# QingYunA/General-Medical-Image-Segmentation-CNN-Framework

Hardware: AMD Instinct MI355X
Metric: train voxels/sec (128^3 patches) 3D U-Net (higher is better)
Workload: dtype f32 (f16x3 split MFMA: every fp32 conv operand = two fp16 parts under a per-tensor power-of-two scale, three fp16 products per fp32 product, fp32 accumulate; graded against fp64 by the same tests as bf16x6 and the exact-fp32 MFMA path); 1 GPU; unet3d_f32_2x128: UNet3D(1,2,32) fwd+BCE+bwd+Adam+Dice, x=[2,1,128,128,128] fp32 per GPU, random-init (kaiming) weights, data-parallel replicas with RCCL gradient all-reduce, conv math f16x3; global_batch=2, parallelism=dp1, conv_math=f16x3, optimizer=torch.optim.Adam(fused=True)

## Files before the change

### general-medical-image-segmentation-cnn-framework_amd/csrc/bn_head.hip

```cpp
#include "common.h"
#include "internal.h"

namespace seg {

namespace {

constexpr int kBhMaxBlocks = 1024;

struct BhArgs {
    const float* y; int ldy;
    const float* mean; const float* rstd; const float* gamma; const float* beta;
    const float* wh; const float* bh;
    const float* dl; int lddl;
    float* out; int ldo;
    const float* s1; const float* s2;
    float* part;
    unsigned* amax;
    long long rows; int C; int act; float slope;
};

template <int K, int ACT>
__device__ __forceinline__ void bn_head_fwd_body(const BhArgs& a) {
    const int LPV = a.C / 4, VPB = 256 / LPV;
    const int c4 = threadIdx.x % LPV, vl = threadIdx.x / LPV;
    f32x4_t wr[K], al, be;
#pragma unroll
    for (int k = 0; k < K; ++k) wr[k] = ld4(a.wh + (long long)k * a.C + c4 * 4);
#pragma unroll
    for (int j = 0; j < 4; ++j) {
        al[j] = a.rstd[c4 * 4 + j] * (a.gamma ? a.gamma[c4 * 4 + j] : 1.f);
        be[j] = (a.beta ? a.beta[c4 * 4 + j] : 0.f) - a.mean[c4 * 4 + j] * al[j];
    }
    float bias[K];
#pragma unroll
// ... 104 lines not shown
        float s = vals[i];
        for (int o = 32; o >= LPV; o >>= 1) s += __shfl_xor(s, o, 64);
        vals[i] = s;
    }
    const int nl = LPV < 64 ? LPV : 64;
    if (lane < nl) {
#pragma unroll
        for (int i = 0; i < NS + K; ++i) sred[(wave * 64 + lane) * (NS + K) + i] = vals[i];
    }
    __syncthreads();
    const int ncol = (2 + K) * a.C + K;
    float* dst = a.part + (long long)blockIdx.x * ncol;
    for (int i = threadIdx.x; i < ncol; i += 256) {
        float s = 0.f;
        if (i < (2 + K) * a.C) {
            const int which = i / a.C, c = i % a.C;
            const int slot = which < 2 ? which * 4 + c % 4 : 8 + 4 * (which - 2) + c % 4;
            for (int w = 0; w < 4; ++w) s += sred[(w * 64 + (c / 4) % 64) * (NS + K) + slot];
        } else {
            const int k = i - (2 + K) * a.C;
            for (int w = 0; w < 4; ++w) s += sred[(w * 64 + 0) * (NS + K) + NS + k];
        }
        dst[i] = s;
    }
}
template <int K>
__global__ __launch_bounds__(256) void bn_head_bwd_sums_kernel(BhArgs a) {
    if (a.act == MI355SEG_ACT_RELU) bn_head_bwd_sums_body<K, MI355SEG_ACT_RELU>(a); else bn_head_bwd_sums_body<K, -1>(a);
}

__global__ __launch_bounds__(64) void bh_finalize_kernel(const float* __restrict__ part, int nblk, int ncol, float* __restrict__ o0, int n0,
                                                        float* __restrict__ o1, int n1, float* __restrict__ o2, int n2, float* __restrict__ o3,
                                                        float* __restrict__ alias0, float* __restrict__ alias1) {
    const int j = blockIdx.x;
    double s = 0.0;
    for (int b = threadIdx.x; b < nblk; b += 64) s += (double)part[(long long)b * ncol + j];
    s = wave_sum(s);
    if (threadIdx.x != 0) return;
    const float v = (float)s;
    if (j < n0) { o0[j] = v; if (alias0) alias0[j] = v; }
    else if (j < n0 + n1) { o1[j - n0] = v; if (alias1) alias1[j - n0] = v; }
    else if (j < n0 + n1 + n2) { if (o2) o2[j - n0 - n1] = v; }
    else if (o3) o3[j - n0 - n1 - n2] = v;
}

template <int K, int ACT>
__device__ __forceinline__ void bn_head_bwd_apply_body(const BhArgs& a) {
    __shared__ float sred[4 * 64 * 4];
    const int LPV = a.C / 4, VPB = 256 / LPV;
    const int c4 = threadIdx.x % LPV, vl = threadIdx.x / LPV;
    BhBwd<K> q;
    q.init(a, c4);
    const float invM = 1.f / (float)a.rows;
    f32x4_t k1, k2, sc, col = {0.f, 0.f, 0.f, 0.f};
#pragma unroll
    for (int j = 0; j < 4; ++j) { k1[j] = a.s1[c4 * 4 + j] * invM; k2[j] = a.s2[c4 * 4 + j] * invM; sc[j] = q.ga[j] * q.rs[j]; }
    float amax = 0.f;
    const long long stride = (long long)gridDim.x * VPB;
    for (long long v = (long long)blockIdx.x * VPB + vl; v < a.rows; v += 2 * stride) {
        const bool two = v + stride < a.rows;
        const float4 x0 = ldf4(a.y + v * a.ldy + c4 * 4);
        const float4 x1 = two ? ldf4(a.y + (v + stride) * a.ldy + c4 * 4) : make_float4(0.f, 0.f, 0.f, 0.f);
        float d0[K], d1[K];
#pragma unroll
        for (int k = 0; k < K; ++k) { d0[k] = a.dl[v * a.lddl + k]; d1[k] = two ? a.dl[(v + stride) * a.lddl + k] : 0.f; }
#pragma unroll
        for (int u = 0; u < 2; ++u) {
            if (u == 1 && !two) break;
            f32x4_t dz, xh, av;
            q.template eval<false, ACT>(a, u ? x1 : x0, u ? d1 : d0, dz, xh, av);
            f32x4_t od;
#pragma unroll
            for (int j = 0; j < 4; ++j) {
                od[j] = sc[j] * (dz[j] - k1[j] - xh[j] * k2[j]);
                amax = fmaxf(amax, fabsf(od[j]));
            }
// ... 219 lines not shown
}

int mi355seg_bn_act_head_bwd_sums_f32(const float* dlogits, int lddl, const float* y, int ldy, const float* mean, const float* rstd,
                                      const float* gamma, const float* beta, int act, float slope, const float* wh,
                                      float* s1, float* s2, float* dgamma, float* dbeta, float* dwh, float* dbh,
                                      long long rows, int C, int K, void* ws, size_t ws_bytes, void* stream) {
    SEG_CHECK_ARG(dlogits && y && mean && rstd && wh && s1 && s2 && bh_ok(rows, C, K, ldy) && lddl >= K && act >= 0 && act <= 4, "bn_act_head_bwd_sums: bad arguments");
    SEG_CHECK_ARG(((uintptr_t)y % 16) == 0 && ((uintptr_t)wh % 16) == 0, "bn_act_head_bwd_sums: y and the head weights must be 16-byte aligned");
    hipStream_t st = (hipStream_t)stream;
    const int grid = bh_grid(rows, 256 / (C / 4));
    const int ncol = (2 + K) * C + K;
    SEG_CHECK_WS((size_t)grid * ncol * sizeof(float), ws_bytes);
    BhArgs a{y, ldy, mean, rstd, gamma, beta, wh, nullptr, dlogits, lddl, nullptr, 0, nullptr, nullptr, (float*)ws, nullptr, rows, C, act, slope};
    {
        ProfScope ps(PF_NORM, 2.0 * rows * C * K * 2, 4.0 * rows * (C + K), st);
        BH_DISPATCH(bn_head_bwd_sums_kernel, K, grid, st, a);
        SEG_CHECK_LAUNCH();
    }
    hipLaunchKernelGGL(bh_finalize_kernel, dim3(ncol), dim3(64), 0, st, (const float*)ws, grid, ncol, s1, C, s2, C, dwh, K * C, dbh, dbeta, dgamma);
    SEG_CHECK_LAUNCH();
    return MI355SEG_OK;
}

int mi355seg_bn_act_head_bwd_apply_f32(const float* dlogits, int lddl, const float* y, int ldy, const float* mean, const float* rstd,
                                       const float* gamma, const float* beta, int act, float slope, const float* wh,
                                       const float* s1, const float* s2, float* dy, int lddy, float* dy_colsum, float* dy_amax,
                                       long long rows, int C, int K, void* ws, size_t ws_bytes, void* stream) {
    SEG_CHECK_ARG(dlogits && y && mean && rstd && wh && s1 && s2 && dy && bh_ok(rows, C, K, ldy) && lddl >= K && (lddy % 4) == 0 && act >= 0 && act <= 4,
                  "bn_act_head_bwd_apply: bad arguments");
    SEG_CHECK_ARG(((uintptr_t)y % 16) == 0 && ((uintptr_t)wh % 16) == 0 && ((uintptr_t)dy % 16) == 0, "bn_act_head_bwd_apply: y, dy and the head weights must be 16-byte aligned");
    hipStream_t st = (hipStream_t)stream;
    const int grid = bh_grid(rows, 256 / (C / 4)) * 2;
    if (dy_colsum) SEG_CHECK_WS((size_t)grid * C * sizeof(float), ws_bytes);
    BhArgs a{y, ldy, mean, rstd, gamma, beta, wh, nullptr, dlogits, lddl, dy, lddy, s1, s2, dy_colsum ? (float*)ws : nullptr,
             (unsigned*)dy_amax, rows, C, act, slope};
    {
        ProfScope ps(PF_NORM, 2.0 * rows * C * K, 4.0 * rows * (2.0 * C + K), st);
        BH_DISPATCH(bn_head_bwd_apply_kernel, K, grid, st, a);
        SEG_CHECK_LAUNCH();
    }
    if (dy_colsum) {
        hipLaunchKernelGGL(bh_finalize_kernel, dim3(C), dim3(64), 0, st, (const float*)ws, grid, C, dy_colsum, C, (float*)nullptr, 0, (float*)nullptr, 0,
                           (float*)nullptr, (float*)nullptr, (float*)nullptr);
        SEG_CHECK_LAUNCH();
    }
    return MI355SEG_OK;
}

int mi355seg_bn_act_pool_supported_f32(int N, int D, int H, int W, int C, int ldy) { return bp_ok(N, D, H, W, C, ldy) ? 1 : 0; }

size_t mi355seg_bn_act_pool_ws_bytes(int C) { return align_up((size_t)2 * kBhMaxBlocks * 2 * C * sizeof(float), 256) + 1024; }

int mi355seg_bn_act_pool_fwd_f32(const float* y, int ldy, const float* mean, const float* rstd, const float* gamma, const float* beta,
                                 int act, float slope, float* a, int lda, float* pooled, unsigned char* idx, float* a_amax,
                                 int N, int D, int H, int W, int C, void* stream) {
    SEG_CHECK_ARG(y && mean && rstd && a && pooled && idx && bp_ok(N, D, H, W, C, ldy) && (lda % 4) == 0 && act >= 0 && act <= 4, "bn_act_pool_fwd: bad arguments");
    SEG_CHECK_ARG(((uintptr_t)y % 16) == 0 && ((uintptr_t)a % 16) == 0 && ((uintptr_t)pooled % 16) == 0 && ((uintptr_t)idx % 4) == 0, "bn_act_pool_fwd: tensors must be 16-byte aligned");
    hipStream_t st = (hipStream_t)stream;
    BpArgs b{};
    b.y = y; b.ldy = ldy; b.mean = mean; b.rstd = rstd; b.gamma = gamma; b.beta = beta; b.a = a; b.lda = lda; b.p = pooled; b.idx = idx;
    b.amax = (unsigned*)a_amax; b.N = N; b.D = D; b.H = H; b.W = W; b.C = C; b.act = act; b.slope = slope;
    const long long npool = (long long)N * (D / 2) * (H / 2) * (W / 2);
    const int vpb = 256 / (C / 4);
    long long nb = (npool + vpb - 1) / vpb;
    nb = (nb + 3) / 4;
    const int grid = (int)(nb < 1 ? 1 : (nb > 4096 ? 4096 : nb));
    ProfScope ps(PF_NORM, 0.0, 4.0 * npool * C * (16.0 + 1.25), st);
    hipLaunchKernelGGL(bn_pool_fwd_kernel, dim3(grid), dim3(256), 0, st, b);
    SEG_CHECK_LAUNCH();
    return MI355SEG_OK;
}

int mi355seg_bn_act_pool_bwd_f32(const float* dskip, int ldds, const float* dpooled, const unsigned char* idx, const float* y, int ldy,
                                 const float* mean, const float* rstd, const float* gamma, const float* beta, int act, float slope,
                                 float* s1, float* s2, float* dgamma, float* dbeta, float* dy, int lddy, float* dy_colsum, float* dy_amax,
                                 int N, int D, int H, int W, int C, void* ws, size_t ws_bytes, void* stream) {
    SEG_CHECK_ARG(dskip && dpooled && idx && y && mean && rstd && s1 && s2 && dy && bp_ok(N, D, H, W, C, ldy) && (ldds % 4) == 0 && (lddy % 4) == 0 && act >= 0 && act <= 4,
                  "bn_act_pool_bwd: bad arguments");
    SEG_CHECK_ARG(((uintptr_t)y % 16) == 0 && ((uintptr_t)dskip % 16) == 0 && ((uintptr_t)dpooled % 16) == 0 && ((uintptr_t)dy % 16) == 0 && ((uintptr_t)idx % 4) == 0,
                  "bn_act_pool_bwd: tensors must be 16-byte aligned");
    hipStream_t st = (hipStream_t)stream;
    BpArgs b{};
    b.y = y; b.ldy = ldy; b.mean = mean; b.rstd = rstd; b.gamma = gamma; b.beta = beta; b.ds = dskip; b.ldds = ldds; b.dp = dpooled; b.cidx = idx;
    b.dy = dy; b.lddy = lddy; b.N = N; b.D = D; b.H = H; b.W = W; b.C = C; b.act = act; b.slope = slope;
    const long long npool = (long long)N * (D / 2) * (H / 2) * (W / 2);
    const int vpb = 256 / (C / 4);
    long long nb = (npool + vpb - 1) / vpb;
    nb = (nb + 3) / 4;
    const int grid = (int)(nb < 1 ? 1 : (nb > 2 * kBhMaxBlocks ? 2 * kBhMaxBlocks : nb));
    SEG_CHECK_WS((size_t)grid * 2 * C * sizeof(float), ws_bytes);
    b.part = (float*)ws;
    {
        ProfScope ps(PF_NORM, 0.0, 4.0 * npool * C * (16.0 + 1.25), st);
        hipLaunchKernelGGL(bn_pool_bwd_kernel<false>, dim3(grid), dim3(256), 0, st, b);
        SEG_CHECK_LAUNCH();
    }
    hipLaunchKernelGGL(bh_finalize_kernel, dim3(2 * C), dim3(64), 0, st, (const float*)ws, grid, 2 * C, s1, C, s2, C, (float*)nullptr, 0, (float*)nullptr, dbeta, dgamma);
    SEG_CHECK_LAUNCH();
    b.s1 = s1; b.s2 = s2; b.amax = (unsigned*)dy_amax; b.part = dy_colsum ? (float*)ws : nullptr;
    {
        ProfScope ps(PF_NORM, 0.0, 4.0 * npool * C * (24.0 + 1.25), st);
        hipLaunchKernelGGL(bn_pool_bwd_kernel<true>, dim3(grid), dim3(256), 0, st, b);
        SEG_CHECK_LAUNCH();
    }
    if (dy_colsum) {
        hipLaunchKernelGGL(bh_finalize_kernel, dim3(C), dim3(64), 0, st, (const float*)ws, grid, C, dy_colsum, C, (float*)nullptr, 0, (float*)nullptr, 0,
                           (float*)nullptr, (float*)nullptr, (float*)nullptr);
        SEG_CHECK_LAUNCH();
    }
    return MI355SEG_OK;
}

}
```

### general-medical-image-segmentation-cnn-framework_amd/csrc/conv_generic.hip

```cpp
#include "common.h"
#include "internal.h"
#include <string.h>
#include <stdlib.h>

namespace seg {

__global__ void pack_w_fwd_kernel(const float* __restrict__ w, float* __restrict__ wp, int Cout, int Cin, int T) {
    long long total = (long long)Cout * Cin * T;
    for (long long i = (long long)blockIdx.x * blockDim.x + threadIdx.x; i < total; i += (long long)gridDim.x * blockDim.x) {
        int co = (int)(i % Cout);
        long long r = i / Cout;
        int ci = (int)(r % Cin);
        int t = (int)(r / Cin);
        wp[i] = w[((long long)co * Cin + ci) * T + t];
    }
}
__global__ void pack_w_dgrad_kernel(const float* __restrict__ w, float* __restrict__ wd, int Cout, int Cin, int T, int flip) {
    long long total = (long long)Cout * Cin * T;
    for (long long i = (long long)blockIdx.x * blockDim.x + threadIdx.x; i < total; i += (long long)gridDim.x * blockDim.x) {
        int ci = (int)(i % Cin);
        long long r = i / Cin;
        int co = (int)(r % Cout);
        int t = (int)(r / Cout);
        int ts = flip ? (T - 1 - t) : t;
        wd[i] = w[((long long)co * Cin + ci) * T + ts];
    }
}

void pack_w_fwd(const float* w, float* wp, int Cout, int Cin, int T, hipStream_t st) {
    long long total = (long long)Cout * Cin * T;
    int grid = (int)((total + 255) / 256 > 2048 ? 2048 : (total + 255) / 256);
    hipLaunchKernelGGL(pack_w_fwd_kernel, dim3(grid), dim3(256), 0, st, w, wp, Cout, Cin, T);
}
void pack_w_dgrad(const float* w, float* wd, int Cout, int Cin, int T, int flip, hipStream_t st) {
// ... 80 lines not shown
            }
        }
        dx[v * lddx + ci] = acc;
    }
}

__global__ __launch_bounds__(256) void conv_wgrad_generic_kernel(const float* __restrict__ dy, int lddy,
        const float* __restrict__ x, int ldx, float* __restrict__ part, ConvGeom g, long long vox_per_split) {
    const int pair = blockIdx.x * blockDim.x + threadIdx.x;
    const int npair = g.Cin * g.Cout;
    const int tap = blockIdx.y;
    const int split = blockIdx.z;
    const int kw = tap % g.k, kh = (tap / g.k) % g.k, kd = tap / (g.k * g.k);
    const long long nvox = (long long)g.N * g.Do * g.Ho * g.Wo;
    long long v0 = (long long)split * vox_per_split;
    long long v1 = v0 + vox_per_split; if (v1 > nvox) v1 = nvox;
    if (pair >= npair) return;
    const int co = pair % g.Cout, ci = pair / g.Cout;
    float acc = 0.f;
    for (long long v = v0; v < v1; ++v) {
        int ow = (int)(v % g.Wo); long long r = v / g.Wo;
        int oh = (int)(r % g.Ho); r /= g.Ho;
        int od = (int)(r % g.Do); int n = (int)(r / g.Do);
        int id = od * g.stride - g.pad + kd, ih = oh * g.stride - g.pad + kh, iw = ow * g.stride - g.pad + kw;
        if ((unsigned)id >= (unsigned)g.D || (unsigned)ih >= (unsigned)g.H || (unsigned)iw >= (unsigned)g.W) continue;
        acc = fmaf(dy[v * lddy + co], x[((((long long)n * g.D + id) * g.H + ih) * g.W + iw) * ldx + ci], acc);
    }
    part[(((long long)split * gridDim.y + tap) * g.Cin + ci) * g.Cout + co] = acc;
}

__global__ __launch_bounds__(256) void wgrad_reduce_kernel(const float* __restrict__ part, float* __restrict__ dw, int splits, int T, int Cin,
                                                           int Cout, int accumulate, int CIT, int TT) {
    extern __shared__ float tr[];
    const long long total = (long long)T * Cin * Cout;
    const int co0 = blockIdx.x * 32, ci0 = blockIdx.y * CIT, t0 = blockIdx.z * TT;
    const int tn = min(TT, T - t0);
    const int run = CIT * TT, pitch = run + 1;
    for (int e0 = threadIdx.x; e0 < 32 * run; e0 += 1024) {
        long long idx[4]; int dst[4]; bool ok[4];
        double s[4] = {0.0, 0.0, 0.0, 0.0};
#pragma unroll
        for (int u = 0; u < 4; ++u) {
            const int e = e0 + 256 * u;
            const int col = e & 31, r = e >> 5;
            const int cil = r % CIT, tl = r / CIT;
            const int co = co0 + col, ci = ci0 + cil;
            ok[u] = e < 32 * run && co < Cout && ci < Cin && tl < tn;
            idx[u] = ok[u] ? ((long long)(t0 + tl) * Cin + ci) * Cout + co : 0;
            dst[u] = e < 32 * run ? col * pitch + cil * TT + tl : -1;
        }
        for (int k = 0; k < splits; ++k) {
            float v[4];
#pragma unroll
            for (int u = 0; u < 4; ++u) v[u] = part[(long long)k * total + idx[u]];
#pragma unroll
            for (int u = 0; u < 4; ++u) if (ok[u]) s[u] += (double)v[u];
        }
#pragma unroll
        for (int u = 0; u < 4; ++u) if (dst[u] >= 0) tr[dst[u]] = (float)s[u];
    }
    __syncthreads();
    const int cin_here = min(CIT, Cin - ci0);
    for (int e = threadIdx.x; e < 32 * run; e += 256) {
        const int col = e / run, j = e - col * run;
        const int cil = j / TT, tl = j - cil * TT;
        const int co = co0 + col;
        if (co < Cout && cil < cin_here && tl < tn) {
            const long long o = ((long long)co * Cin + ci0 + cil) * T + t0 + tl;
            const float v = tr[col * pitch + j];
            dw[o] = accumulate ? dw[o] + v : v;
        }
    }
}

__global__ void wgrad_reduce_flat_kernel(const float* __restrict__ part, float* __restrict__ dw, int splits, int T, int Cin,
                                         int Cout, int accumulate) {
    long long total = (long long)T * Cin * Cout;
    for (long long i = (long long)blockIdx.x * blockDim.x + threadIdx.x; i < total; i += (long long)gridDim.x * blockDim.x) {
        int co = (int)(i % Cout);
        long long r = i / Cout;
        int ci = (int)(r % Cin);
        int t = (int)(r / Cin);
        double s = 0.0;
        int k = 0;
        for (; k + 8 <= splits; k += 8) {
            float v[8];
#pragma unroll
            for (int u = 0; u < 8; ++u) v[u] = part[(long long)(k + u) * total + i];
#pragma unroll
            for (int u = 0; u < 8; ++u) s += (double)v[u];
        }
        for (; k < splits; ++k) s += (double)part[(long long)k * total + i];
        long long o = ((long long)co * Cin + ci) * T + t;
        dw[o] = accumulate ? dw[o] + (float)s : (float)s;
    }
}

__global__ __launch_bounds__(256) void wgrad_reduce_cols_kernel(const float* __restrict__ part, float* __restrict__ dw, int splits, int T, int Cin,
                                                                int Cout, int accumulate) {
    __shared__ double sh[8][32];
    const long long total = (long long)T * Cin * Cout;
    const int c = threadIdx.x & 31, q = threadIdx.x >> 5;
    const long long col = (long long)blockIdx.x * 32 + c;
    double s0 = 0.0, s1 = 0.0;
    if (col < total) {
        const float* p = part + col;
        int k = q;
        for (; k + 8 < splits; k += 16) { s0 += (double)p[(long long)k * total]; s1 += (double)p[(long long)(k + 8) * total]; }
        if (k < splits) s0 += (double)p[(long long)k * total];
    }
    sh[q][c] = s0 + s1;
    __syncthreads();
    if (q == 0 && col < total) {
        double s = sh[0][c];
#pragma unroll
        for (int j = 1; j < 8; ++j) s += sh[j][c];
        const int co = (int)(col % Cout); const long long r = col / Cout;
        const int ci = (int)(r % Cin), t = (int)(r / Cin);
        const long long o = ((long long)co * Cin + ci) * T + t;
        dw[o] = accumulate ? dw[o] + (float)s : (float)s;
    }
}

__global__ __launch_bounds__(256) void wgrad_reduce_cols_swapped_kernel(const float* __restrict__ part, float* __restrict__ dw, int splits, int T, int Cin,
                                                                        int Cout, int accumulate) {
    __shared__ double sh[8][32];
    const long long total = (long long)T * Cin * Cout;
    const int c = threadIdx.x & 31, q = threadIdx.x >> 5;
    const long long col = (long long)blockIdx.x * 32 + c;
    double s0 = 0.0, s1 = 0.0;
    if (col < total) {
        const float* p = part + col;
        int k = q;
        for (; k + 8 < splits; k += 16) { s0 += (double)p[(long long)k * total]; s1 += (double)p[(long long)(k + 8) * total]; }
        if (k < splits) s0 += (double)p[(long long)k * total];
    }
    sh[q][c] = s0 + s1;
    __syncthreads();
    if (q == 0 && col < total) {
        double s = sh[0][c];
#pragma unroll
        for (int j = 1; j < 8; ++j) s += sh[j][c];
        const int ci = (int)(col % Cin); const long long r = col / Cin;
        const int co = (int)(r % Cout), tp = (int)(r / Cout);
        const long long o = ((long long)co * Cin + ci) * T + (T - 1 - tp);
        dw[o] = accumulate ? dw[o] + (float)s : (float)s;
    }
}
void wgrad_reduce_swapped(const float* part, float* dw, int splits, int T, int Cin, int Cout, int accumulate, hipStream_t st) {
    const long long total = (long long)T * Cin * Cout;
    hipLaunchKernelGGL(wgrad_reduce_cols_swapped_kernel, dim3((unsigned)((total + 31) / 32)), dim3(256), 0, st, part, dw, splits, T, Cin, Cout, accumulate);
}

void wgrad_reduce(const float* part, float* dw, int splits, int T, int Cin, int Cout, int accumulate, hipStream_t st) {
    const int TT = T > 256 ? 256 : T;
    int CIT = 256 / TT;
    CIT = CIT < 1 ? 1 : (CIT > 32 ? 32 : CIT);
    if (CIT > Cin) CIT = Cin;
    auto blocks = [&](int cit) { return (long long)((Cout + 31) / 32) * ((Cin + cit - 1) / cit) * ((T + TT - 1) / TT); };
    if (splits >= 8) {
        const long long total = (long long)T * Cin * Cout;
        hipLaunchKernelGGL(wgrad_reduce_cols_kernel, dim3((unsigned)((total + 31) / 32)), dim3(256), 0, st, part, dw, splits, T, Cin, Cout, accumulate);
        return;
    }
    while (CIT > 1 && blocks(CIT) < 1024) CIT = (CIT + 1) / 2;
    if (blocks(CIT) < 256) {
        long long total = (long long)T * Cin * Cout;
        int grid = (int)((total + 255) / 256 > 4096 ? 4096 : (total + 255) / 256);
        hipLaunchKernelGGL(wgrad_reduce_flat_kernel, dim3(grid), dim3(256), 0, st, part, dw, splits, T, Cin, Cout, accumulate);
        return;
    }
    const size_t lds = (size_t)32 * (CIT * TT + 1) * sizeof(float);
    hipLaunchKernelGGL(wgrad_reduce_kernel, dim3((Cout + 31) / 32, (Cin + CIT - 1) / CIT, (T + TT - 1) / TT), dim3(256), lds, st, part, dw,
                       splits, T, Cin, Cout, accumulate, CIT, TT);
}

static int generic_splits(const ConvGeom& g) {
    const int T = g.k * g.k * g.k;
    const long long nvox = (long long)g.N * g.Do * g.Ho * g.Wo;
    int pairblocks = cdiv((long long)g.Cin * g.Cout, 256);
    long long want = 4096 / ((long long)pairblocks * T) + 1;
    long long maxs = nvox / 64 + 1;
    if (want > maxs) want = maxs;
    if (want > 128) want = 128;
    if (want < 1) want = 1;
    return (int)want;
}

size_t conv_generic_ws_bytes(int N, int D, int H, int W, int Cin, int Cout, int k, int stride, int pad) {
    ConvGeom g{N, D, H, W, Cin, Cout, k, stride, pad, (D + 2 * pad - k) / stride + 1, (H + 2 * pad - k) / stride + 1,
               (W + 2 * pad - k) / stride + 1};
    const size_t T = (size_t)k * k * k;
    size_t wbytes = align_up(T * Cin * Cout * sizeof(float), 256);
    size_t part = align_up((size_t)generic_splits(g) * T * Cin * Cout * sizeof(float), 256);
    size_t red = colsum_ws_bytes(Cout);
    return wbytes + (part > red ? part : red) + 1024;
}

static int ew_blocks(long long total) {
    long long b = (total + 255) / 256;
    return (int)(b < 1 ? 1 : (b > 16384 ? 16384 : b));
}

int conv_fwd_generic(const float* x, int ldx, const float* w, const float* bias, float* y, int ldy, const ConvGeom& g,
// ... 9 lines not shown
    {
        ProfScope ps(PF_GENERIC, 2.0 * total * T * g.Cin, 0.0, st);
        hipLaunchKernelGGL(conv_fwd_generic_kernel, dim3(ew_blocks(total)), dim3(256), 0, st, x, ldx, wp, bias, y, ldy, g);
    }
    SEG_CHECK_LAUNCH();
    if (ssum || ssq)
        return channel_sums(y, ldy, (long long)g.N * g.Do * g.Ho * g.Wo, g.Cout, ssum, ssq, nullptr, 0, (char*)ws + off,
                            ws_bytes - off, st);
    return MI355SEG_OK;
}

int conv_dgrad_generic(const float* dy, int lddy, const float* w, float* dx, int lddx, const ConvGeom& g, void* ws,
                       size_t ws_bytes, hipStream_t st) {
    const int T = g.k * g.k * g.k;
    Carver cv(ws);
    float* wd = cv.take<float>((size_t)T * g.Cin * g.Cout);
    SEG_CHECK_WS(cv.used(), ws_bytes);
    pack_w_dgrad(w, wd, g.Cout, g.Cin, T, 0, st);
    SEG_CHECK_LAUNCH();
    long long total = (long long)g.N * g.D * g.H * g.W * g.Cin;
    {
        ProfScope ps(PF_GENERIC, 2.0 * total * T * g.Cout, 0.0, st);
        hipLaunchKernelGGL(conv_dgrad_generic_kernel, dim3(ew_blocks(total)), dim3(256), 0, st, dy, lddy, wd, dx, lddx, g);
    }
    SEG_CHECK_LAUNCH();
    return MI355SEG_OK;
}

int conv_wgrad_generic(const float* dy, int lddy, const float* x, int ldx, float* dw, const ConvGeom& g, int accumulate,
                       void* ws, size_t ws_bytes, hipStream_t st) {
    const int T = g.k * g.k * g.k;
    const int splits = generic_splits(g);
    Carver cv(ws);
    float* part = cv.take<float>((size_t)splits * T * g.Cin * g.Cout);
    SEG_CHECK_WS(cv.used(), ws_bytes);
    const long long nvox = (long long)g.N * g.Do * g.Ho * g.Wo;
    long long vps = (nvox + splits - 1) / splits;
    dim3 grid(cdiv((long long)g.Cin * g.Cout, 256), T, splits);
    {
        ProfScope ps(PF_GENERIC, 2.0 * nvox * T * g.Cin * g.Cout, 0.0, st);
        hipLaunchKernelGGL(conv_wgrad_generic_kernel, grid, dim3(256), 0, st, dy, lddy, x, ldx, part, g, vps);
    }
    SEG_CHECK_LAUNCH();
    wgrad_reduce(part, dw, splits, T, g.Cin, g.Cout, accumulate, st);
    SEG_CHECK_LAUNCH();
    return MI355SEG_OK;
}

int conv_call(ConvCall* c, const char* who, const void* x, int ldx, const void* w, const void* y, int ldy, int N, int D, int H, int W,
              int Cin, int Cout, int k, int stride, int pad, void* ws, size_t ws_bytes, void* stream) {
    SEG_CHECK_ARG(N > 0 && D > 0 && H > 0 && W > 0 && Cin > 0 && Cout > 0, "%s: non-positive extent", who);
    SEG_CHECK_ARG(k >= 1 && k <= 16 && stride >= 1 && pad >= 0, "%s: bad k/stride/pad %d/%d/%d", who, k, stride, pad);
    SEG_CHECK_ARG(D + 2 * pad >= k && H + 2 * pad >= k && W + 2 * pad >= k, "%s: kernel larger than padded input", who);
    SEG_CHECK_ARG(x && w && y && ldx >= Cin && ldy >= Cout, "%s: null pointer or pitch < channels", who);
    *c = ConvCall{{N, D, H, W, Cin, Cout, k, stride, pad, (D + 2 * pad - k) / stride + 1, (H + 2 * pad - k) / stride + 1, (W + 2 * pad - k) / stride + 1},
                  ldx, ldy, x, y, w, ws, ws_bytes, (hipStream_t)stream};
    return MI355SEG_OK;
}

size_t ladder_ws_bytes(const Rung* r, const ConvGeom& g) {
    const ConvKey d = dense_key(g);
    size_t most = 0;
    for (;; ++r) {
        if (r->ws && (r->reach ? r->reach(g) : !r->fits || (r->fits(d) && (!r->aligned || r->aligned(d))))) {
            const size_t need = r->ws(g);
            if (need > most) most = need;
        }
// ... 458 lines not shown
```

### general-medical-image-segmentation-cnn-framework_amd/csrc/conv_gwgrad.hip

```cpp
#include "common.h"
#include "internal.h"

namespace seg {

using f32x16 = __attribute__((ext_vector_type(16))) float;
using f32x4 = __attribute__((ext_vector_type(4))) float;

struct GwArgs {
    const void* x; const void* dy; float* part;
    int ldx, lddy, N, D, H, W, Do, Ho, Wo, Cin, Cout, k, stride, pad, T;
    int ntiles, nstrips, npairs, ncob, ngroups;
};

constexpr int GW_V = 64, GW_TG = 8;
constexpr int GW_XIT = GW_TG * GW_V * 8 / 256, GW_DIT = GW_V * 8 / 256;
constexpr int GW_LDS = (GW_V * 32 + GW_TG * GW_V * 32) * 4;

template <typename IN_T>
__global__ __launch_bounds__(256, 2) void conv_gwgrad_kernel(GwArgs a) {
    const IN_T* __restrict__ xin = reinterpret_cast<const IN_T*>(a.x);
    const IN_T* __restrict__ dyin = reinterpret_cast<const IN_T*>(a.dy);
    extern __shared__ __attribute__((aligned(16))) float lds[];
    float* ds = lds;
    float* xs = lds + GW_V * 32;
    const int tid = threadIdx.x, lane = tid & 63;
    const int wave = __builtin_amdgcn_readfirstlane(tid >> 6);
    const int h = lane >> 5, i = lane & 31;

    const int nwg = gridDim.x, bid = blockIdx.x;
    const int q8 = nwg >> 3, r8 = nwg & 7, xcd = bid & 7;
    int t = (xcd < r8 ? xcd * (q8 + 1) : r8 * (q8 + 1) + (xcd - r8) * q8) + (bid >> 3);
    const int tg = t % a.ngroups; t /= a.ngroups;
    const int pair = t % a.npairs, strip = t / a.npairs;
    const int ci0 = (pair / a.ncob) * 32, co0 = (pair % a.ncob) * 32;
// ... 85 lines not shown
    p->ngroups = (p->T + GW_TG - 1) / GW_TG;
    long long units = (long long)p->npairs * p->ngroups;
    long long want = (768 + units - 1) / units;
    long long cap = (long long)(96u << 20) / ((long long)p->T * Cin * Cout * 4);
    if (cap < 1) cap = 1;
    if (want > cap) want = cap;
    if (want > p->ntiles) want = p->ntiles;
    if (want < 1) want = 1;
    p->nstrips = (int)want;
    return units * want < (1ll << 30);
}

size_t gwgrad_ws_bytes(int N, int D, int H, int W, int Cin, int Cout, int k, int stride, int pad) {
    GwPlan p;
    const int Do = (D + 2 * pad - k) / stride + 1, Ho = (H + 2 * pad - k) / stride + 1, Wo = (W + 2 * pad - k) / stride + 1;
    if (!gw_plan(N, Do, Ho, Wo, Cin, Cout, k, &p)) return 0;
    return align_up((size_t)p.nstrips * p.T * Cin * Cout * sizeof(float), 256) + 1024;
}

bool gwgrad_supported(int N, int D, int H, int W, int Cin, int Cout, int k, int stride, int pad, int ldx, int lddy) {
    GwPlan p;
    const int Do = (D + 2 * pad - k) / stride + 1, Ho = (H + 2 * pad - k) / stride + 1, Wo = (W + 2 * pad - k) / stride + 1;
    return (ldx % 4) == 0 && (lddy % 4) == 0 && k <= 7 && gw_plan(N, Do, Ho, Wo, Cin, Cout, k, &p);
}

template <typename IN_T>
int conv_gwgrad(const IN_T* dy, int lddy, const IN_T* x, int ldx, float* dw, int N, int D, int H, int W, int Cin, int Cout,
                int k, int stride, int pad, int accumulate, void* ws, size_t ws_bytes, hipStream_t st) {
    GwPlan p;
    const int Do = (D + 2 * pad - k) / stride + 1, Ho = (H + 2 * pad - k) / stride + 1, Wo = (W + 2 * pad - k) / stride + 1;
    SEG_CHECK_ARG(gw_plan(N, Do, Ho, Wo, Cin, Cout, k, &p), "conv_gwgrad: unsupported shape");
    SEG_CHECK_ARG(((uintptr_t)x % (4 * sizeof(IN_T))) == 0 && ((uintptr_t)dy % (4 * sizeof(IN_T))) == 0, "conv_gwgrad: pointers must be aligned to four elements");
    Carver cv(ws);
    float* part = cv.take<float>((size_t)p.nstrips * p.T * Cin * Cout);
    SEG_CHECK_WS(cv.used(), ws_bytes);
    GwArgs a{x, dy, part, ldx, lddy, N, D, H, W, Do, Ho, Wo, Cin, Cout, k, stride, pad, p.T,
             p.ntiles, p.nstrips, p.npairs, (Cout + 31) / 32, p.ngroups};
    const int nwg = p.nstrips * p.npairs * p.ngroups;
    const double vox = (double)N * Do * Ho * Wo;
    {
        ProfScope ps(PF_WGRAD, 2.0 * vox * p.T * Cin * Cout, (double)sizeof(IN_T) * vox * ((double)p.T * Cin + Cout) + 4.0 * p.T * Cin * Cout, st);
        SEG_SET_LDS((conv_gwgrad_kernel<IN_T>), GW_LDS);
        hipLaunchKernelGGL(conv_gwgrad_kernel<IN_T>, dim3(nwg), dim3(256), GW_LDS, st, a);
        SEG_CHECK_LAUNCH();
    }
    wgrad_reduce(part, dw, p.nstrips, p.T, Cin, Cout, accumulate, st);
    SEG_CHECK_LAUNCH();
    return MI355SEG_OK;
}

template int conv_gwgrad<float>(const float*, int, const float*, int, float*, int, int, int, int, int, int, int, int, int, int, void*, size_t, hipStream_t);
template int conv_gwgrad<bf16>(const bf16*, int, const bf16*, int, float*, int, int, int, int, int, int, int, int, int, int, void*, size_t, hipStream_t);

}
```

### general-medical-image-segmentation-cnn-framework_amd/csrc/conv_small.hip

```cpp
#include "common.h"
#include "internal.h"

namespace seg {

using f32x4 = __attribute__((ext_vector_type(4))) float;

struct SmallGeom { int N, D, H, W, Cin, Cout, ldx, ldy; };

template <typename T, int CIN>
__global__ __launch_bounds__(256) void stem_fwd_kernel(const T* __restrict__ x, const float* __restrict__ w,
        const float* __restrict__ bias, T* __restrict__ y, float* __restrict__ spart, SmallGeom g) {
    extern __shared__ __attribute__((aligned(16))) float sw[];
    const int Cout = g.Cout, LPV = Cout / 4;
    for (int i = threadIdx.x; i < 27 * CIN * Cout; i += 256) {
        int co = i % Cout, r = i / Cout, ci = r % CIN, tap = r / CIN;
        sw[i] = w[((long long)co * CIN + ci) * 27 + tap];
    }
    __syncthreads();
    const int cq = threadIdx.x % LPV, vl = threadIdx.x / LPV, VPB = 256 / LPV;
    const long long nvox = (long long)g.N * g.D * g.H * g.W;
    f32x4 bv = {0.f, 0.f, 0.f, 0.f};
    if (bias) bv = ld4(bias + cq * 4);
    f32x4 s1 = {0.f, 0.f, 0.f, 0.f}, s2 = s1;
    for (long long v = (long long)blockIdx.x * VPB + vl; v < nvox; v += (long long)gridDim.x * VPB) {
        int xw = (int)(v % g.W); long long r = v / g.W;
        int yh = (int)(r % g.H); r /= g.H;
        int zd = (int)(r % g.D); int n = (int)(r / g.D);
        f32x4 acc = bv;
#pragma unroll
        for (int tap = 0; tap < 27; ++tap) {
            const int dz = tap / 9 - 1, dy = (tap / 3) % 3 - 1, dx = tap % 3 - 1;
            const int iz = zd + dz, iy = yh + dy, ix = xw + dx;
            if ((unsigned)iz < (unsigned)g.D && (unsigned)iy < (unsigned)g.H && (unsigned)ix < (unsigned)g.W) {
                const T* xp = x + ((((long long)n * g.D + iz) * g.H + iy) * g.W + ix) * g.ldx;
// ... 362 lines not shown
            float s = acc[t][j];
            for (int o = 32; o >= LPV; o >>= 1) s += __shfl_xor(s, o, 64);
            acc[t][j] = s;
        }
    }
#pragma unroll
    for (int j = 0; j < 4; ++j) {
        float s = col[j];
        for (int o = 32; o >= LPV; o >>= 1) s += __shfl_xor(s, o, 64);
        col[j] = s;
    }
    __syncthreads();
    if (lane < LPV) {
#pragma unroll
        for (int t = 0; t < 27; ++t) st4(sm + ((wave * 28 + t) * LPV + lane) * 4, acc[t]);
        st4(sm + ((wave * 28 + 27) * LPV + lane) * 4, col);
    }
    __syncthreads();
    for (int i = threadIdx.x; i < 28 * Cout; i += 256) {
        const int t = i / Cout, co = i % Cout;
        float s = 0.f;
        for (int w = 0; w < 4; ++w) s += sm[((w * 28 + t) * LPV + co / 4) * 4 + co % 4];
        if (t < 27) part[((long long)blockIdx.x * 27 + t) * Cout + co] = s;
        else cpart[(long long)blockIdx.x * Cout + co] = s;
    }
}
__global__ __launch_bounds__(256, 2) void stem1_wgrad_bn_kernel(const float* __restrict__ x, StemBn b, float* __restrict__ part, float* __restrict__ cpart,
                                                               SmallGeom g, int ntiles) {
    if (b.act == MI355SEG_ACT_RELU) stem1_wgrad_bn_body<MI355SEG_ACT_RELU>(x, b, part, cpart, g, ntiles);
    else stem1_wgrad_bn_body<-1>(x, b, part, cpart, g, ntiles);
}

__global__ __launch_bounds__(64) void colpart_finalize_kernel(const float* __restrict__ cpart, int nblk, int C, float* __restrict__ out) {
    const int c = blockIdx.x;
    double s = 0.0;
    for (int k = threadIdx.x; k < nblk; k += 64) s += (double)cpart[(long long)k * C + c];
    s = wave_sum(s);
    if (threadIdx.x == 0) out[c] = (float)s;
}

template <typename T>
__global__ __launch_bounds__(256) void stem1k5_wgrad_kernel(const T* __restrict__ x, const T* __restrict__ dy,
        float* __restrict__ part, SmallGeom g, int lddy, int ntiles) {
    extern __shared__ __attribute__((aligned(16))) float sm[];
    const int Cout = g.Cout, LPV = Cout / 4, TX = 256 / LPV, HX = TX + 4, HY = S1_TY + 4;
    const int cq = threadIdx.x % LPV, xs = threadIdx.x / LPV;
    const int dzp = blockIdx.y;
    f32x4 acc[25];
#pragma unroll
    for (int t = 0; t < 25; ++t) acc[t] = f32x4{0.f, 0.f, 0.f, 0.f};
    const int ntx = g.W / TX, nty = g.H / S1_TY, ntz = g.D / S1_TZ;
    for (int tile = blockIdx.x; tile < ntiles; tile += gridDim.x) {
        int mt = tile;
        const int txi = mt % ntx; mt /= ntx;
        const int tyi = mt % nty; mt /= nty;
        const int tzi = mt % ntz; const int n = mt / ntz;
        const int x0 = txi * TX, y0 = tyi * S1_TY, z0 = tzi * S1_TZ;
        f32x4 dreg[S1_TZ * S1_TY];
#pragma unroll
        for (int line = 0; line < S1_TZ * S1_TY; ++line) {
            const int lz = line / S1_TY, ly = line % S1_TY;
            const long long v = (((long long)n * g.D + z0 + lz) * g.H + y0 + ly) * g.W + x0 + xs;
            dreg[line] = ld4(dy + v * lddy + cq * 4);
        }
        __syncthreads();
        for (int p = threadIdx.x; p < HX * HY * S1_TZ; p += 256) {
            const int hx = p % HX, r = p / HX, hy = r % HY, hz = r / HY;
            const int gz = z0 + hz + dzp - 2, gy = y0 - 2 + hy, gx = x0 - 2 + hx;
            float v = 0.f;
            if ((unsigned)gz < (unsigned)g.D && (unsigned)gy < (unsigned)g.H && (unsigned)gx < (unsigned)g.W)
                v = ld1(x + ((((long long)n * g.D + gz) * g.H + gy) * g.W + gx) * g.ldx);
// ... 80 lines not shown
    __syncthreads();
    if (threadIdx.x < g.Cin * g.Cout) {
        const int ci = threadIdx.x / g.Cout, co = threadIdx.x % g.Cout;
        part[((long long)blockIdx.x * g.Cin + ci) * g.Cout + co] = sh[0][ci * 4 + co] + sh[1][ci * 4 + co] + sh[2][ci * 4 + co] + sh[3][ci * 4 + co];
    }
}

static bool stem1_tiled_ok(const SmallGeom& g) {
    if (g.Cin != 1) return false;
    const int TX = 256 / (g.Cout / 4);
    return g.W % TX == 0 && g.H % S1_TY == 0 && g.D % S1_TZ == 0;
}
static size_t stem1_lds(int Cout) {
    const int TX = 256 / (Cout / 4);
    size_t a = (size_t)(TX + 2) * (S1_TY + 2) * (S1_TZ + 2) * 4, b = 256 * 9 * 4, c = (size_t)4 * 27 * Cout * 4;
    size_t m = a > b ? a : b;
    return m > c ? m : c;
}

bool stem_wgrad_bn_supported(int N, int D, int H, int W, int Cin, int Cout, int k, int stride, int pad) {
    if (!(k == 3 && stride == 1 && pad == 1 && Cin == 1 && Cout % 4 == 0 && Cout >= 4 && Cout <= 64 && ((Cout / 4) & (Cout / 4 - 1)) == 0)) return false;
    SmallGeom g{N, D, H, W, Cin, Cout, 1, Cout};
    return stem1_tiled_ok(g) && ((size_t)stem_bn_scratch_floats(Cout) + 6 * Cout) * 4 + (size_t)S1_TZ * S1_TY * 256 * 16 <= 80 * 1024;
}

int stem_wgrad_bn(const float* da, int ldda, const float* y, int ldy, const float* mean, const float* rstd, const float* gamma, const float* beta,
                  int act, float slope, const float* s1, const float* s2, const float* x, int ldx, float* dw, float* db,
                  int N, int D, int H, int W, int Cout, void* ws, size_t ws_bytes, hipStream_t st) {
    SmallGeom g{N, D, H, W, 1, Cout, ldx, 0};
    const long long nvox = (long long)N * D * H * W;
    const int ntiles = (int)(nvox / ((long long)S1_TZ * S1_TY * (256 / (Cout / 4))));
    const int nb = ntiles < 512 ? ntiles : 512;
    Carver cv(ws);
    float* part = cv.take<float>((size_t)nb * 27 * Cout);
    float* cpart = cv.take<float>((size_t)nb * Cout);
    SEG_CHECK_WS(cv.used(), ws_bytes);
    StemBn b{da, ldda, y, ldy, mean, rstd, gamma, beta, s1, s2, act, slope, 1.f / (float)nvox};
    const size_t lds = ((size_t)stem_bn_scratch_floats(Cout) + 6 * Cout) * 4 + (size_t)S1_TZ * S1_TY * 256 * 16;
    {
        ProfScope ps(PF_DIRECT, 2.0 * nvox * 27.0 * Cout, 4.0 * nvox * (1 + 2.0 * Cout), st);
        hipLaunchKernelGGL(stem1_wgrad_bn_kernel, dim3(nb), dim3(256), lds, st, x, b, part, cpart, g, ntiles);
        SEG_CHECK_LAUNCH();
    }
    wgrad_reduce(part, dw, nb, 27, 1, Cout, 0, st);
    SEG_CHECK_LAUNCH();
    if (db) {
        hipLaunchKernelGGL(colpart_finalize_kernel, dim3(Cout), dim3(64), 0, st, cpart, nb, Cout, db);
        SEG_CHECK_LAUNCH();
    }
    return MI355SEG_OK;
}

template <typename T, int COUT>
__global__ __launch_bounds__(256) void head_fwd_kernel(const T* __restrict__ x, const float* __restrict__ w,
        const float* __restrict__ bias, T* __restrict__ y, SmallGeom g) {
    const int LPV = g.Cin / 4, VPB = 256 / LPV;
    const int c4 = threadIdx.x % LPV, vl = threadIdx.x / LPV;
    const long long nvox = (long long)g.N * g.D * g.H * g.W;
    f32x4 wr[COUT];
#pragma unroll
    for (int co = 0; co < COUT; ++co) wr[co] = ld4(w + (long long)co * g.Cin + c4 * 4);
    for (long long v = (long long)blockIdx.x * VPB + vl; v < nvox; v += (long long)gridDim.x * VPB) {
        const f32x4 xv = ld4(x + v * g.ldx + c4 * 4);
        float o[COUT];
#pragma unroll
        for (int co = 0; co < COUT; ++co) {
            float s = xv[0] * wr[co][0] + xv[1] * wr[co][1] + xv[2] * wr[co][2] + xv[3] * wr[co][3];
            for (int off = LPV >> 1; off > 0; off >>= 1) s += __shfl_xor(s, off, 64);
            o[co] = s + (bias ? bias[co] : 0.f);
        }
        if (c4 == 0) {
#pragma unroll
            for (int co = 0; co < COUT; ++co) y[v * g.ldy + co] = o[co];
        }
    }
}

template <typename T, int COUT>
__global__ __launch_bounds__(256) void head_dgrad_kernel(const T* __restrict__ dy, int lddy, const float* __restrict__ w,
// ... 193 lines not shown
template <typename T>
int smallcin_wgrad(const T* dy, int lddy, const T* x, int ldx, float* dw, int N, int D, int H, int W, int Cin, int Cout,
                   int k, int stride, int pad, int accumulate, void* ws, size_t ws_bytes, hipStream_t st) {
    SmallConv g{N, D, H, W, (D + 2 * pad - k) / stride + 1, (H + 2 * pad - k) / stride + 1, (W + 2 * pad - k) / stride + 1,
                Cin, Cout, k, stride, pad, k * k * k, ldx, lddy};
    const long long nvox = (long long)N * g.Do * g.Ho * g.Wo;
    if (Cin == 1 && k == 5 && stride == 1 && pad == 2 && Cout % 4 == 0 && Cout <= 64 && (256 % (Cout / 4)) == 0 && lddy % 4 == 0 &&
        ((uintptr_t)dy % (4 * sizeof(T))) == 0) {
        SmallGeom sg{N, D, H, W, 1, Cout, ldx, 0};
        const int TX = 256 / (Cout / 4);
        if (W % TX == 0 && H % S1_TY == 0 && D % S1_TZ == 0) {
            if constexpr (sizeof(T) == 4) note_conv_path(MI355SEG_PATH_WGRAD_SMALLCIN_K5_TILED);
            const int ntiles = (int)(nvox / ((long long)S1_TZ * S1_TY * TX));
            int nb = ntiles < 128 ? ntiles : 128;
            SEG_CHECK_WS((size_t)nb * 125 * Cout * sizeof(float), ws_bytes);
            float* part5 = (float*)ws;
            size_t lds5 = (size_t)(TX + 4) * (S1_TY + 4) * S1_TZ * 4, red5 = (size_t)4 * 25 * Cout * 4;
            if (red5 > lds5) lds5 = red5;
            {
                ProfScope ps(PF_DIRECT, 2.0 * nvox * 125.0 * Cout, (double)sizeof(T) * nvox * (1 + Cout), st);
                hipLaunchKernelGGL((stem1k5_wgrad_kernel<T>), dim3(nb, 5), dim3(256), lds5, st, x, dy, part5, sg, lddy, ntiles);
                SEG_CHECK_LAUNCH();
            }
            wgrad_reduce(part5, dw, nb, 125, 1, Cout, accumulate, st);
            SEG_CHECK_LAUNCH();
            return MI355SEG_OK;
        }
    }
    if constexpr (sizeof(T) == 4) note_conv_path(MI355SEG_PATH_WGRAD_SMALLCIN);
    const int vw = (Cout % 4 == 0) ? 4 : 1, lpv = Cout / vw;
    int nblk = small_grid(nvox, 256 / lpv);
    if (nblk > 512) nblk = 512;
    SEG_CHECK_WS((size_t)nblk * g.T * Cin * Cout * sizeof(float), ws_bytes);
    float* part = (float*)ws;
    const int TPG = 25;
    dim3 grid(nblk, Cin, (g.T + TPG - 1) / TPG);
    size_t lds = (size_t)4 * TPG * Cout * 4;
    {
        ProfScope ps(PF_DIRECT, 2.0 * nvox * g.T * Cin * Cout, (double)sizeof(T) * nvox * (Cin + Cout), st);
        if (vw == 4) hipLaunchKernelGGL((smallcin_wgrad_kernel<T, 25, 4>), grid, dim3(256), lds, st, x, dy, part, g);
        else hipLaunchKernelGGL((smallcin_wgrad_kernel<T, 25, 1>), grid, dim3(256), lds, st, x, dy, part, g);
        SEG_CHECK_LAUNCH();
    }
    wgrad_reduce(part, dw, nblk, g.T, Cin, Cout, accumulate, st);
    SEG_CHECK_LAUNCH();
    return MI355SEG_OK;
}

template <typename T>
int smallcout_wgrad(const T* dy, int lddy, const T* x, int ldx, float* dw, int N, int D, int H, int W, int Cin, int Cout,
                    int k, int stride, int pad, int accumulate, void* ws, size_t ws_bytes, hipStream_t st) {
    SmallConv g{N, D, H, W, (D + 2 * pad - k) / stride + 1, (H + 2 * pad - k) / stride + 1, (W + 2 * pad - k) / stride + 1,
                Cin, Cout, k, stride, pad, k * k * k, ldx, lddy};
    const long long nvox = (long long)N * g.Do * g.Ho * g.Wo;
    int nblk = small_grid(nvox, 256 / (Cin / 4));
    if (nblk > 512) nblk = 512;
    SEG_CHECK_WS((size_t)nblk * g.T * Cin * Cout * sizeof(float), ws_bytes);
    float* part = (float*)ws;
    {
        ProfScope ps(PF_DIRECT, 2.0 * nvox * g.T * Cin * Cout, (double)sizeof(T) * nvox * (Cin + Cout), st);
        if (Cout == 2) {
            constexpr int TPG = 25;
            dim3 grid(nblk, (g.T + TPG - 1) / TPG);
            hipLaunchKernelGGL((smallcout_wgrad_kernel<T, 2, TPG>), grid, dim3(256), (size_t)4 * TPG * 2 * (Cin / 4) * 16, st, x, dy, part, g);
        } else {
            constexpr int TPG = 13;
            dim3 grid(nblk, (g.T + TPG - 1) / TPG);
            hipLaunchKernelGGL((smallcout_wgrad_kernel<T, 4, TPG>), grid, dim3(256), (size_t)4 * TPG * 4 * (Cin / 4) * 16, st, x, dy, part, g);
        }
        SEG_CHECK_LAUNCH();
    }
    wgrad_reduce(part, dw, nblk, g.T, Cin, Cout, accumulate, st);
    SEG_CHECK_LAUNCH();
    return MI355SEG_OK;
}

bool stem_supported(int Cin, int Cout, int k, int stride, int pad, int ldy) {
    const int lpv = Cout / 4;
    return k == 3 && stride == 1 && pad == 1 && (Cin == 1 || Cin == 2 || Cin == 4) && Cout % 4 == 0 && Cout >= 4 && Cout <= 64 &&
           (lpv & (lpv - 1)) == 0 && ldy % 4 == 0;
}
bool head_supported(int Cin, int Cout, int k, int stride, int pad, int ldx) {
    const int lpv = Cin / 4;
    return k == 1 && stride == 1 && pad == 0 && (Cout == 2 || Cout == 4) && Cin % 4 == 0 && Cin >= 4 && Cin <= 256 &&
           (lpv & (lpv - 1)) == 0 && ldx % 4 == 0;
}

size_t small_ws_bytes(int Cin, int Cout, int k) {
    size_t T = (size_t)k * k * k;
    return align_up((size_t)1024 * T * Cin * Cout * sizeof(float), 256) + colsum_ws_bytes(Cout) + 1024;
}
// ... 23 lines not shown
            }
            else hipLaunchKernelGGL((stem1_fwd_kernel<T, false>), dim3(nb), dim3(256), stem1_lds(Cout), st, x, w, bias, y, spart, g, ntiles, (unsigned*)nullptr);
            SEG_CHECK_LAUNCH();
        }
        if (in_kernel) {
            if (!tile_stats_finalize2(spart, nb, Cout, ssum, ssq, reinterpret_cast<double*>((char*)ws + sp_bytes), st)) { set_error("stem_fwd: statistics finalise refused"); return MI355SEG_EINVAL; }
            SEG_CHECK_LAUNCH();
            return MI355SEG_OK;
        }
        if (ssum) return channel_sums(y, ldy, nvox, Cout, ssum, ssq, nullptr, 0, ws, ws_bytes, st);
        return MI355SEG_OK;
    }
    {
        ProfScope ps(PF_DIRECT, 2.0 * nvox * 27.0 * Cin * Cout, (double)sizeof(T) * nvox * (Cin + Cout), st);
        if constexpr (sizeof(T) == 4) note_conv_path(Cin == 1 ? MI355SEG_PATH_FWD_STEM_C1 : (Cin == 2 ? MI355SEG_PATH_FWD_STEM_C2 : MI355SEG_PATH_FWD_STEM_C4));
        if (Cin == 1) hipLaunchKernelGGL((stem_fwd_kernel<T, 1>), dim3(nblk), dim3(256), lds, st, x, w, bias, y, spart, g);
        else if (Cin == 2) hipLaunchKernelGGL((stem_fwd_kernel<T, 2>), dim3(nblk), dim3(256), lds, st, x, w, bias, y, spart, g);
        else hipLaunchKernelGGL((stem_fwd_kernel<T, 4>), dim3(nblk), dim3(256), lds, st, x, w, bias, y, spart, g);
        SEG_CHECK_LAUNCH();
    }
    if (ssum) return channel_sums(y, ldy, nvox, Cout, ssum, ssq, nullptr, 0, ws, ws_bytes, st);
    return MI355SEG_OK;
}

template <typename T>
int stem_wgrad(const T* dy, int lddy, const T* x, int ldx, float* dw, int N, int D, int H, int W, int Cin, int Cout,
               int accumulate, void* ws, size_t ws_bytes, hipStream_t st) {
    SmallGeom g{N, D, H, W, Cin, Cout, ldx, 0};
    const long long nvox = (long long)N * D * H * W;
    const int vpb = 256 / (Cout / 4);
    int nblk = small_grid(nvox, vpb);
    if (nblk > 512) nblk = 512;
    SEG_CHECK_WS((size_t)nblk * 27 * Cin * Cout * sizeof(float), ws_bytes);
    float* part = (float*)ws;
    size_t lds = (size_t)4 * 27 * Cout * 4;
    if (stem1_tiled_ok(g)) {
        const int ntiles = (int)(nvox / ((long long)S1_TZ * S1_TY * (256 / (Cout / 4))));
        int nb = ntiles < 512 ? ntiles : 512;
        if constexpr (sizeof(T) == 4) note_conv_path(MI355SEG_PATH_WGRAD_STEM_TILED);
        {
            ProfScope ps(PF_DIRECT, 2.0 * nvox * 27.0 * Cin * Cout, (double)sizeof(T) * nvox * (Cin + Cout), st);
            hipLaunchKernelGGL(stem1_wgrad_kernel<T>, dim3(nb), dim3(256), stem1_lds(Cout), st, x, dy, part, g, lddy, ntiles);
            SEG_CHECK_LAUNCH();
        }
        wgrad_reduce(part, dw, nb, 27, Cin, Cout, accumulate, st);
        SEG_CHECK_LAUNCH();
        return MI355SEG_OK;
    }
    if (Cin == 4 && ldx % 4 == 0 && ((uintptr_t)x % (4 * sizeof(T))) == 0 && (size_t)4 * 9 * 4 * Cout * 4 <= 64 * 1024) {
        if constexpr (sizeof(T) == 4) note_conv_path(MI355SEG_PATH_WGRAD_STEM_C4);
        ProfScope ps(PF_DIRECT, 2.0 * nvox * 27.0 * Cin * Cout, (double)sizeof(T) * nvox * (Cin + Cout), st);
        hipLaunchKernelGGL((stem4_wgrad_kernel<T>), dim3(nblk, 3), dim3(256), (size_t)4 * 9 * 4 * Cout * 4, st, x, dy, part, g, lddy);
        SEG_CHECK_LAUNCH();
    } else {
        if constexpr (sizeof(T) == 4) note_conv_path(MI355SEG_PATH_WGRAD_STEM);
        ProfScope ps(PF_DIRECT, 2.0 * nvox * 27.0 * Cin * Cout, (double)sizeof(T) * nvox * (Cin + Cout), st);
        hipLaunchKernelGGL((stem_wgrad_kernel<T, 0>), dim3(nblk, Cin), dim3(256), lds, st, x, dy, part, g, lddy);
        SEG_CHECK_LAUNCH();
    }
    wgrad_reduce(part, dw, nblk, 27, Cin, Cout, accumulate, st);
    SEG_CHECK_LAUNCH();
    return MI355SEG_OK;
}

template <typename T>
int head_fwd(const T* x, int ldx, const float* w, const float* bias, T* y, int ldy, int N, int D, int H, int W, int Cin,
             int Cout, hipStream_t st) {
    SmallGeom g{N, D, H, W, Cin, Cout, ldx, ldy};
    const long long nvox = (long long)N * D * H * W;
    const int nblk = small_grid(nvox, 256 / (Cin / 4)) * 2;
    ProfScope ps(PF_DIRECT, 2.0 * nvox * Cin * Cout, (double)sizeof(T) * nvox * (Cin + Cout), st);
    if (Cout == 2) hipLaunchKernelGGL((head_fwd_kernel<T, 2>), dim3(nblk), dim3(256), 0, st, x, w, bias, y, g);
    else hipLaunchKernelGGL((head_fwd_kernel<T, 4>), dim3(nblk), dim3(256), 0, st, x, w, bias, y, g);
    SEG_CHECK_LAUNCH();
    return MI355SEG_OK;
}

template <typename T>
int head_dgrad(const T* dy, int lddy, const float* w, T* dx, int lddx, int N, int D, int H, int W, int Cin, int Cout,
               hipStream_t st) {
    SmallGeom g{N, D, H, W, Cin, Cout, lddx, 0};
    const long long nvox = (long long)N * D * H * W;
    const int nblk = small_grid(nvox, 256 / (Cin / 4)) * 2;
    ProfScope ps(PF_DIRECT, 2.0 * nvox * Cin * Cout, (double)sizeof(T) * nvox * (Cin + Cout), st);
    if (Cout == 2) hipLaunchKernelGGL((head_dgrad_kernel<T, 2>), dim3(nblk), dim3(256), 0, st, dy, lddy, w, dx, g);
    else hipLaunchKernelGGL((head_dgrad_kernel<T, 4>), dim3(nblk), dim3(256), 0, st, dy, lddy, w, dx, g);
    SEG_CHECK_LAUNCH();
    return MI355SEG_OK;
}

template <typename T>
int head_wgrad(const T* dy, int lddy, const T* x, int ldx, float* dw, int N, int D, int H, int W, int Cin, int Cout,
               int accumulate, void* ws, size_t ws_bytes, hipStream_t st) {
    SmallGeom g{N, D, H, W, Cin, Cout, ldx, 0};
    const long long nvox = (long long)N * D * H * W;
    int nblk = small_grid(nvox, 256 / (Cin / 4));
    if (nblk > 512) nblk = 512;
    SEG_CHECK_WS((size_t)nblk * Cin * Cout * sizeof(float), ws_bytes);
    float* part = (float*)ws;
    {
        ProfScope ps(PF_DIRECT, 2.0 * nvox * Cin * Cout, (double)sizeof(T) * nvox * (Cin + Cout), st);
        if (Cout == 2) hipLaunchKernelGGL((head_wgrad_kernel<T, 2>), dim3(nblk), dim3(256), 0, st, x, dy, lddy, part, g);
        else hipLaunchKernelGGL((head_wgrad_kernel<T, 4>), dim3(nblk), dim3(256), 0, st, x, dy, lddy, part, g);
        SEG_CHECK_LAUNCH();
    }
    wgrad_reduce(part, dw, nblk, 1, Cin, Cout, accumulate, st);
    SEG_CHECK_LAUNCH();
    return MI355SEG_OK;
}

bool tinypw_supported(int Cin, int Cout, int k, int stride, int pad) { return k == 1 && stride == 1 && pad == 0 && Cin <= 4 && Cout <= 4; }
template <typename T>
int tinypw_fwd(const T* x, int ldx, const float* w, const float* bias, T* y, int ldy, long long nvox, int Cin, int Cout, hipStream_t st) {
    TinyPw g{Cin, Cout, ldx, ldy, nvox};
    ProfScope ps(PF_DIRECT, 2.0 * nvox * Cin * Cout, (double)sizeof(T) * nvox * (Cin + Cout), st);
    hipLaunchKernelGGL((tinypw_fwd_kernel<T>), dim3(small_grid(nvox, 256) * 4), dim3(256), 0, st, x, w, bias, y, g);
    SEG_CHECK_LAUNCH();
    return MI355SEG_OK;
}
template <typename T>
int tinypw_dgrad(const T* dy, int lddy, const float* w, T* dx, int lddx, long long nvox, int Cin, int Cout, hipStream_t st) {
    TinyPw g{Cin, Cout, lddx, lddy, nvox};
    ProfScope ps(PF_DIRECT, 2.0 * nvox * Cin * Cout, (double)sizeof(T) * nvox * (Cin + Cout), st);
    hipLaunchKernelGGL((tinypw_dgrad_kernel<T>), dim3(small_grid(nvox, 256) * 4), dim3(256), 0, st, dy, w, dx, g);
    SEG_CHECK_LAUNCH();
    return MI355SEG_OK;
}
template <typename T>
int tinypw_wgrad(const T* dy, int lddy, const T* x, int ldx, float* dw, long long nvox, int Cin, int Cout, int accumulate, void* ws, size_t ws_bytes,
                 hipStream_t st) {
    TinyPw g{Cin, Cout, ldx, lddy, nvox};
    int nblk = small_grid(nvox, 256);
    if (nblk > 512) nblk = 512;
    SEG_CHECK_WS((size_t)nblk * Cin * Cout * sizeof(float), ws_bytes);
    float* part = (float*)ws;
    {
        ProfScope ps(PF_DIRECT, 2.0 * nvox * Cin * Cout, (double)sizeof(T) * nvox * (Cin + Cout), st);
        hipLaunchKernelGGL((tinypw_wgrad_kernel<T>), dim3(nblk), dim3(256), 0, st, x, dy, part, g);
        SEG_CHECK_LAUNCH();
    }
    wgrad_reduce(part, dw, nblk, 1, Cin, Cout, accumulate, st);
    SEG_CHECK_LAUNCH();
    return MI355SEG_OK;
}

#define SEG_INST(T) \
    template int smallcin_wgrad<T>(const T*, int, const T*, int, float*, int, int, int, int, int, int, int, int, int, int, void*, size_t, hipStream_t); \
    template int smallcout_wgrad<T>(const T*, int, const T*, int, float*, int, int, int, int, int, int, int, int, int, int, void*, size_t, hipStream_t); \
    template int stem_fwd<T>(const T*, int, const float*, const float*, T*, int, int, int, int, int, int, int, double*, double*, void*, size_t, hipStream_t, float*, bool*); \
    template int stem_wgrad<T>(const T*, int, const T*, int, float*, int, int, int, int, int, int, int, void*, size_t, hipStream_t); \
    template int head_fwd<T>(const T*, int, const float*, const float*, T*, int, int, int, int, int, int, int, hipStream_t); \
    template int head_dgrad<T>(const T*, int, const float*, T*, int, int, int, int, int, int, int, hipStream_t); \
    template int head_wgrad<T>(const T*, int, const T*, int, float*, int, int, int, int, int, int, int, void*, size_t, hipStream_t); \
    template int tinypw_fwd<T>(const T*, int, const float*, const float*, T*, int, long long, int, int, hipStream_t); \
    template int tinypw_dgrad<T>(const T*, int, const float*, T*, int, long long, int, int, hipStream_t); \
    template int tinypw_wgrad<T>(const T*, int, const T*, int, float*, long long, int, int, int, void*, size_t, hipStream_t);
SEG_INST(float)
SEG_INST(bf16)
#undef SEG_INST

}
```

### general-medical-image-segmentation-cnn-framework_amd/csrc/conv_wgrad_lowp.hip

```cpp
#include "common.h"
#include "internal.h"
#include <initializer_list>
#include <type_traits>
#include <stdlib.h>

namespace seg {

using f32x16 = __attribute__((ext_vector_type(16))) float;
using f32x4 = __attribute__((ext_vector_type(4))) float;
typedef short s16x4 __attribute__((ext_vector_type(4)));
typedef short s16x8 __attribute__((ext_vector_type(8)));
typedef __attribute__((address_space(3))) s16x4 lds_s16x4;

constexpr int LW_WAVES = 8;
constexpr int LW_THREADS = LW_WAVES * 64;
constexpr int LW_TPW = 4;

template <int BX, int KS, int NP, int S = 1>
struct LTile {
    static constexpr int HALO = KS / 2;
    static constexpr int NTAPS = KS == 3 ? 27 : KS * KS;
    static constexpr int PLANES = KS == 3 ? 1 : KS;
    static constexpr int VOX = (NP >= 2 || S == 2) ? 128 : 256;
    static constexpr int TY = BX == 8 ? 8 : 4;
    static constexpr int LINES = VOX / BX;
    static constexpr int TZ = LINES / TY;
    static constexpr int HX = (BX - 1) * S + KS, HY = (TY - 1) * S + KS, HZ = KS == 3 ? (TZ - 1) * S + 3 : TZ;
    static_assert(S == 1 || KS == 3, "strided tiles are built for k3");
    static constexpr int NVOX = HX * HY * HZ;
    static constexpr int ROW = 64 * NP + (S == 1 ? 32 : 0);
    static constexpr int KSTEPS = VOX / 32;
    static constexpr int X_BYTES = NVOX * ROW, D_BYTES = VOX * ROW;
    static constexpr int LDS_BYTES = X_BYTES + D_BYTES;
    static_assert(TZ >= 1 && LINES % TY == 0, "tile lines must fill whole y-rows");
// ... 711 lines not shown
    SEG_SET_LDS((conv_wgrad_wide_kernel<BX, KS, IN_T>), F::LDS_BYTES);
    hipLaunchKernelGGL((conv_wgrad_wide_kernel<BX, KS, IN_T>), dim3(nwg), dim3(FW_THREADS), F::LDS_BYTES, st, a);
}

template <int KS>
static void dispatch_lwgrad(int math, const LWgradPlan& p, const LWgradArgs& a, int nwg, hipStream_t st) {
    if (math == MATH_X3 && a.amax_x) {
        if (p.BX == 16) launch_lwgrad<16, KS, 2, float>(a, nwg, st);
        else launch_lwgrad<8, KS, 2, float>(a, nwg, st);
    } else if (math == MATH_X3) {
        if (p.BX == 16) launch_lwgrad<16, KS, 3, float>(a, nwg, st);
        else launch_lwgrad<8, KS, 3, float>(a, nwg, st);
    } else {
        if (p.BX == 32) launch_lwgrad<32, KS, 1, bf16>(a, nwg, st);
        else if (p.BX == 16) launch_lwgrad<16, KS, 1, bf16>(a, nwg, st);
        else launch_lwgrad<8, KS, 1, bf16>(a, nwg, st);
    }
}

int conv_wgrad_lowp(int math, const void* dy, int lddy, const void* x, int ldx, float* dw, int N, int D, int H, int W, int Cin,
                    int Cout, int k, int stride, int accumulate, void* ws, size_t ws_bytes, hipStream_t st, const float* x_amax, const float* dy_amax,
                    const ConvPro* pro) {
    LWgradPlan p;
    const int pad = k / 2, Do = lw_out(D, k, stride, pad), Ho = lw_out(H, k, stride, pad), Wo = lw_out(W, k, stride, pad);
    const bool wide = g_wgrad_wide != 0 && (math == MATH_B16 || (math == MATH_X3 && x3_f16())) && lwgrad_plan(math, k, stride, N, Do, Ho, Wo, Cin, Cout, &p, true);
    LWgradPlan psw;
    const bool swap = !wide && !pro && g_wgrad_wide != 0 && math == MATH_X3 && x3_f16() && k == 3 && stride == 1 && Cin % 64 == 0 && Cout % 64 != 0 &&
                      lwgrad_plan(math, k, stride, N, Do, Ho, Wo, Cout, Cin, &psw, true) && psw.nstrips >= 8 && lw_offsets_fit(math, Ho, Wo, lddy, H, W, ldx);
    if (math == MATH_X3) note_conv_path(wide ? MI355SEG_PATH_WGRAD_LOWP_WIDE : (swap ? MI355SEG_PATH_WGRAD_LOWP_SWAPPED : MI355SEG_PATH_WGRAD_LOWP_NARROW));
    else if (math == MATH_B16) note_conv_path(wide ? MI355SEG_PATH_B16_WGRAD_LOWP_WIDE : (swap ? MI355SEG_PATH_B16_WGRAD_LOWP_SWAPPED : MI355SEG_PATH_B16_WGRAD_LOWP_NARROW));
    if (swap) {
        SEG_CHECK_ARG(((uintptr_t)x % 16) == 0 && ((uintptr_t)dy % 16) == 0, "conv_wgrad_lowp: pointers must be 16-byte aligned");
        Carver cv(ws);
        float* part = cv.take<float>((size_t)psw.nstrips * psw.taps * Cin * Cout);
        float* amax = cv.take<float>(2);
        SEG_CHECK_WS(cv.used(), ws_bytes);
        LWgradArgs a{dy, x, part, lddy, ldx, N, D, H, W, Cout, Cin, Do, Ho, Wo, psw.ntx, psw.nty, psw.ntz, psw.ntiles, psw.nstrips, psw.npairs, Cin / psw.cob, psw.taps,
                     nullptr, nullptr, nullptr, nullptr, 0, 0.f, 0};
        if (!x_amax || !dy_amax) {
            if (hipMemsetAsync(amax, 0, 2 * sizeof(float), st) != hipSuccess) { set_error("conv_wgrad_lowp: hipMemsetAsync failed"); return MI355SEG_EHIP; }
            if (!x_amax) { tensor_amax((const float*)x, ldx, (long long)N * D * H * W, Cin, nullptr, amax, st); x_amax = amax; }
            if (!dy_amax) { tensor_amax((const float*)dy, lddy, (long long)N * Do * Ho * Wo, Cout, nullptr, amax + 1, st); dy_amax = amax + 1; }
            SEG_CHECK_LAUNCH();
        }
        a.amax_x = dy_amax; a.amax_dy = x_amax;
#ifdef MI355SEG_TUNE
        { static const char* e = getenv("MI355SEG_DBG"); a.dbg = e ? atoi(e) : 0; }
#endif
        const int nwg = psw.nstrips * psw.npairs * psw.planes;
        const double vox = (double)N * Do * Ho * Wo;
        {
            ProfScope ps(PF_WGRAD, 2.0 * vox * psw.taps * Cin * Cout, 4.0 * vox * (Cin + Cout) + 4.0 * psw.taps * Cin * Cout, st);
            if (psw.BX == 16) launch_wide<16, 3, float>(a, nwg, st); else launch_wide<8, 3, float>(a, nwg, st);
            SEG_CHECK_LAUNCH();
        }
        wgrad_reduce_swapped(part, dw, psw.nstrips, psw.taps, Cin, Cout, accumulate, st);
        SEG_CHECK_LAUNCH();
        return MI355SEG_OK;
    }
    SEG_CHECK_ARG(wide || lwgrad_plan(math, k, stride, N, Do, Ho, Wo, Cin, Cout, &p), "conv_wgrad_lowp: unsupported shape");
    SEG_CHECK_ARG(((uintptr_t)x % 16) == 0 && ((uintptr_t)dy % 16) == 0, "conv_wgrad_lowp: pointers must be 16-byte aligned");
    SEG_CHECK_ARG(lw_offsets_fit(math, H, W, ldx, Ho, Wo, lddy), "conv_wgrad_lowp: a tile's halo spans more than 2 GB (wgrad_lowp_supported says so)");
    Carver cv(ws);
    float* part = cv.take<float>((size_t)p.nstrips * p.taps * Cin * Cout);
    const bool f16 = math == MATH_X3 && x3_f16();
    float* amax = f16 ? cv.take<float>(2) : nullptr;
    SEG_CHECK_WS(cv.used(), ws_bytes);
    LWgradArgs a{x, dy, part, ldx, lddy, N, D, H, W, Cin, Cout, Do, Ho, Wo, p.ntx, p.nty, p.ntz, p.ntiles, p.nstrips, p.npairs, Cout / p.cob, p.taps, nullptr, nullptr, nullptr, nullptr, 0, 0.f, 0};
    if (f16) {
        if (!x_amax || !dy_amax) {
            if (hipMemsetAsync(amax, 0, 2 * sizeof(float), st) != hipSuccess) { set_error("conv_wgrad_lowp: hipMemsetAsync failed"); return MI355SEG_EHIP; }
            if (!x_amax) { tensor_amax((const float*)x, ldx, (long long)N * D * H * W, Cin, nullptr, amax, st); x_amax = amax; }
            if (!dy_amax) { tensor_amax((const float*)dy, lddy, (long long)N * Do * Ho * Wo, Cout, nullptr, amax + 1, st); dy_amax = amax + 1; }
            SEG_CHECK_LAUNCH();
        }
        a.amax_x = x_amax; a.amax_dy = dy_amax;
    }
    if (pro) {
        SEG_CHECK_ARG(f16 && stride == 1 && k == 3 && pro->al && pro->be && conv_pro_act_ok(pro->act) && x_amax, "conv_wgrad_lowp: the norm + activation prologue needs the f16x3 k3 kernels and the caller's bound on the prologue's output");
        a.pro_al = pro->al; a.pro_be = pro->be; a.pro_act = pro->act; a.pro_slope = pro->act == MI355SEG_ACT_RELU ? 0.f : pro->slope;
        SEG_CHECK_ARG(a.pro_slope >= 0.f && a.pro_slope < 1.f, "conv_wgrad_lowp: prologue slope must lie in [0, 1)");
    }
#ifdef MI355SEG_TUNE
    { static const char* e = getenv("MI355SEG_DBG"); a.dbg = e ? atoi(e) : 0; }
#endif
    const int nwg = p.nstrips * p.npairs * p.planes;
    const double vox = (double)N * Do * Ho * Wo;
    {
        ProfScope ps(PF_WGRAD, 2.0 * vox * p.taps * Cin * Cout, (math == MATH_B16 ? 2.0 : 4.0) * vox * (Cin + Cout) + 4.0 * p.taps * Cin * Cout, st);
        if (wide) {
            if (math == MATH_X3) { if (p.BX == 16) launch_wide<16, 3, float>(a, nwg, st); else launch_wide<8, 3, float>(a, nwg, st); }
            else if (k == 3) { if (p.BX == 32) launch_wide<32, 3, bf16>(a, nwg, st); else if (p.BX == 16) launch_wide<16, 3, bf16>(a, nwg, st); else launch_wide<8, 3, bf16>(a, nwg, st); }
            else { if (p.BX == 32) launch_wide<32, 5, bf16>(a, nwg, st); else if (p.BX == 16) launch_wide<16, 5, bf16>(a, nwg, st); else launch_wide<8, 5, bf16>(a, nwg, st); }
        }
        else if (k == 3 && stride == 2) {
            if (p.BX == 32) launch_lwgrad<32, 3, 1, bf16, 2>(a, nwg, st);
            else if (p.BX == 16) launch_lwgrad<16, 3, 1, bf16, 2>(a, nwg, st);
// ... 13 lines not shown
```

### general-medical-image-segmentation-cnn-framework_amd/csrc/conv_wgrad_mfma.hip

```cpp
#include "common.h"
#include "internal.h"
#include <initializer_list>

namespace seg {

using f32x16 = __attribute__((ext_vector_type(16))) float;
using f32x4 = __attribute__((ext_vector_type(4))) float;

constexpr int WG_WAVES = 8;
constexpr int WG_THREADS = WG_WAVES * 64;
constexpr int TPW = (27 + WG_WAVES - 1) / WG_WAVES;

template <int BX, int KS>
struct WTile {
    static constexpr int HALO = KS / 2;
    static constexpr int NTAPS = KS == 3 ? 27 : KS * KS;
    static constexpr int PLANES = KS == 3 ? 1 : KS;
    static constexpr int TY = BX == 8 ? 8 : 4;
    static constexpr int LINES = 256 / BX;
    static constexpr int TZ = LINES / TY;
    static constexpr int HX = BX + 2 * HALO, HY = TY + 2 * HALO, HZ = KS == 3 ? TZ + 2 : TZ;
    static_assert((NTAPS + WG_WAVES - 1) / WG_WAVES == TPW, "tap dealing assumes 4 tap-tiles per wave");
    static constexpr int NVOX = HX * HY * HZ;
    static constexpr int XPIECES = NVOX * 8;
    static constexpr int XITER = (XPIECES + WG_THREADS - 1) / WG_THREADS;
    static constexpr int DYITER = 256 * 8 / WG_THREADS;
    static constexpr int X_FLOATS = NVOX * 32;
    static constexpr int LDS_BYTES = (X_FLOATS + 256 * 32) * 4;
};

struct WgradArgs {
    const float* x; const float* dy; float* part;
    int ldx, lddy, N, D, H, W, Cin, Cout;
    int ntx, nty, ntz, ntiles, nstrips, npairs, ncob, ntaps_total;
// ... 148 lines not shown
    if (cap < 1) cap = 1;
    if (want > cap) want = (int)cap;
    if (want > p->ntiles) want = p->ntiles;
    if (want < 1) want = 1;
    p->nstrips = want;
    return true;
}

bool wgrad_mfma_supported(int N, int D, int H, int W, int Cin, int Cout, int k, int stride, int pad, int ldx, int lddy) {
    if (!((k == 3 && pad == 1) || (k == 5 && pad == 2)) || stride != 1 || (ldx % 4) || (lddy % 4)) return false;
    WgradPlan p;
    return wgrad_plan(k, N, D, H, W, Cin, Cout, &p);
}

size_t wgrad_mfma_ws_bytes(int N, int D, int H, int W, int Cin, int Cout, int k) {
    WgradPlan p;
    if (!wgrad_plan(k, N, D, H, W, Cin, Cout, &p)) return 0;
    return align_up((size_t)p.nstrips * p.taps * Cin * Cout * sizeof(float), 256) + 1024;
}

template <int BX, int KS>
static void launch_wgrad(const WgradArgs& a, int nwg, hipStream_t st) {
    using T = WTile<BX, KS>;
    SEG_SET_LDS((conv_wgrad_kernel<BX, KS>), T::LDS_BYTES);
    hipLaunchKernelGGL((conv_wgrad_kernel<BX, KS>), dim3(nwg), dim3(WG_THREADS), T::LDS_BYTES, st, a);
}

int conv_wgrad_mfma(const float* dy, int lddy, const float* x, int ldx, float* dw, int N, int D, int H, int W, int Cin,
                    int Cout, int k, int accumulate, void* ws, size_t ws_bytes, hipStream_t st) {
    WgradPlan p;
    SEG_CHECK_ARG(wgrad_plan(k, N, D, H, W, Cin, Cout, &p), "conv_wgrad_mfma: unsupported shape");
    SEG_CHECK_ARG(((uintptr_t)x % 16) == 0 && ((uintptr_t)dy % 16) == 0, "conv_wgrad_mfma: pointers must be 16-byte aligned");
    Carver cv(ws);
    float* part = cv.take<float>((size_t)p.nstrips * p.taps * Cin * Cout);
    SEG_CHECK_WS(cv.used(), ws_bytes);
    WgradArgs a{x, dy, part, ldx, lddy, N, D, H, W, Cin, Cout, p.ntx, p.nty, p.ntz, p.ntiles, p.nstrips, p.npairs, Cout / 32, p.taps};
    const int nwg = p.nstrips * p.npairs * p.planes;
    const double vox = (double)N * D * H * W;
    {
        ProfScope ps(PF_WGRAD, 2.0 * vox * p.taps * Cin * Cout, 4.0 * (vox * (Cin + Cout) + (double)p.taps * Cin * Cout), st);
        if (k == 3) {
            if (p.BX == 32) launch_wgrad<32, 3>(a, nwg, st);
            else if (p.BX == 16) launch_wgrad<16, 3>(a, nwg, st);
            else launch_wgrad<8, 3>(a, nwg, st);
        } else {
            if (p.BX == 32) launch_wgrad<32, 5>(a, nwg, st);
            else if (p.BX == 16) launch_wgrad<16, 5>(a, nwg, st);
            else launch_wgrad<8, 5>(a, nwg, st);
        }
        SEG_CHECK_LAUNCH();
    }
    wgrad_reduce(part, dw, p.nstrips, p.taps, Cin, Cout, accumulate, st);
    SEG_CHECK_LAUNCH();
    return MI355SEG_OK;
}

}
```

### general-medical-image-segmentation-cnn-framework_amd/csrc/convt.hip

```cpp
#include "common.h"
#include "internal.h"

namespace seg {

__global__ void convt_pack_kernel(const float* __restrict__ w, float* __restrict__ wp, float* __restrict__ wd, int Cin, int Cout) {
    long long total = (long long)Cin * Cout * 8;
    for (long long i = (long long)blockIdx.x * blockDim.x + threadIdx.x; i < total; i += (long long)gridDim.x * blockDim.x) {
        int t = (int)(i % 8); long long r = i / 8;
        int co = (int)(r % Cout); int ci = (int)(r / Cout);
        float v = w[i];
        if (wp) wp[((long long)t * Cin + ci) * Cout + co] = v;
        if (wd) wd[((long long)t * Cout + co) * Cin + ci] = v;
    }
}

template <typename T>
__global__ __launch_bounds__(256) void convt_fwd_kernel(const T* __restrict__ x, int ldx, const float* __restrict__ wp,
        const float* __restrict__ bias, T* __restrict__ y, int ldy, int N, int D, int H, int W, int Cin, int Cout) {
    const int D2 = 2 * D, H2 = 2 * H, W2 = 2 * W;
    const long long total = (long long)N * D2 * H2 * W2 * Cout;
    for (long long i = (long long)blockIdx.x * blockDim.x + threadIdx.x; i < total; i += (long long)gridDim.x * blockDim.x) {
        int co = (int)(i % Cout); long long v = i / Cout;
        int ow = (int)(v % W2); long long r = v / W2;
        int oh = (int)(r % H2); r /= H2;
        int od = (int)(r % D2); int n = (int)(r / D2);
        int t = ((od & 1) << 2) | ((oh & 1) << 1) | (ow & 1);
        const T* xp = x + ((((long long)n * D + (od >> 1)) * H + (oh >> 1)) * W + (ow >> 1)) * ldx;
        const float* wq = wp + (long long)t * Cin * Cout + co;
        float acc = bias ? bias[co] : 0.f;
        int ci = 0;
        for (; ci + 4 <= Cin; ci += 4) {
            acc = fmaf(xp[ci], wq[(long long)ci * Cout], acc);
            acc = fmaf(xp[ci + 1], wq[(long long)(ci + 1) * Cout], acc);
            acc = fmaf(xp[ci + 2], wq[(long long)(ci + 2) * Cout], acc);
// ... 18 lines not shown
#pragma unroll
        for (int t = 0; t < 8; ++t) {
            const T* dp = dy + ((((long long)n * D2 + 2 * id + (t >> 2)) * H2 + 2 * ih + ((t >> 1) & 1)) * W2 + 2 * iw + (t & 1)) * lddy;
            const float* wq = wd + (long long)t * Cout * Cin + ci;
            for (int co = 0; co < Cout; ++co) acc = fmaf(dp[co], wq[(long long)co * Cin], acc);
        }
        dx[v * lddx + ci] = acc;
    }
}

template <typename T>
__global__ __launch_bounds__(256) void convt_wgrad_kernel(const T* __restrict__ dy, int lddy, const T* __restrict__ x, int ldx,
        float* __restrict__ part, int N, int D, int H, int W, int Cin, int Cout, long long vps) {
    const int pair = blockIdx.x * blockDim.x + threadIdx.x;
    const int t = blockIdx.y, split = blockIdx.z;
    const long long nvox = (long long)N * D * H * W;
    long long v0 = (long long)split * vps, v1 = v0 + vps;
    if (v1 > nvox) v1 = nvox;
    if (pair >= Cin * Cout) return;
    const int co = pair % Cout, ci = pair / Cout;
    const int H2 = 2 * H, W2 = 2 * W, D2 = 2 * D;
    float acc = 0.f;
    for (long long v = v0; v < v1; ++v) {
        int iw = (int)(v % W); long long r = v / W;
        int ih = (int)(r % H); r /= H;
        int id = (int)(r % D); int n = (int)(r / D);
        long long ov = (((long long)n * D2 + 2 * id + (t >> 2)) * H2 + 2 * ih + ((t >> 1) & 1)) * W2 + 2 * iw + (t & 1);
        acc = fmaf(x[v * ldx + ci], dy[ov * lddy + co], acc);
    }
    part[(((long long)split * 8 + t) * Cin + ci) * Cout + co] = acc;
}

__global__ __launch_bounds__(256) void convt_wgrad_reduce_kernel(const float* __restrict__ part, float* __restrict__ dw, int splits, int Cin, int Cout) {
    __shared__ float sh[8][32];
    const long long pairs = (long long)Cin * Cout, total = 8 * pairs;
    const int c = threadIdx.x & 31, q = threadIdx.x >> 5;
    const long long col = (long long)blockIdx.x * 32 + c;
    float s0 = 0.f, s1 = 0.f;
    if (col < total) {
        const float* p = part + col;
        int k = q;
        for (; k + 8 < splits; k += 16) { s0 += p[(long long)k * total]; s1 += p[(long long)(k + 8) * total]; }
        if (k < splits) s0 += p[(long long)k * total];
    }
    sh[q][c] = s0 + s1;
    __syncthreads();
    if (q == 0 && col < total) {
        float s = sh[0][c];
#pragma unroll
        for (int j = 1; j < 8; ++j) s += sh[j][c];
        const long long t = col / pairs, pr = col - t * pairs;
        dw[pr * 8 + t] = s;
    }
}

void convt_wgrad_reduce(const float* part, float* dw, int splits, int Cin, int Cout, hipStream_t st) {
    const long long b = ((long long)8 * Cin * Cout + 31) / 32;
    hipLaunchKernelGGL(convt_wgrad_reduce_kernel, dim3((unsigned)b), dim3(256), 0, st, part, dw, splits, Cin, Cout);
}

static int convt_splits(long long nvox, int Cin, int Cout) {
    int pairblocks = cdiv((long long)Cin * Cout, 256);
    long long want = 4096 / ((long long)pairblocks * 8) + 1;
    long long maxs = nvox / 64 + 1;
    if (want > maxs) want = maxs;
    if (want > 128) want = 128;
    return (int)(want < 1 ? 1 : want);
}
static int tgrid(long long total) {
    long long b = (total + 255) / 256;
    return (int)(b < 1 ? 1 : (b > 16384 ? 16384 : b));
}
}

using namespace seg;

extern "C" {


size_t mi355seg_convt3d_k2s2_ws_bytes(int N, int D, int H, int W, int Cin, int Cout) {
    size_t wb = align_up((size_t)8 * Cin * Cout * sizeof(float), 256);
    if (convt_direct_ws_bytes(Cin, Cout) > wb) wb = convt_direct_ws_bytes(Cin, Cout);
    size_t part = align_up((size_t)convt_splits((long long)N * D * H * W, Cin, Cout) * 8 * Cin * Cout * sizeof(float), 256);
    size_t red = colsum_ws_bytes(Cout);
    size_t pw = pw_wgrad_ws_bytes((long long)N * D * H * W, Cin, Cout, 8);
    if (pw > part) part = pw;
    const size_t lw = convt_wgrad_lowp_ws_bytes((long long)N * D * H * W, Cin, Cout);
    if (lw > part) part = lw;
    const size_t slab = convt_direct_slab_bytes((long long)N * D * H * W, Cin, Cout);
// ... 22 lines not shown
```

### general-medical-image-segmentation-cnn-framework_amd/csrc/convt_api.inc

```
#define CONVT_B16 (MI355SEG_PATH_B16_CONVT_FWD_DIRECT - MI355SEG_PATH_CONVT_FWD_DIRECT)
#define CONVT_NOTE(code) note_conv_path(sizeof(TT) == 4 ? (code) : (code) + CONVT_B16)
int FN(convt3d_k2s2_fwd)(const TT* x, int ldx, const float* w, const float* bias,
                                  TT* y, int ldy, int N, int D, int H, int W, int Cin, int Cout,
                                  void* ws, size_t ws_bytes, void* stream) {
    return FN(convt3d_k2s2_fwd_ax)(x, ldx, w, bias, y, ldy, N, D, H, W, Cin, Cout, nullptr, ws, ws_bytes, stream);
}
int FN(convt3d_k2s2_fwd_ax)(const TT* x, int ldx, const float* w, const float* bias,
                                  TT* y, int ldy, int N, int D, int H, int W, int Cin, int Cout, float* y_amax,
                                  void* ws, size_t ws_bytes, void* stream) {
    SEG_CHECK_ARG(x && w && y && N > 0 && D > 0 && H > 0 && W > 0 && Cin > 0 && Cout > 0 && ldx >= Cin && ldy >= Cout,
                  "convt3d_k2s2_fwd: bad arguments");
    SEG_CHECK_ARG(!(y_amax && sizeof(TT) != 4), "convt3d_k2s2_fwd_ax: y_amax is for fp32 tensors");
    hipStream_t st = (hipStream_t)stream;
    if ((sizeof(TT) == 2 || f32_conv_policy() == MATH_X3) && convt_direct_supported((int)sizeof(TT), false, N, D, H, W, Cin, Cout, ldx, ldy) &&
        ((uintptr_t)x % 16) == 0 && ((uintptr_t)y % 16) == 0 && ((uintptr_t)bias % 16) == 0) {
        CONVT_NOTE(MI355SEG_PATH_CONVT_FWD_DIRECT);
        return convt_direct<TT>(false, x, ldx, w, bias, y, ldy, N, D, H, W, Cin, Cout, ws, ws_bytes, st, y_amax);
    }
    struct AmaxAfter {
        const TT* y; int ldy; long long rows; int C; float* slot; hipStream_t st;
        ~AmaxAfter() { if constexpr (sizeof(TT) == 4) { if (slot) tensor_amax((const float*)y, ldy, rows, C, nullptr, slot, st); } }
    } after{y, ldy, (long long)N * 8 * D * H * W, Cout, y_amax, st};
    if (convt_mfma_supported(TT_MATH, N, D, H, W, Cin, Cout, ldx, ldy) && ((uintptr_t)x % 16) == 0) {
        CONVT_NOTE(MI355SEG_PATH_CONVT_FWD_MFMA);
// ... 16 lines not shown
                                    void* ws, size_t ws_bytes, void* stream) {
    SEG_CHECK_ARG(dy && w && dx && N > 0 && D > 0 && H > 0 && W > 0 && Cin > 0 && Cout > 0 && lddy >= Cout && lddx >= Cin,
                  "convt3d_k2s2_dgrad: bad arguments");
    hipStream_t st = (hipStream_t)stream;
    if ((sizeof(TT) == 2 || f32_conv_policy() == MATH_X3) && convt_direct_supported((int)sizeof(TT), true, N, D, H, W, Cin, Cout, lddx, lddy) &&
        ((uintptr_t)dy % 16) == 0 && ((uintptr_t)dx % 16) == 0) {
        CONVT_NOTE(MI355SEG_PATH_CONVT_DGRAD_DIRECT);
        return convt_direct<TT>(true, dy, lddy, w, nullptr, dx, lddx, N, D, H, W, Cin, Cout, ws, ws_bytes, st);
    }
    if (convt_mfma_supported(TT_MATH, N, D, H, W, Cin, Cout, lddx, lddy) && ((uintptr_t)dy % 16) == 0) {
        CONVT_NOTE(MI355SEG_PATH_CONVT_DGRAD_MFMA);
        return convt_dgrad_mfma(TT_MATH, dy, lddy, w, dx, lddx, N, D, H, W, Cin, Cout, ws, ws_bytes, st);
    }
    CONVT_NOTE(MI355SEG_PATH_CONVT_DGRAD_PLAIN);
    Carver cv(ws);
    float* wd = cv.take<float>((size_t)8 * Cin * Cout);
    SEG_CHECK_WS(cv.used(), ws_bytes);
    hipLaunchKernelGGL(convt_pack_kernel, dim3(tgrid((long long)8 * Cin * Cout)), dim3(256), 0, st, w, (float*)nullptr, wd, Cin, Cout);
    SEG_CHECK_LAUNCH();
    long long total = (long long)N * D * H * W * Cin;
    hipLaunchKernelGGL(convt_dgrad_kernel<TT>, dim3(tgrid(total)), dim3(256), 0, st, dy, lddy, wd, dx, lddx, N, D, H, W, Cin, Cout);
    SEG_CHECK_LAUNCH();
    return MI355SEG_OK;
}

int FN(convt3d_k2s2_wgrad)(const TT* dy, int lddy, const TT* x, int ldx,
                                    float* dw, float* db, int N, int D, int H, int W, int Cin, int Cout,
                                    void* ws, size_t ws_bytes, void* stream) {
    SEG_CHECK_ARG(dy && x && dw && N > 0 && D > 0 && H > 0 && W > 0 && Cin > 0 && Cout > 0 && lddy >= Cout && ldx >= Cin,
                  "convt3d_k2s2_wgrad: bad arguments");
    hipStream_t st = (hipStream_t)stream;
    const long long nvox = (long long)N * D * H * W;
    if (db) {
        int rc = channel_sums(dy, lddy, nvox * 8, Cout, nullptr, nullptr, db, 0, ws, ws_bytes, st);
        if (rc) return rc;
    }
    if ((sizeof(TT) == 2 || f32_conv_policy() == MATH_X3) && convt_wgrad_lowp_supported(nvox, Cin, Cout, ldx, lddy, (int)sizeof(TT)) &&
        ((uintptr_t)x % 16) == 0 && ((uintptr_t)dy % 16) == 0) {
        float* part; int nstrips;
        CONVT_NOTE(MI355SEG_PATH_CONVT_WGRAD_LOWP);
        int rc = convt_wgrad_lowp(dy, lddy, x, ldx, N, D, H, W, Cin, Cout, &part, &nstrips, ws, ws_bytes, st);
        if (rc) return rc;
        convt_wgrad_reduce(part, dw, nstrips, Cin, Cout, st);
        SEG_CHECK_LAUNCH();
        return MI355SEG_OK;
    }
    if (pw_wgrad_supported(nvox, Cin, Cout, 8, ldx, lddy) && ((uintptr_t)x % (4 * sizeof(TT))) == 0 && ((uintptr_t)dy % (4 * sizeof(TT))) == 0) {
        float* part; int nstrips;
        CONVT_NOTE(MI355SEG_PATH_CONVT_WGRAD_MFMA);
        int rc = pw_wgrad_mfma(dy, lddy, x, ldx, N, D, H, W, Cin, Cout, 8, &part, &nstrips, ws, ws_bytes, st);
        if (rc) return rc;
        convt_wgrad_reduce(part, dw, nstrips, Cin, Cout, st);
        SEG_CHECK_LAUNCH();
        return MI355SEG_OK;
    }
    CONVT_NOTE(MI355SEG_PATH_CONVT_WGRAD_PLAIN);
    const int splits = convt_splits(nvox, Cin, Cout);
    Carver cv(ws);
    float* part = cv.take<float>((size_t)splits * 8 * Cin * Cout);
    SEG_CHECK_WS(cv.used(), ws_bytes);
    long long vps = (nvox + splits - 1) / splits;
    dim3 grid(cdiv((long long)Cin * Cout, 256), 8, splits);
    hipLaunchKernelGGL(convt_wgrad_kernel<TT>, grid, dim3(256), 0, st, dy, lddy, x, ldx, part, N, D, H, W, Cin, Cout, vps);
    SEG_CHECK_LAUNCH();
    convt_wgrad_reduce(part, dw, splits, Cin, Cout, st);
    SEG_CHECK_LAUNCH();
    return MI355SEG_OK;
}

#undef CONVT_NOTE
#undef CONVT_B16
```

### general-medical-image-segmentation-cnn-framework_amd/csrc/convt_wgrad_lowp.hip

```cpp
#include "common.h"
#include "internal.h"
#include <type_traits>

namespace seg {

using f32x16 = __attribute__((ext_vector_type(16))) float;
using f32x4 = __attribute__((ext_vector_type(4))) float;
typedef short s16x4 __attribute__((ext_vector_type(4)));
typedef short s16x8 __attribute__((ext_vector_type(8)));
typedef __attribute__((address_space(3))) s16x4 lds_s16x4;

template <int NP>
struct CwCfg {
    static constexpr int V = NP == 3 ? 32 : 64;
    static constexpr int ROW = 64 * NP;
    static constexpr int X_BYTES = 2 * V * ROW, D_BYTES = 8 * V * ROW;
    static constexpr int LDS_BYTES = X_BYTES + D_BYTES;
    static constexpr int KSTEPS = V / 16;
};

struct CwArgs {
    const void* x; const void* dy; float* part;
    int ldx, lddy, N, D, H, W, Cin, Cout;
    int ntiles, nstrips, npairs, ncob;
};

__device__ __forceinline__ bf16x8_t cw_frag(const unsigned char* p, int row_bytes) {
    const s16x4 a = __builtin_amdgcn_ds_read_tr16_b64_v4i16((lds_s16x4*)p);
    const s16x4 b = __builtin_amdgcn_ds_read_tr16_b64_v4i16((lds_s16x4*)(p + 4 * row_bytes));
    return __builtin_bit_cast(bf16x8_t, (s16x8)__builtin_shufflevector(a, b, 0, 1, 2, 3, 4, 5, 6, 7));
}

template <int NP, typename IN_T>
__global__ __launch_bounds__(256, 2) void convt_wgrad_lowp_kernel(CwArgs a) {
// ... 350 lines not shown
    if (want > cap) want = (int)cap;
    if (want > p->ntiles) want = p->ntiles;
    if (want < 1) want = 1;
    p->nstrips = want;
    return true;
}

size_t convt_wgrad_lowp_ws_bytes(long long nvox, int Cin, int Cout) {
    size_t best = 0;
    for (int np : {1, 3}) {
        CwPlan p;
        if (!cw_plan(np, nvox, Cin, Cout, &p)) continue;
        const size_t b = align_up((size_t)p.nstrips * 8 * Cin * Cout * sizeof(float), 256) + 1024;
        if (b > best) best = b;
    }
    return best;
}

bool convt_wgrad_lowp_supported(long long nvox, int Cin, int Cout, int ldx, int lddy, int elem_bytes) {
    CwPlan p;
    const int al = 16 / elem_bytes;
    return (ldx % al) == 0 && (lddy % al) == 0 && cw_plan(elem_bytes == 4 ? 3 : 1, nvox, Cin, Cout, &p);
}

template <typename IN_T>
int convt_wgrad_lowp(const IN_T* dy, int lddy, const IN_T* x, int ldx, int N, int D, int H, int W, int Cin, int Cout,
                     float** part_out, int* nstrips_out, void* ws, size_t ws_bytes, hipStream_t st) {
    constexpr int NP = std::is_same<IN_T, float>::value ? 3 : 1;
    CwPlan p;
    const long long nvox = (long long)N * D * H * W;
    SEG_CHECK_ARG(cw_plan(NP, nvox, Cin, Cout, &p), "convt_wgrad_lowp: unsupported shape");
    SEG_CHECK_ARG(((uintptr_t)x % 16) == 0 && ((uintptr_t)dy % 16) == 0, "convt_wgrad_lowp: pointers must be 16-byte aligned");
    Carver cv(ws);
    float* part = cv.take<float>((size_t)p.nstrips * 8 * Cin * Cout);
    SEG_CHECK_WS(cv.used(), ws_bytes);
    CwArgs a{x, dy, part, ldx, lddy, N, D, H, W, Cin, Cout, p.ntiles, p.nstrips, p.npairs, (Cout + 31) / 32};
    SEG_SET_LDS((convt_wgrad_lowp_kernel<NP, IN_T>), CwCfg<NP>::LDS_BYTES);
    ProfScope ps(PF_CONVT, 2.0 * nvox * 8 * Cin * Cout, (double)sizeof(IN_T) * nvox * (Cin + 8.0 * Cout) + 32.0 * Cin * Cout, st);
    hipLaunchKernelGGL((convt_wgrad_lowp_kernel<NP, IN_T>), dim3(p.nstrips * p.npairs), dim3(256), CwCfg<NP>::LDS_BYTES, st, a);
    SEG_CHECK_LAUNCH();
    *part_out = part; *nstrips_out = p.nstrips;
    return MI355SEG_OK;
}
template int convt_wgrad_lowp<float>(const float*, int, const float*, int, int, int, int, int, int, int, float**, int*, void*, size_t, hipStream_t);
template int convt_wgrad_lowp<bf16>(const bf16*, int, const bf16*, int, int, int, int, int, int, int, float**, int*, void*, size_t, hipStream_t);

}
```

### general-medical-image-segmentation-cnn-framework_amd/csrc/internal.h

```cpp
#pragma once
#include "common.h"

namespace seg {

size_t colsum_ws_bytes(int C);
int channel_sums(const float* x, int ldx, long long rows, int C, double* sum, double* sq, float* fsum, int accumulate,
                 void* ws, size_t ws_bytes, hipStream_t st);
int channel_sums(const bf16* x, int ldx, long long rows, int C, double* sum, double* sq, float* fsum, int accumulate,
                 void* ws, size_t ws_bytes, hipStream_t st);

int finalize_channel_partials(const float* part, int nblk, int C, double* sum, double* sq, hipStream_t st);

bool stem_supported(int Cin, int Cout, int k, int stride, int pad, int ldy);
bool stem4_lowp_supported(int Cin, int Cout, int k, int stride, int pad, int ldx, int ldy);
size_t stem4_lowp_ws_bytes(int Cout);
int stem4_fwd_lowp(const bf16* x, const float* w, const float* bias, bf16* y, int ldy, int N, int D, int H, int W, int Cout,
                   void* ws, size_t ws_bytes, hipStream_t st);
int stem4_wgrad_lowp(const bf16* dy, int lddy, const bf16* x, float* dw, int N, int D, int H, int W, int Cout, int accumulate,
                     void* ws, size_t ws_bytes, hipStream_t st);
bool head_supported(int Cin, int Cout, int k, int stride, int pad, int ldx);
size_t small_ws_bytes(int Cin, int Cout, int k);
template <typename T> int stem_fwd(const T* x, int ldx, const float* w, const float* bias, T* y, int ldy, int N, int D, int H, int W, int Cin,
             int Cout, double* ssum, double* ssq, void* ws, size_t ws_bytes, hipStream_t st, float* y_amax = nullptr, bool* amax_done = nullptr);
bool stem_wgrad_bn_supported(int N, int D, int H, int W, int Cin, int Cout, int k, int stride, int pad);
int stem_wgrad_bn(const float* da, int ldda, const float* y, int ldy, const float* mean, const float* rstd, const float* gamma, const float* beta,
                  int act, float slope, const float* s1, const float* s2, const float* x, int ldx, float* dw, float* db,
                  int N, int D, int H, int W, int Cout, void* ws, size_t ws_bytes, hipStream_t st);
template <typename T> int stem_wgrad(const T* dy, int lddy, const T* x, int ldx, float* dw, int N, int D, int H, int W, int Cin, int Cout,
               int accumulate, void* ws, size_t ws_bytes, hipStream_t st);
template <typename T> int head_fwd(const T* x, int ldx, const float* w, const float* bias, T* y, int ldy, int N, int D, int H, int W, int Cin,
             int Cout, hipStream_t st);
template <typename T> int head_dgrad(const T* dy, int lddy, const float* w, T* dx, int lddx, int N, int D, int H, int W, int Cin, int Cout,
               hipStream_t st);
bool tinypw_supported(int Cin, int Cout, int k, int stride, int pad);
template <typename T> int tinypw_fwd(const T* x, int ldx, const float* w, const float* bias, T* y, int ldy, long long nvox, int Cin, int Cout, hipStream_t st);
template <typename T> int tinypw_dgrad(const T* dy, int lddy, const float* w, T* dx, int lddx, long long nvox, int Cin, int Cout, hipStream_t st);
template <typename T> int tinypw_wgrad(const T* dy, int lddy, const T* x, int ldx, float* dw, long long nvox, int Cin, int Cout, int accumulate, void* ws,
                                       size_t ws_bytes, hipStream_t st);
bool smallcin_wgrad_supported(int Cin, int Cout, int k);
bool smallcout_wgrad_supported(int Cin, int Cout, int k, int ldx);
size_t small_wgrad_ws_bytes(int Cin, int Cout, int k);
template <typename T> int smallcin_wgrad(const T* dy, int lddy, const T* x, int ldx, float* dw, int N, int D, int H, int W, int Cin, int Cout,
// ... 150 lines not shown
```

### general-medical-image-segmentation-cnn-framework_amd/csrc/norm.hip

```cpp
#include "common.h"
#include "internal.h"
#include <initializer_list>
#include <type_traits>

namespace seg {

constexpr int kRedThreads = 256;
constexpr int kMaxRedBlocks = 1024;

struct RedPlan {
    bool vec;
    int lanes;
    int rpi;
    int nblk;
};

static bool is_pow2(int v) { return v > 0 && (v & (v - 1)) == 0; }

static bool red_plan(long long rows, int C, int ld, RedPlan* p) {
    if (is_pow2(C) && C >= 4 && C <= 1024 && (ld % 4) == 0) {
        p->vec = true;
        p->lanes = C / 4;
    } else if (C <= kRedThreads) {
        p->vec = false;
        p->lanes = C;
    } else {
        return false;
    }
    p->rpi = kRedThreads / p->lanes;
    long long iters = (rows + p->rpi - 1) / p->rpi;
    long long nb = (iters + 7) / 8;
    p->nblk = (int)(nb < 1 ? 1 : (nb > kMaxRedBlocks ? kMaxRedBlocks : nb));
    return true;
}
// ... 562 lines not shown
    else
        act_host_dispatch(act, [&](auto A_) { hipLaunchKernelGGL((act_kernel<T, false, true, decltype(A_)::value>), grid, dim3(256), 0, st, dy, lddy, x,
                           ldx, res, ldres, dx, lddx, rows, C, rm.lanes, rm.rpi, act, slope, (const float*)nullptr, addend, ldadd); });
    SEG_CHECK_LAUNCH();
    return MI355SEG_OK;
}

template <typename T>
struct SumF {
    const T* x; int ldx; long long rows; int use_pivot;
    struct State { float p[4]; };
    __device__ __forceinline__ State prepC(int g, int c, int nj, int C) const {
        State s;
        for (int j = 0; j < 4; ++j) s.p[j] = (use_pivot && j < nj) ? stats_pivot(x, ldx, 0, rows, c + j) : 0.f;
        return s;
    }
    __device__ __forceinline__ void eval(const State& st, long long r, int g, int c, int C, float& a, float& b) const {
        float v = ld1(x + r * ldx + c) - st.p[0]; a = v; b = v * v;
    }
    __device__ __forceinline__ void eval4(const State& st, long long r, int g, int c, int C, float4& a, float4& b) const {
        float4 v = ldf4(x + r * ldx + c);
        v.x -= st.p[0]; v.y -= st.p[1]; v.z -= st.p[2]; v.w -= st.p[3];
        a = v; b = make_float4(v.x * v.x, v.y * v.y, v.z * v.z, v.w * v.w);
    }
};

template <> struct Combine64<SumF<bf16>> { static constexpr bool value = true; };

template <typename T>
__global__ __launch_bounds__(64) void sums_finalize_kernel(const float* __restrict__ part, int nblk, int C, double* __restrict__ sum,
                                     double* __restrict__ sq, float* __restrict__ fsum, int accumulate,
                                     const T* __restrict__ x, int ldx, long long rows, int use_pivot) {
    const int c = blockIdx.x;
    double a = 0.0, b = 0.0;
    for (int k = threadIdx.x; k < nblk; k += 64) {
        a += (double)part[((long long)k * C + c) * 2];
        b += (double)part[((long long)k * C + c) * 2 + 1];
    }
    a = wave_sum(a); b = wave_sum(b);
    if (threadIdx.x != 0) return;
    if (use_pivot) {
        const double pv = (double)stats_pivot(x, ldx, 0, rows, c), n = (double)rows;
        b = b + 2.0 * pv * a + n * pv * pv;
        a = a + n * pv;
    }
    if (sum) sum[c] = a;
    if (sq) sq[c] = b;
    if (fsum) fsum[c] = accumulate ? fsum[c] + (float)a : (float)a;
}

size_t colsum_ws_bytes(int C) { return align_up((size_t)kMaxRedBlocks * C * 2 * sizeof(float), 256); }

int finalize_channel_partials(const float* part, int nblk, int C, double* sum, double* sq, hipStream_t st) {
    hipLaunchKernelGGL(sums_finalize_kernel<float>, dim3(C), dim3(64), 0, st, part, nblk, C, sum, sq, (float*)nullptr, 0,
                       (const float*)nullptr, 0, 0LL, 0);
    SEG_CHECK_LAUNCH();
    return MI355SEG_OK;
}

template <typename T>
static int channel_sums_chunk(const T* x, int ldx, long long rows, int C, double* sum, double* sq, float* fsum, int accumulate,
                              void* ws, size_t ws_bytes, hipStream_t st) {
    SEG_CHECK_WS(colsum_ws_bytes(C), ws_bytes);
    float* part = (float*)ws;
    RedPlan p;
    const int use_pivot = sq != nullptr;
    SumF<T> f{x, ldx, rows, use_pivot};
    int rc = launch_colreduce2(f, rows, 1, C, ldx, part, &p, st);
    if (rc) return rc;
    hipLaunchKernelGGL(sums_finalize_kernel<T>, dim3(C), dim3(64), 0, st, part, p.nblk, C, sum, sq, fsum, accumulate, x, ldx, rows, use_pivot);
    SEG_CHECK_LAUNCH();
    return MI355SEG_OK;
}

template <typename T>
static int channel_sums_t(const T* x, int ldx, long long rows, int C, double* sum, double* sq, float* fsum, int accumulate,
                          void* ws, size_t ws_bytes, hipStream_t st) {
    int c0 = 0;
    while (c0 < C) {
        int rem = C - c0, take;
        if (rem >= 4 && (ldx % 4) == 0 && (c0 % 4) == 0 && ((uintptr_t)x % (4 * sizeof(T))) == 0) {
            take = 4;
            while (take * 2 <= rem && take * 2 <= 1024) take *= 2;
        } else {
            take = rem < 256 ? rem : 256;
        }
        int rc = channel_sums_chunk(x + c0, ldx, rows, take, sum ? sum + c0 : nullptr, sq ? sq + c0 : nullptr, fsum ? fsum + c0 : nullptr,
                                    accumulate, ws, ws_bytes, st);
        if (rc) return rc;
        c0 += take;
    }
    return MI355SEG_OK;
}
int channel_sums(const float* x, int ldx, long long rows, int C, double* sum, double* sq, float* fsum, int accumulate,
                 void* ws, size_t ws_bytes, hipStream_t st) {
    return channel_sums_t(x, ldx, rows, C, sum, sq, fsum, accumulate, ws, ws_bytes, st);
}
int channel_sums(const bf16* x, int ldx, long long rows, int C, double* sum, double* sq, float* fsum, int accumulate,
                 void* ws, size_t ws_bytes, hipStream_t st) {
    return channel_sums_t(x, ldx, rows, C, sum, sq, fsum, accumulate, ws, ws_bytes, st);
}

template <int NV, int MODE>
__global__ __launch_bounds__(256) void part_reduce_kernel(const float* __restrict__ part, int nblk, int C, int R, double* __restrict__ tmp) {
    constexpr int NO = MODE == 1 ? 2 : NV;
    __shared__ double sh[8][32][NO];
    const int cl = threadIdx.x & 31, q = threadIdx.x >> 5, c = blockIdx.x * 32 + cl, rb = blockIdx.y;
    const int rpb = (nblk + R - 1) / R, k0 = rb * rpb, k1 = min(nblk, k0 + rpb);
    double a[NO];
#pragma unroll
    for (int v = 0; v < NO; ++v) a[v] = 0.0;
    if (c < C)
        for (int k = k0 + q; k < k1; k += 8) {
            const float* p = part + ((long long)k * C + c) * NV;
            if (MODE == 1) {
                const double s = (double)p[0], n = (double)p[2];
                a[0] += s; a[1] += (double)p[1] + (n > 0.0 ? s * s / n : 0.0);
            } else {
#pragma unroll
                for (int v = 0; v < NV; ++v) a[v] += (double)p[v];
            }
        }
#pragma unroll
    for (int v = 0; v < NO; ++v) sh[q][cl][v] = a[v];
    __syncthreads();
    if (q == 0 && c < C) {
#pragma unroll
        for (int v = 0; v < NO; ++v) {
            double t = sh[0][cl][v];
#pragma unroll
            for (int j = 1; j < 8; ++j) t += sh[j][cl][v];
            tmp[((long long)rb * C + c) * NO + v] = t;
        }
// ... 154 lines not shown
```

### general-medical-image-segmentation-cnn-framework_amd/csrc/norm_api.inc

```



int FN(norm_stats)(const TT* x, int ldx, long long rows, int groups, int C, float eps,
                            float* mean, float* rstd, float* running_mean, float* running_var,
                            float momentum, void* ws, size_t ws_bytes, void* stream) {
    SEG_CHECK_ARG(x && mean && rstd && rows > 0 && groups > 0 && C > 0 && ldx >= C, "norm_stats: bad arguments");
    SEG_CHECK_ARG(!(running_mean && groups != 1), "norm_stats: running stats need groups == 1");
    SEG_CHECK_ARG((running_mean == nullptr) == (running_var == nullptr), "norm_stats: running_mean/var must come together");
    RedPlan p;
    SEG_CHECK_ARG(red_plan(rows, C, ldx, &p), "norm_stats: unsupported channel count C=%d", C);
    size_t need = (size_t)groups * p.nblk * C * 2 * sizeof(float);
    SEG_CHECK_WS(need, ws_bytes);
    float* part = (float*)ws;
    hipStream_t st = (hipStream_t)stream;
    StatsF<TT> f{x, ldx, rows};
    ProfScope ps(PF_NORM, 0.0, (double)sizeof(TT) * rows * groups * C, st);
    int rc = launch_colreduce2(f, rows, groups, C, ldx, part, &p, st);
    if (rc) return rc;
    hipLaunchKernelGGL(stats_finalize_kernel<TT>, dim3(groups * C), dim3(64), 0, st, part, p.nblk, C,
                       groups, (double)rows, eps, mean, rstd, running_mean, running_var, momentum, x, ldx);
    SEG_CHECK_LAUNCH();
    return MI355SEG_OK;
}

// ... 42 lines not shown
    int ldmin = 4;
    if ((lddy % 4) || (ldx % 4) || (res && (ldres % 4))) ldmin = 1;
    SEG_CHECK_ARG(red_plan(rows, C, ldmin, &p), "norm_act_bwd_sums: unsupported channel count C=%d", C);
    Carver cv(ws);
    float* part = cv.take<float>((size_t)groups * p.nblk * C * 2);
    SEG_CHECK_WS(cv.used(), ws_bytes);
    hipStream_t st = (hipStream_t)stream;
    int rc = MI355SEG_OK;
    {
        ProfScope ps(PF_NORM, 0.0, (double)sizeof(TT) * rows * groups * C * (res ? 3.0 : 2.0), st);
        act_host_dispatch(act, [&](auto A_) {
            BwdF<TT, decltype(A_)::value> f{dy, lddy, x, ldx, mean, rstd, gamma, beta, res, ldres, act, slope};
            rc = launch_colreduce2(f, rows, groups, C, ldmin, part, &p, st);
        });
    }
    if (rc) return rc;
    hipLaunchKernelGGL(bwd_finalize_kernel, dim3(groups * C), dim3(64), 0, st, part, p.nblk, C, groups, s1, s2, dgamma, dbeta);
    SEG_CHECK_LAUNCH();
    return MI355SEG_OK;
}

int FN(norm_act_bwd_apply_ax)(const TT* dy, int lddy, const TT* x, int ldx,
                           const float* mean, const float* rstd, const float* gamma, const float* beta, const TT* res, int ldres,
                           const float* s1, const float* s2, TT* dx, int lddx, TT* dres, int lddres, float* dx_colsum, float* dx_amax,
                           long long rows, int groups, int C, int act, float slope, void* ws, size_t ws_bytes, void* stream) {
    SEG_CHECK_ARG(dy && x && mean && rstd && s1 && s2 && dx && rows > 0 && groups > 0 && C > 0, "norm_act_bwd_apply: bad arguments");
    SEG_CHECK_ARG(!(dx_colsum && groups != 1), "norm_act_bwd_apply: dx column sums need groups == 1");
    bool v = vec_ok(C, {lddy, ldx, lddx, res ? ldres : 4, dres ? lddres : 4});
    RowMap rm = ew_map(C, v);
    int nrb = row_grid(rows, rm.rpi);
    if (dx_colsum && nrb > 1024) nrb = 1024;
    const bool fused_sum = dx_colsum && rm.lanes == (v ? C / 4 : C) && (256 % rm.lanes) == 0;
    Carver cv(ws);
    float* dxpart = fused_sum ? cv.take<float>((size_t)nrb * C * 2) : nullptr;
    SEG_CHECK_WS(cv.used(), ws_bytes);
    hipStream_t st = (hipStream_t)stream;
    dim3 grid(nrb, groups);
    unsigned* ao = reinterpret_cast<unsigned*>(dx_amax);
    {
        ProfScope ps(PF_NORM, 0.0, (double)sizeof(TT) * rows * groups * C * 3.0, st);
        if (v)
            act_host_dispatch(act, [&](auto A_) { hipLaunchKernelGGL((norm_act_bwd_apply_kernel<TT, true, decltype(A_)::value>), grid, dim3(256), 0, st, dy, lddy, x, ldx, mean,
                               rstd, gamma, beta, res, ldres, s1, s2, dx, lddx, dres, lddres, rows, C, rm.lanes, rm.rpi, act, slope, dxpart, ao); });
        else
            act_host_dispatch(act, [&](auto A_) { hipLaunchKernelGGL((norm_act_bwd_apply_kernel<TT, false, decltype(A_)::value>), grid, dim3(256), 0, st, dy, lddy, x, ldx, mean,
                               rstd, gamma, beta, res, ldres, s1, s2, dx, lddx, dres, lddres, rows, C, rm.lanes, rm.rpi, act, slope, dxpart, ao); });
        SEG_CHECK_LAUNCH();
    }
    if (dx_colsum) {
        if (fused_sum) {
            hipLaunchKernelGGL(sums_finalize_kernel<float>, dim3(C), dim3(64), 0, st, dxpart, nrb, C, (double*)nullptr, (double*)nullptr, dx_colsum, 0,
                               (const float*)nullptr, 0, 0LL, 0);
            SEG_CHECK_LAUNCH();
        } else {
            return channel_sums(dx, lddx, rows, C, nullptr, nullptr, dx_colsum, 0, ws, ws_bytes, st);
        }
    }
    return MI355SEG_OK;
}

int FN(norm_act_bwd_apply)(const TT* dy, int lddy, const TT* x, int ldx,
                           const float* mean, const float* rstd, const float* gamma, const float* beta, const TT* res, int ldres,
                           const float* s1, const float* s2, TT* dx, int lddx, TT* dres, int lddres, float* dx_colsum,
                           long long rows, int groups, int C, int act, float slope, void* ws, size_t ws_bytes, void* stream) {
    return FN(norm_act_bwd_apply_ax)(dy, lddy, x, ldx, mean, rstd, gamma, beta, res, ldres, s1, s2, dx, lddx, dres, lddres, dx_colsum, nullptr,
                                     rows, groups, C, act, slope, ws, ws_bytes, stream);
}

static int NORM_IMPL(const TT* dy, int lddy, const TT* x, int ldx,
                             const float* mean, const float* rstd, const float* gamma, const float* beta,
                             const TT* res, int ldres,
                             TT* dx, int lddx, float* dgamma, float* dbeta, TT* dres, int lddres, float* dx_colsum,
                             long long rows, int groups, int C, int act, float slope,
                             void* ws, size_t ws_bytes, void* stream, float* dx_amax = nullptr) {
    SEG_CHECK_ARG(dy && x && mean && rstd && dx && rows > 0 && groups > 0 && C > 0, "norm_act_bwd: bad arguments");
    SEG_CHECK_ARG(!(dgamma && groups != 1), "norm_act_bwd: affine grads need groups == 1");
    SEG_CHECK_ARG(!(dx_colsum && groups != 1), "norm_act_bwd: dx column sums need groups == 1");
    SEG_CHECK_ARG((dgamma == nullptr) == (dbeta == nullptr), "norm_act_bwd: dgamma/dbeta must come together");
    const size_t sb = align_up((size_t)groups * C * sizeof(float), 256);
    SEG_CHECK_WS(2 * sb + 256, ws_bytes);
    char* tail = (char*)ws + ((ws_bytes - 2 * sb) & ~(size_t)255);
    float* s1 = (float*)tail;
    float* s2 = (float*)(tail + sb);
    const size_t front = (size_t)(tail - (char*)ws);
    int rc = FN(norm_act_bwd_sums)(dy, lddy, x, ldx, mean, rstd, gamma, beta, res, ldres, s1, s2, dgamma, dbeta, rows, groups, C, act, slope,
                                   ws, front, stream);
    if (rc) return rc;
    return FN(norm_act_bwd_apply_ax)(dy, lddy, x, ldx, mean, rstd, gamma, beta, res, ldres, s1, s2, dx, lddx, dres, lddres, dx_colsum, dx_amax,
// ... 152 lines not shown
```

### general-medical-image-segmentation-cnn-framework_amd/distributed.py

```python
import os

import torch
import torch.distributed as dist


def init_from_env(backend=None):
    world = int(os.environ.get("WORLD_SIZE", "1"))
    rank = int(os.environ.get("RANK", "0"))
    local = int(os.environ.get("LOCAL_RANK", "0"))
    if world > 1 and not dist.is_initialized():
        os.environ.setdefault("MASTER_ADDR", "127.0.0.1")
        os.environ.setdefault("MASTER_PORT", "29500")
        if backend is None:
            backend = "nccl" if torch.cuda.is_available() else "gloo"
        if backend == "nccl":
            torch.cuda.set_device(local % max(1, torch.cuda.device_count()))
        dist.init_process_group(backend=backend, rank=rank, world_size=world)
    return rank, world, local


def self_launch(nproc, argv, env=None):
    import socket
    import subprocess
    import sys
# ... 112 lines not shown
                 "and in broadcast_buffers" if dev == "cuda" else "host clock (CPU / gloo rehearsal)",
    }


class GradAllReducer:

    def __init__(self, model, bucket_mb=32.0, overlap=True, always=False):
        self.params = [p for p in model.parameters() if p.requires_grad]
        self.always = always
        self.bucket_mb = bucket_mb
        self.timer, self.pack_timer, self.unpack_timer = CommTimer(), CommTimer(), CommTimer()
        cap = int(bucket_mb * (1 << 20) / 4)
        self.buckets, cur, n = [], [], 0
        for p in reversed(self.params):
            if cur and n + p.numel() > cap:
                self.buckets.append(cur)
                cur, n = [], 0
            cur.append(p)
            n += p.numel()
        if cur:
            self.buckets.append(cur)
        self._flat = [None] * len(self.buckets)
        self._pending = [len(b) for b in self.buckets]
        self._works = [None] * len(self.buckets)
        self._handles = []
        if overlap:
            for bi, bucket in enumerate(self.buckets):
                for p in bucket:
                    self._handles.append(p.register_post_accumulate_grad_hook(self._make_hook(bi)))

    def _active(self):
        return self.always or world_size() > 1

    def suspend_hooks(self, on=True):
        self._suspended = bool(on)
        if on:
            self._pending = [len(b) for b in self.buckets]

    def _make_hook(self, bi):
        def hook(_param):
            if not self._active() or getattr(self, "_suspended", False):
                return
            self._pending[bi] -= 1
            if self._pending[bi] == 0:
                self._launch(bi)
        return hook

    def _launch(self, bi):
        bucket = self.buckets[bi]
        grads = [p.grad if p.grad is not None else torch.zeros_like(p) for p in bucket]
        total = sum(g.numel() for g in grads)
        flat = self._flat[bi]
        if flat is None or flat.numel() != total or flat.device != grads[0].device:
            flat = torch.empty(total, dtype=grads[0].dtype, device=grads[0].device)
            self._flat[bi] = flat
        token = self.pack_timer.start(flat.device)
        torch.cat([g.reshape(-1) for g in grads], out=flat)
        self.pack_timer.stop(token)
        self._avg_in_collective = dist.get_backend() == "nccl"
        op = dist.ReduceOp.AVG if self._avg_in_collective else dist.ReduceOp.SUM
        self._works[bi] = dist.all_reduce(flat, op=op, async_op=True)

    def detach(self):
        for h in self._handles:
            h.remove()
        self._handles = []
# ... 124 lines not shown
```

### general-medical-image-segmentation-cnn-framework_amd/engine.py

```python
import torch

from . import functional as F
from .utils.metric import class_metrics_from_counts, metric_from_counts


def two_channel_gt(gt):
    return F.two_channel_gt(gt)


def mixed_precision_dtype(config=None):
    import os
    mode = None
    if config is not None:
        mode = config.get("mixed_precision") if hasattr(config, "get") else getattr(config, "mixed_precision", None)
    mode = str(mode if mode is not None else os.environ.get("ACCELERATE_MIXED_PRECISION", "no")).lower()
    if mode in ("no", "none", "false", "fp32", "f32", ""):
        return torch.float32
    if mode in ("bf16", "bfloat16"):
        return torch.bfloat16
    raise ValueError(f"mixed_precision must be 'no' or 'bf16', got {mode!r}")


def make_adam(params, lr, **kw):
    params = list(params)
    if "fused" not in kw and "foreach" not in kw and params and all(p.is_cuda and p.is_floating_point() for p in params):
        try:
            return torch.optim.Adam(params, lr=lr, fused=True, **kw)
        except (RuntimeError, TypeError, ValueError):
            pass
    return torch.optim.Adam(params, lr=lr, **kw)


def _forward(model, leaves, *args):
    if leaves is None:
        return model(*args)
    return torch.func.functional_call(model, leaves, args)


def _sync_metrics(out, multiclass):
    if multiclass:
        m = class_metrics_from_counts(out["class_counts"])
        out["class_dice"] = m["dice"]
        out["dice"] = m["mean_dice"]
        out["jaccard"] = m["mean_jaccard"]
    else:
        out["jaccard"], out["dice"] = metric_from_counts(out["counts"].cpu().tolist())


def train_step(model, optimizer, x, gt, criterion=None, sync_metric=True, grad_hook=None, dtype=None, step_optimizer=True, _leaves=None,
               multiclass=None, label_bad=None):
    optimizer.zero_grad(set_to_none=True)
    loss_terms = class_counts = None
    if multiclass is None:
        gt2 = two_channel_gt(gt)
    else:
        if isinstance(multiclass, bool) or not isinstance(multiclass, int) or not 2 <= multiclass <= F.MAX_LOSS_CLASSES:
            raise ValueError(f"train_step: multiclass must be the number of classes, an integer in 2..{F.MAX_LOSS_CLASSES}, got {multiclass!r}")
        if not hasattr(criterion, "tail_labels"):
            raise ValueError("train_step: multiclass needs a criterion with a tail_labels method (utils.loss_function.CompoundLoss; config.loss)")
        labels, label_bad = F.labels_u8(gt, multiclass, label_bad)
    x = x.to(torch.float32)
    bns = [m for m in model.modules()
           if isinstance(m, torch.nn.modules.batchnorm._BatchNorm) and m.training and m.num_batches_tracked is not None]
    F.dropout_pool_begin_step()
    with F.prepacked_weights(model, (str(dtype or F.compute_dtype()), F.conv_math_signature(), tuple(x.shape))) as pp:
        if (dtype or F.compute_dtype()) == torch.float32 and not pp.replaying:
            F.prefetch_weight_amax(model)
        try:
            with F.autocast(dtype or F.compute_dtype()), F.counters_batched(bns):
                if getattr(model, "takes_frequency_bands", False):
                    from .models.three_d.IS import frequency_bands
                    low_x, high_x = frequency_bands(x, impl=getattr(model, "band_split", "fft"))
                    pred, _ = _forward(model, _leaves, x, low_x, high_x)
                else:
                    pred = _forward(model, _leaves, x)
        finally:
            F.clear_weight_amax()
        F.flush_deferred_waits()
        if bns:
            torch._foreach_add_([m.num_batches_tracked for m in bns], 1)
        if multiclass is not None:
            if pred.shape[1] != multiclass:
                raise ValueError(f"train_step: multiclass={multiclass} but the model has {pred.shape[1]} output channels")
            loss, mask, counts, loss_terms, class_counts = criterion.tail_labels(pred, labels)
        elif criterion is None:
            loss, mask, counts = F.bce_argmax_dice(pred, gt2)
        elif hasattr(criterion, "tail"):
            loss, mask, counts, loss_terms = criterion.tail(pred, gt2)
        else:
            loss = criterion(pred, gt2)
            with torch.no_grad():
                mask = F.argmax_channels(pred)
                gt_lab = F.argmax_channels(gt2)
                counts = F.dice_counts(gt_lab, mask)
        loss.backward()
    if _leaves is not None:
        for name, p in model.named_parameters():
            p.grad = _leaves[name].grad
    if grad_hook is not None:
        grad_hook(model)
    if step_optimizer:
        optimizer.step()
    out = {"pred": pred, "mask": mask, "loss": loss.detach(), "counts": counts}
    if loss_terms is not None:
        out["loss_terms"] = loss_terms
    if class_counts is not None:
        out["class_counts"], out["label_bad"] = class_counts, label_bad
    if sync_metric:
        _sync_metrics(out, multiclass)
    return out


class GraphedTrainStep:

    def __init__(self, model, optimizer, x, gt, criterion=None, warmup=3, dtype=None, grad_hook=None, multiclass=None):
        from ._lib import lib
        if not all(g.get("capturable", False) for g in optimizer.param_groups):
            raise ValueError("GraphedTrainStep: build the optimizer with capturable=True (e.g. torch.optim.Adam(..., capturable=True))")
        lib().call("mi355seg_prof_enable", 0)
        self.model, self.optimizer, self.criterion, self.grad_hook = model, optimizer, criterion, grad_hook
        self.x = x.detach().to(torch.float32).clone()
        self.gt = gt.detach().clone()
        self.multiclass = multiclass
        self.label_bad = torch.zeros(1, dtype=torch.int64, device=self.x.device) if multiclass is not None else None
        mc = {"multiclass": multiclass, "label_bad": self.label_bad} if multiclass is not None else {}
        if grad_hook is not None and hasattr(grad_hook, "suspend_hooks"):
            grad_hook.suspend_hooks(True)
        side = torch.cuda.Stream()
        side.wait_stream(torch.cuda.current_stream())
        with torch.cuda.stream(side):
            self.first = None
            for _ in range(warmup):
                o = train_step(model, optimizer, self.x, self.gt, criterion, sync_metric=False, dtype=dtype, grad_hook=grad_hook, **mc)
                self.first = {"loss": o["loss"].detach().clone(), "counts": o["counts"].clone()}
                if "loss_terms" in o:
                    self.first["loss_terms"] = o["loss_terms"].clone()
                if "class_counts" in o:
                    self.first["class_counts"] = o["class_counts"].clone()
                del o
        torch.cuda.current_stream().wait_stream(side)
        torch.cuda.synchronize()
        self.graph = torch.cuda.CUDAGraph()
        self.opt_graph = None
        F.amax_pool_reset()
        leaves = {name: p.detach().requires_grad_(p.requires_grad) for name, p in model.named_parameters()}
        if grad_hook is None:
            with torch.cuda.graph(self.graph):
                self.out = train_step(model, optimizer, self.x, self.gt, criterion, sync_metric=False, dtype=dtype, _leaves=leaves, **mc)
        else:
            with torch.cuda.graph(self.graph):
                self.out = train_step(model, optimizer, self.x, self.gt, criterion, sync_metric=False, dtype=dtype, step_optimizer=False, _leaves=leaves, **mc)
            for p in model.parameters():
                if p.requires_grad and p.grad is None:
                    p.grad = torch.zeros_like(p)
            self.opt_graph = torch.cuda.CUDAGraph()
            with torch.cuda.graph(self.opt_graph, pool=self.graph.pool()):
                optimizer.step()
        F.amax_pool_reset()
        self._prepack_arenas = [rec.get("arena") for rec in F.prepack_plans(model).values()]

    def __call__(self, x, gt, sync_metric=True):
        self.x.copy_(x, non_blocking=True)
        self.gt.copy_(gt, non_blocking=True)
        F.flush_deferred_waits()
        self.graph.replay()
        if self.opt_graph is not None:
            self.grad_hook(self.model)
            self.opt_graph.replay()
        out = dict(self.out)
        if sync_metric:
            _sync_metrics(out, self.multiclass)
        return out


def weights_init_normal(init_type):
    from torch.nn import init

    def init_func(m):
        name = type(m).__name__
        if "BatchNorm2d" in name:
            if getattr(m, "weight", None) is not None:
                init.normal_(m.weight.data, 1.0, 0.02)
            if getattr(m, "bias", None) is not None:
                init.constant_(m.bias.data, 0.0)
            return
        if not (hasattr(m, "weight") and ("Conv" in name or "Linear" in name)):
            return
        table = {
            "normal": lambda w: init.normal_(w, 0.0, 0.02),
            "xavier": lambda w: init.xavier_normal_(w, gain=0.02),
            "xavier_uniform": lambda w: init.xavier_uniform_(w, gain=1.0),
            "kaiming": lambda w: init.kaiming_normal_(w, a=0, mode="fan_in"),
# ... 13 lines not shown
```

### general-medical-image-segmentation-cnn-framework_amd/functional.py

```python
import collections
import ctypes
import os
import threading
import weakref

import numpy as np
import torch
from torch.autograd import Function

from ._lib import lib, Mi355SegError

ACT_NONE, ACT_RELU, ACT_ELU, ACT_LRELU, ACT_SIGMOID = 0, 1, 2, 3, 4

_WS = {}

class _AutocastState(threading.local):

    def __init__(self):
        self.stack = [torch.float32]


_AUTOCAST = _AutocastState()
_SFX = {torch.float32: "f32", torch.bfloat16: "bf16"}

# ... 133 lines not shown
        L = lib()
        if rec is None:
            if torch.cuda.is_current_stream_capturing():
                return self
            if len(plans) >= 4:
                old = next(iter(plans))
                L.call("mi355seg_prepack_free", plans.pop(old)["plan"])
            L.call("mi355seg_prepack_record_begin")
            self.mode, self.sig, self.plans = "record", sig, plans
        elif rec["plan"]:
            L.call("mi355seg_prepack_run", rec["plan"], _p(rec["arena"]), rec["arena"].numel(), _stream())
            self.mode = "run"
            prepacked_weights.active = L.query("mi355seg_prepack_active") != 0
        return self

    def __exit__(self, *exc):
        L = lib()
        mode, self.mode = self.mode, None
        if mode == "record":
            n = len(self.params)
            base = (ctypes.c_void_p * n)(*[p.data_ptr() for p in self.params])
            size = (ctypes.c_size_t * n)(*[p.numel() * p.element_size() for p in self.params])
            plan, nbytes = ctypes.c_int(0), ctypes.c_size_t(0)
            L.call("mi355seg_prepack_record_end", ctypes.byref(plan), ctypes.byref(nbytes), base, size, n)
            if exc[0] is not None:
                if plan.value:
                    L.call("mi355seg_prepack_free", plan.value)
            else:
                arena = torch.empty(max(int(nbytes.value), 256), dtype=torch.uint8, device=self.params[0].device) if plan.value else None
                self.plans[self.sig] = {"plan": plan.value, "arena": arena}
        elif mode == "run":
            prepacked_weights.active = False
            L.call("mi355seg_prepack_done", _stream())
        return False


def _require_cuda(t, what, allow_bf16=False):
    if not t.is_cuda:
        raise Mi355SegError(f"{what}: expected a tensor on an MI355X (cuda/HIP) device, got {t.device}; "
                            "there is no CPU fallback in this package")
    if t.dtype != torch.float32 and not (allow_bf16 and t.dtype == torch.bfloat16):
        raise Mi355SegError(f"{what}: expected float32{' or bfloat16' if allow_bf16 else ''}, got {t.dtype}")


def aligned_contiguous(t):
    t = t.contiguous()
    if t.data_ptr() % 16:
        t = t.clone(memory_format=torch.contiguous_format)
    return t


def cl_view(t, what="tensor", allow_bf16=True):
    _require_cuda(t, what, allow_bf16=allow_bf16)
    if t.dim() != 5:
        raise Mi355SegError(f"{what}: expected 5-D [N,D,H,W,C], got shape {tuple(t.shape)}")
    N, D, H, W, C = t.shape
    s = t.stride()
    ld = s[3]
    ok = (C == 1 or s[4] == 1) and ld >= C and W > 1
    ok = ok and (H == 1 or s[2] == W * ld) and (D == 1 or s[1] == H * W * ld) and (N == 1 or s[0] == D * H * W * ld)
    ok = ok and t.data_ptr() % 16 == 0
    if not ok:
        t = aligned_contiguous(t)
        ld = C
    return t, ld

# ... 3165 lines not shown
```

### include/mi355seg.h

```cpp
#ifndef MI355SEG_H
#define MI355SEG_H

#include <stddef.h>
#include <stdint.h>

#ifdef __cplusplus
extern "C" {
#endif

#if defined(__HIP__) || defined(__HIPCC__)
typedef __bf16 mi355seg_bf16;
#else
typedef uint16_t mi355seg_bf16;
#endif

#define MI355SEG_OK 0
#define MI355SEG_EINVAL (-1)
#define MI355SEG_EWORKSPACE (-2)
#define MI355SEG_EHIP (-3)

#define MI355SEG_ACT_NONE 0
#define MI355SEG_ACT_RELU 1
#define MI355SEG_ACT_ELU 2
#define MI355SEG_ACT_LRELU 3
// ... 590 lines not shown
int mi355seg_maxpool2_fwd_bf16(const mi355seg_bf16* x, int ldx, mi355seg_bf16* y, int ldy, uint8_t* idx, int N, int D, int H, int W, int C, void* stream);
int mi355seg_maxpool2_bwd_bf16(const mi355seg_bf16* dy, int lddy, const uint8_t* idx, mi355seg_bf16* dx, int lddx, int N, int D, int H, int W, int C, void* stream);
int mi355seg_maxpool2_bwd_add_bf16(const mi355seg_bf16* dy, int lddy, const uint8_t* idx, const mi355seg_bf16* add, int ldadd, mi355seg_bf16* dx, int lddx, int N, int D, int H, int W, int C, void* stream);
int mi355seg_upsample2_fwd_bf16(const mi355seg_bf16* x, int ldx, mi355seg_bf16* y, int ldy, int N, int D, int H, int W, int C, void* stream);
int mi355seg_upsample2_bwd_bf16(const mi355seg_bf16* dy, int lddy, mi355seg_bf16* dx, int lddx, int N, int D, int H, int W, int C, void* stream);
int mi355seg_convt3d_k2s2_fwd_ax_bf16(const mi355seg_bf16* x, int ldx, const float* w, const float* bias, mi355seg_bf16* y, int ldy, int N, int D, int H, int W, int Cin, int Cout, float* y_amax, void* ws, size_t ws_bytes, void* stream);
int mi355seg_convt3d_k2s2_fwd_bf16(const mi355seg_bf16* x, int ldx, const float* w, const float* bias, mi355seg_bf16* y, int ldy, int N, int D, int H, int W, int Cin, int Cout, void* ws, size_t ws_bytes, void* stream);
int mi355seg_convt3d_k2s2_dgrad_bf16(const mi355seg_bf16* dy, int lddy, const float* w, mi355seg_bf16* dx, int lddx, int N, int D, int H, int W, int Cin, int Cout, void* ws, size_t ws_bytes, void* stream);
int mi355seg_convt3d_k2s2_wgrad_bf16(const mi355seg_bf16* dy, int lddy, const mi355seg_bf16* x, int ldx, float* dw, float* db, int N, int D, int H, int W, int Cin, int Cout, void* ws, size_t ws_bytes, void* stream);
int mi355seg_ncdhw_f32_to_ndhwc_bf16(const float* src, mi355seg_bf16* dst, int lddst, long long N, int C, long long S, void* stream);
int mi355seg_ndhwc_bf16_to_ncdhw_f32(const mi355seg_bf16* src, int ldsrc, float* dst, long long N, int C, long long S, void* stream);
int mi355seg_copy_rows_bf16(const mi355seg_bf16* src, int ldsrc, mi355seg_bf16* dst, int lddst, long long rows, int C, void* stream);
int mi355seg_add_rows_bf16(const mi355seg_bf16* src, int ldsrc, mi355seg_bf16* dst, int lddst, long long rows, int C, void* stream);
int mi355seg_repeat_channels_bf16(const mi355seg_bf16* x, int ldx, mi355seg_bf16* y, int ldy, long long rows, int C, int rep, void* stream);
int mi355seg_repeat_channels_bwd_bf16(const mi355seg_bf16* dy, int lddy, mi355seg_bf16* dx, int lddx, long long rows, int C, int rep, void* stream);
int mi355seg_add_bias_bf16(mi355seg_bf16* y, int ldy, const float* bias, long long rows, int C, void* stream);
size_t mi355seg_conv3d_ws_bytes_bf16(int N, int D, int H, int W, int Cin, int Cout, int k, int stride, int pad);
int mi355seg_conv3d_fwd_bf16(const mi355seg_bf16* x, int ldx, const float* w, const float* bias, mi355seg_bf16* y, int ldy, int N, int D, int H, int W, int Cin, int Cout, int k, int stride, int pad, double* stats_sum, double* stats_sq, void* ws, size_t ws_bytes, void* stream);
int mi355seg_conv3d_fwd_res_bf16(const mi355seg_bf16* x, int ldx, const float* w, const float* bias, const mi355seg_bf16* res, int ldres, mi355seg_bf16* y, int ldy, int N, int D, int H, int W, int Cin, int Cout, int k, int stride, int pad, void* ws, size_t ws_bytes, void* stream);
int mi355seg_conv3d_dgrad_bf16(const mi355seg_bf16* dy, int lddy, const float* w, mi355seg_bf16* dx, int lddx, int N, int D, int H, int W, int Cin, int Cout, int k, int stride, int pad, void* ws, size_t ws_bytes, void* stream);
int mi355seg_conv3d_dgrad_res_bf16(const mi355seg_bf16* dy, int lddy, const float* w, const mi355seg_bf16* res, int ldres, mi355seg_bf16* dx, int lddx, int N, int D, int H, int W, int Cin, int Cout, int k, int stride, int pad, void* ws, size_t ws_bytes, void* stream);
int mi355seg_conv3d_wgrad_bf16(const mi355seg_bf16* dy, int lddy, const mi355seg_bf16* x, int ldx, float* dw, float* db, int N, int D, int H, int W, int Cin, int Cout, int k, int stride, int pad, int accumulate, void* ws, size_t ws_bytes, void* stream);
int mi355seg_cast_f32_to_bf16(const float* src, int ldsrc, mi355seg_bf16* dst, int lddst, long long rows, int C, void* stream);
int mi355seg_cast_bf16_to_f32(const mi355seg_bf16* src, int ldsrc, float* dst, int lddst, long long rows, int C, void* stream);

int mi355seg_prepack_record_begin(void);
int mi355seg_prepack_record_end(int* plan, size_t* arena_bytes, const void* const* param_base_host, const size_t* param_bytes_host, int nparams);
int mi355seg_prepack_jobs(int plan);
int mi355seg_prepack_run(int plan, void* arena, size_t arena_bytes, void* stream);
int mi355seg_prepack_done(void* stream);
int mi355seg_prepack_active(void);
int mi355seg_prepack_free(int plan);

#ifdef __cplusplus
}
#endif
#endif
```

Measured before the change: 221.0 million voxels/s.

## Defer parameter-gradient reduction kernels into one batched flush after backward

Adds a deferral mechanism. Per-layer partial-sum slabs for weight, bias and BN parameter gradients are redirected into a persistent arena, and the many small finalize/reduce launches are recorded as jobs instead of run inline. A single flush after loss.backward runs them together. The goal is to remove many tiny kernel launches and their serialization during backward. In exchange it adds arena memory, a measure pass on the first step, and falls back when gradients are read inside backward (e.g. DDP hooks) or when the arena exceeds its size cap.

```diff
diff --git a/general-medical-image-segmentation-cnn-framework_amd/csrc/bn_head.hip b/general-medical-image-segmentation-cnn-framework_amd/csrc/bn_head.hip
--- a/general-medical-image-segmentation-cnn-framework_amd/csrc/bn_head.hip
+++ b/general-medical-image-segmentation-cnn-framework_amd/csrc/bn_head.hip
@@ -1,5 +1,6 @@
 #include "common.h"
 #include "internal.h"
+#include "grad_flush.h"
 
 namespace seg {
 
@@ -170,16 +171,7 @@
 __global__ __launch_bounds__(64) void bh_finalize_kernel(const float* __restrict__ part, int nblk, int ncol, float* __restrict__ o0, int n0,
                                                         float* __restrict__ o1, int n1, float* __restrict__ o2, int n2, float* __restrict__ o3,
                                                         float* __restrict__ alias0, float* __restrict__ alias1) {
-    const int j = blockIdx.x;
-    double s = 0.0;
-    for (int b = threadIdx.x; b < nblk; b += 64) s += (double)part[(long long)b * ncol + j];
-    s = wave_sum(s);
-    if (threadIdx.x != 0) return;
-    const float v = (float)s;
-    if (j < n0) { o0[j] = v; if (alias0) alias0[j] = v; }
-    else if (j < n0 + n1) { o1[j - n0] = v; if (alias1) alias1[j - n0] = v; }
-    else if (j < n0 + n1 + n2) { if (o2) o2[j - n0 - n1] = v; }
-    else if (o3) o3[j - n0 - n1 - n2] = v;
+    bh_finalize_body((int)blockIdx.x, part, nblk, ncol, o0, n0, o1, n1, o2, n2, o3, alias0, alias1);
 }
 
 template <int K, int ACT>
@@ -465,15 +457,16 @@
     hipStream_t st = (hipStream_t)stream;
     const int grid = bh_grid(rows, 256 / (C / 4)) * 2;
     if (dy_colsum) SEG_CHECK_WS((size_t)grid * C * sizeof(float), ws_bytes);
-    BhArgs a{y, ldy, mean, rstd, gamma, beta, wh, nullptr, dlogits, lddl, dy, lddy, s1, s2, dy_colsum ? (float*)ws : nullptr,
+    float* cpart = dy_colsum ? grad_slab((float*)ws, (size_t)grid * C, st) : nullptr;
+    BhArgs a{y, ldy, mean, rstd, gamma, beta, wh, nullptr, dlogits, lddl, dy, lddy, s1, s2, cpart,
              (unsigned*)dy_amax, rows, C, act, slope};
     {
         ProfScope ps(PF_NORM, 2.0 * rows * C * K, 4.0 * rows * (2.0 * C + K), st);
         BH_DISPATCH(bn_head_bwd_apply_kernel, K, grid, st, a);
         SEG_CHECK_LAUNCH();
     }
-    if (dy_colsum) {
-        hipLaunchKernelGGL(bh_finalize_kernel, dim3(C), dim3(64), 0, st, (const float*)ws, grid, C, dy_colsum, C, (float*)nullptr, 0, (float*)nullptr, 0,
+    if (dy_colsum && !grad_defer(GradJob{cpart, dy_colsum, GJ_BH, 0, 0, 0, {grid, C, 0, 0, 0, 0}}, st)) {
+        hipLaunchKernelGGL(bh_finalize_kernel, dim3(C), dim3(64), 0, st, (const float*)cpart, grid, C, dy_colsum, C, (float*)nullptr, 0, (float*)nullptr, 0,
                            (float*)nullptr, (float*)nullptr, (float*)nullptr);
         SEG_CHECK_LAUNCH();
     }
@@ -530,14 +523,15 @@
     }
     hipLaunchKernelGGL(bh_finalize_kernel, dim3(2 * C), dim3(64), 0, st, (const float*)ws, grid, 2 * C, s1, C, s2, C, (float*)nullptr, 0, (float*)nullptr, dbeta, dgamma);
     SEG_CHECK_LAUNCH();
-    b.s1 = s1; b.s2 = s2; b.amax = (unsigned*)dy_amax; b.part = dy_colsum ? (float*)ws : nullptr;
+    float* cpart = dy_colsum ? grad_slab((float*)ws, (size_t)grid * C, st) : nullptr;
+    b.s1 = s1; b.s2 = s2; b.amax = (unsigned*)dy_amax; b.part = cpart;
     {
         ProfScope ps(PF_NORM, 0.0, 4.0 * npool * C * (24.0 + 1.25), st);
         hipLaunchKernelGGL(bn_pool_bwd_kernel<true>, dim3(grid), dim3(256), 0, st, b);
         SEG_CHECK_LAUNCH();
     }
-    if (dy_colsum) {
-        hipLaunchKernelGGL(bh_finalize_kernel, dim3(C), dim3(64), 0, st, (const float*)ws, grid, C, dy_colsum, C, (float*)nullptr, 0, (float*)nullptr, 0,
+    if (dy_colsum && !grad_defer(GradJob{cpart, dy_colsum, GJ_BH, 0, 0, 0, {grid, C, 0, 0, 0, 0}}, st)) {
+        hipLaunchKernelGGL(bh_finalize_kernel, dim3(C), dim3(64), 0, st, (const float*)cpart, grid, C, dy_colsum, C, (float*)nullptr, 0, (float*)nullptr, 0,
                            (float*)nullptr, (float*)nullptr, (float*)nullptr);
         SEG_CHECK_LAUNCH();
     }
diff --git a/general-medical-image-segmentation-cnn-framework_amd/csrc/conv_generic.hip b/general-medical-image-segmentation-cnn-framework_amd/csrc/conv_generic.hip
--- a/general-medical-image-segmentation-cnn-framework_amd/csrc/conv_generic.hip
+++ b/general-medical-image-segmentation-cnn-framework_amd/csrc/conv_generic.hip
@@ -1,5 +1,6 @@
 #include "common.h"
 #include "internal.h"
+#include "grad_flush.h"
 #include <string.h>
 #include <stdlib.h>
 
@@ -146,45 +147,7 @@
 __global__ __launch_bounds__(256) void wgrad_reduce_kernel(const float* __restrict__ part, float* __restrict__ dw, int splits, int T, int Cin,
                                                            int Cout, int accumulate, int CIT, int TT) {
     extern __shared__ float tr[];
-    const long long total = (long long)T * Cin * Cout;
-    const int co0 = blockIdx.x * 32, ci0 = blockIdx.y * CIT, t0 = blockIdx.z * TT;
-    const int tn = min(TT, T - t0);
-    const int run = CIT * TT, pitch = run + 1;
-    for (int e0 = threadIdx.x; e0 < 32 * run; e0 += 1024) {
-        long long idx[4]; int dst[4]; bool ok[4];
-        double s[4] = {0.0, 0.0, 0.0, 0.0};
-#pragma unroll
-        for (int u = 0; u < 4; ++u) {
-            const int e = e0 + 256 * u;
-            const int col = e & 31, r = e >> 5;
-            const int cil = r % CIT, tl = r / CIT;
-            const int co = co0 + col, ci = ci0 + cil;
-            ok[u] = e < 32 * run && co < Cout && ci < Cin && tl < tn;
-            idx[u] = ok[u] ? ((long long)(t0 + tl) * Cin + ci) * Cout + co : 0;
-            dst[u] = e < 32 * run ? col * pitch + cil * TT + tl : -1;
-        }
-        for (int k = 0; k < splits; ++k) {
-            float v[4];
-#pragma unroll
-            for (int u = 0; u < 4; ++u) v[u] = part[(long long)k * total + idx[u]];
-#pragma unroll
-            for (int u = 0; u < 4; ++u) if (ok[u]) s[u] += (double)v[u];
-        }
-#pragma unroll
-        for (int u = 0; u < 4; ++u) if (dst[u] >= 0) tr[dst[u]] = (float)s[u];
-    }
-    __syncthreads();
-    const int cin_here = min(CIT, Cin - ci0);
-    for (int e = threadIdx.x; e < 32 * run; e += 256) {
-        const int col = e / run, j = e - col * run;
-        const int cil = j / TT, tl = j - cil * TT;
-        const int co = co0 + col;
-        if (co < Cout && cil < cin_here && tl < tn) {
-            const long long o = ((long long)co * Cin + ci0 + cil) * T + t0 + tl;
-            const float v = tr[col * pitch + j];
-            dw[o] = accumulate ? dw[o] + v : v;
-        }
-    }
+    wgrad_reduce_body(tr, (int)blockIdx.x, (int)blockIdx.y, (int)blockIdx.z, part, dw, splits, T, Cin, Cout, accumulate, CIT, TT);
 }
 
 __global__ void wgrad_reduce_flat_kernel(const float* __restrict__ part, float* __restrict__ dw, int splits, int T, int Cin,
@@ -212,57 +175,15 @@
 
 __global__ __launch_bounds__(256) void wgrad_reduce_cols_kernel(const float* __restrict__ part, float* __restrict__ dw, int splits, int T, int Cin,
                                                                 int Cout, int accumulate) {
-    __shared__ double sh[8][32];
-    const long long total = (long long)T * Cin * Cout;
-    const int c = threadIdx.x & 31, q = threadIdx.x >> 5;
-    const long long col = (long long)blockIdx.x * 32 + c;
-    double s0 = 0.0, s1 = 0.0;
-    if (col < total) {
-        const float* p = part + col;
-        int k = q;
-        for (; k + 8 < splits; k += 16) { s0 += (double)p[(long long)k * total]; s1 += (double)p[(long long)(k + 8) * total]; }
-        if (k < splits) s0 += (double)p[(long long)k * total];
-    }
-    sh[q][c] = s0 + s1;
-    __syncthreads();
-    if (q == 0 && col < total) {
-        double s = sh[0][c];
-#pragma unroll
-        for (int j = 1; j < 8; ++j) s += sh[j][c];
-        const int co = (int)(col % Cout); const long long r = col / Cout;
-        const int ci = (int)(r % Cin), t = (int)(r / Cin);
-        const long long o = ((long long)co * Cin + ci) * T + t;
-        dw[o] = accumulate ? dw[o] + (float)s : (float)s;
-    }
-}
-
+    wgrad_reduce_cols_body<false>((int)blockIdx.x, part, dw, splits, T, Cin, Cout, accumulate);
+}
 __global__ __launch_bounds__(256) void wgrad_reduce_cols_swapped_kernel(const float* __restrict__ part, float* __restrict__ dw, int splits, int T, int Cin,
                                                                         int Cout, int accumulate) {
-    __shared__ double sh[8][32];
-    const long long total = (long long)T * Cin * Cout;
-    const int c = threadIdx.x & 31, q = threadIdx.x >> 5;
-    const long long col = (long long)blockIdx.x * 32 + c;
-    double s0 = 0.0, s1 = 0.0;
-    if (col < total) {
-        const float* p = part + col;
-        int k = q;
-        for (; k + 8 < splits; k += 16) { s0 += (double)p[(long long)k * total]; s1 += (double)p[(long long)(k + 8) * total]; }
-        if (k < splits) s0 += (double)p[(long long)k * total];
-    }
-    sh[q][c] = s0 + s1;
-    __syncthreads();
-    if (q == 0 && col < total) {
-        double s = sh[0][c];
-#pragma unroll
-        for (int j = 1; j < 8; ++j) s += sh[j][c];
-        const int ci = (int)(col % Cin); const long long r = col / Cin;
-        const int co = (int)(r % Cout), tp = (int)(r / Cout);
-        const long long o = ((long long)co * Cin + ci) * T + (T - 1 - tp);
-        dw[o] = accumulate ? dw[o] + (float)s : (float)s;
-    }
+    wgrad_reduce_cols_body<true>((int)blockIdx.x, part, dw, splits, T, Cin, Cout, accumulate);
 }
 void wgrad_reduce_swapped(const float* part, float* dw, int splits, int T, int Cin, int Cout, int accumulate, hipStream_t st) {
     const long long total = (long long)T * Cin * Cout;
+    if (grad_defer(GradJob{part, dw, GJ_COLS_SWAPPED, accumulate, 0, 0, {splits, T, Cin, Cout, 0, 0}}, st)) return;
     hipLaunchKernelGGL(wgrad_reduce_cols_swapped_kernel, dim3((unsigned)((total + 31) / 32)), dim3(256), 0, st, part, dw, splits, T, Cin, Cout, accumulate);
 }
 
@@ -274,6 +195,7 @@
     auto blocks = [&](int cit) { return (long long)((Cout + 31) / 32) * ((Cin + cit - 1) / cit) * ((T + TT - 1) / TT); };
     if (splits >= 8) {
         const long long total = (long long)T * Cin * Cout;
+        if (grad_defer(GradJob{part, dw, GJ_COLS, accumulate, 0, 0, {splits, T, Cin, Cout, 0, 0}}, st)) return;
         hipLaunchKernelGGL(wgrad_reduce_cols_kernel, dim3((unsigned)((total + 31) / 32)), dim3(256), 0, st, part, dw, splits, T, Cin, Cout, accumulate);
         return;
     }
@@ -281,9 +203,11 @@
     if (blocks(CIT) < 256) {
         long long total = (long long)T * Cin * Cout;
         int grid = (int)((total + 255) / 256 > 4096 ? 4096 : (total + 255) / 256);
+        grad_defer(GradJob{part, dw, GJ_NONE, accumulate, 0, 0, {}}, st);
         hipLaunchKernelGGL(wgrad_reduce_flat_kernel, dim3(grid), dim3(256), 0, st, part, dw, splits, T, Cin, Cout, accumulate);
         return;
     }
+    if (grad_defer(GradJob{part, dw, GJ_WGRAD, accumulate, 0, 0, {splits, T, Cin, Cout, CIT, TT}}, st)) return;
     const size_t lds = (size_t)32 * (CIT * TT + 1) * sizeof(float);
     hipLaunchKernelGGL(wgrad_reduce_kernel, dim3((Cout + 31) / 32, (Cin + CIT - 1) / CIT, (T + TT - 1) / TT), dim3(256), lds, st, part, dw,
                        splits, T, Cin, Cout, accumulate, CIT, TT);
@@ -359,7 +283,7 @@
     const int T = g.k * g.k * g.k;
     const int splits = generic_splits(g);
     Carver cv(ws);
-    float* part = cv.take<float>((size_t)splits * T * g.Cin * g.Cout);
+    float* part = grad_slab(cv.take<float>((size_t)splits * T * g.Cin * g.Cout), (size_t)splits * T * g.Cin * g.Cout, st);
     SEG_CHECK_WS(cv.used(), ws_bytes);
     const long long nvox = (long long)g.N * g.Do * g.Ho * g.Wo;
     long long vps = (nvox + splits - 1) / splits;
diff --git a/general-medical-image-segmentation-cnn-framework_amd/csrc/conv_gwgrad.hip b/general-medical-image-segmentation-cnn-framework_amd/csrc/conv_gwgrad.hip
--- a/general-medical-image-segmentation-cnn-framework_amd/csrc/conv_gwgrad.hip
+++ b/general-medical-image-segmentation-cnn-framework_amd/csrc/conv_gwgrad.hip
@@ -1,5 +1,6 @@
 #include "common.h"
 #include "internal.h"
+#include "grad_flush.h"
 
 namespace seg {
 
@@ -151,7 +152,7 @@
     SEG_CHECK_ARG(gw_plan(N, Do, Ho, Wo, Cin, Cout, k, &p), "conv_gwgrad: unsupported shape");
     SEG_CHECK_ARG(((uintptr_t)x % (4 * sizeof(IN_T))) == 0 && ((uintptr_t)dy % (4 * sizeof(IN_T))) == 0, "conv_gwgrad: pointers must be aligned to four elements");
     Carver cv(ws);
-    float* part = cv.take<float>((size_t)p.nstrips * p.T * Cin * Cout);
+    float* part = grad_slab(cv.take<float>((size_t)p.nstrips * p.T * Cin * Cout), (size_t)p.nstrips * p.T * Cin * Cout, st);
     SEG_CHECK_WS(cv.used(), ws_bytes);
     GwArgs a{x, dy, part, ldx, lddy, N, D, H, W, Do, Ho, Wo, Cin, Cout, k, stride, pad, p.T,
              p.ntiles, p.nstrips, p.npairs, (Cout + 31) / 32, p.ngroups};
diff --git a/general-medical-image-segmentation-cnn-framework_amd/csrc/conv_small.hip b/general-medical-image-segmentation-cnn-framework_amd/csrc/conv_small.hip
--- a/general-medical-image-segmentation-cnn-framework_amd/csrc/conv_small.hip
+++ b/general-medical-image-segmentation-cnn-framework_amd/csrc/conv_small.hip
@@ -1,5 +1,6 @@
 #include "common.h"
 #include "internal.h"
+#include "grad_flush.h"
 
 namespace seg {
 
@@ -428,11 +429,7 @@
 }
 
 __global__ __launch_bounds__(64) void colpart_finalize_kernel(const float* __restrict__ cpart, int nblk, int C, float* __restrict__ out) {
-    const int c = blockIdx.x;
-    double s = 0.0;
-    for (int k = threadIdx.x; k < nblk; k += 64) s += (double)cpart[(long long)k * C + c];
-    s = wave_sum(s);
-    if (threadIdx.x == 0) out[c] = (float)s;
+    colpart_finalize_body((int)blockIdx.x, cpart, nblk, C, out);
 }
 
 template <typename T>
@@ -579,8 +576,9 @@
     const int ntiles = (int)(nvox / ((long long)S1_TZ * S1_TY * (256 / (Cout / 4))));
     const int nb = ntiles < 512 ? ntiles : 512;
     Carver cv(ws);
-    float* part = cv.take<float>((size_t)nb * 27 * Cout);
+    float* part = grad_slab(cv.take<float>((size_t)nb * 27 * Cout), (size_t)nb * 27 * Cout, st);
     float* cpart = cv.take<float>((size_t)nb * Cout);
+    if (db) cpart = grad_slab(cpart, (size_t)nb * Cout, st);
     SEG_CHECK_WS(cv.used(), ws_bytes);
     StemBn b{da, ldda, y, ldy, mean, rstd, gamma, beta, s1, s2, act, slope, 1.f / (float)nvox};
     const size_t lds = ((size_t)stem_bn_scratch_floats(Cout) + 6 * Cout) * 4 + (size_t)S1_TZ * S1_TY * 256 * 16;
@@ -591,7 +589,7 @@
     }
     wgrad_reduce(part, dw, nb, 27, 1, Cout, 0, st);
     SEG_CHECK_LAUNCH();
-    if (db) {
+    if (db && !grad_defer(GradJob{cpart, db, GJ_COLPART, 0, 0, 0, {nb, Cout, 0, 0, 0, 0}}, st)) {
         hipLaunchKernelGGL(colpart_finalize_kernel, dim3(Cout), dim3(64), 0, st, cpart, nb, Cout, db);
         SEG_CHECK_LAUNCH();
     }
@@ -851,7 +849,7 @@
     int nblk = small_grid(nvox, 256 / lpv);
     if (nblk > 512) nblk = 512;
     SEG_CHECK_WS((size_t)nblk * g.T * Cin * Cout * sizeof(float), ws_bytes);
-    float* part = (float*)ws;
+    float* part = grad_slab((float*)ws, (size_t)nblk * g.T * Cin * Cout, st);
     const int TPG = 25;
     dim3 grid(nblk, Cin, (g.T + TPG - 1) / TPG);
     size_t lds = (size_t)4 * TPG * Cout * 4;
@@ -875,7 +873,7 @@
     int nblk = small_grid(nvox, 256 / (Cin / 4));
     if (nblk > 512) nblk = 512;
     SEG_CHECK_WS((size_t)nblk * g.T * Cin * Cout * sizeof(float), ws_bytes);
-    float* part = (float*)ws;
+    float* part = grad_slab((float*)ws, (size_t)nblk * g.T * Cin * Cout, st);
     {
         ProfScope ps(PF_DIRECT, 2.0 * nvox * g.T * Cin * Cout, (double)sizeof(T) * nvox * (Cin + Cout), st);
         if (Cout == 2) {
@@ -965,7 +963,7 @@
     int nblk = small_grid(nvox, vpb);
     if (nblk > 512) nblk = 512;
     SEG_CHECK_WS((size_t)nblk * 27 * Cin * Cout * sizeof(float), ws_bytes);
-    float* part = (float*)ws;
+    float* part = grad_slab((float*)ws, (size_t)nblk * 27 * Cin * Cout, st);
     size_t lds = (size_t)4 * 27 * Cout * 4;
     if (stem1_tiled_ok(g)) {
         const int ntiles = (int)(nvox / ((long long)S1_TZ * S1_TY * (256 / (Cout / 4))));
@@ -1030,7 +1028,7 @@
     int nblk = small_grid(nvox, 256 / (Cin / 4));
     if (nblk > 512) nblk = 512;
     SEG_CHECK_WS((size_t)nblk * Cin * Cout * sizeof(float), ws_bytes);
-    float* part = (float*)ws;
+    float* part = grad_slab((float*)ws, (size_t)nblk * Cin * Cout, st);
     {
         ProfScope ps(PF_DIRECT, 2.0 * nvox * Cin * Cout, (double)sizeof(T) * nvox * (Cin + Cout), st);
         if (Cout == 2) hipLaunchKernelGGL((head_wgrad_kernel<T, 2>), dim3(nblk), dim3(256), 0, st, x, dy, lddy, part, g);
@@ -1066,7 +1064,7 @@
     int nblk = small_grid(nvox, 256);
     if (nblk > 512) nblk = 512;
     SEG_CHECK_WS((size_t)nblk * Cin * Cout * sizeof(float), ws_bytes);
-    float* part = (float*)ws;
+    float* part = grad_slab((float*)ws, (size_t)nblk * Cin * Cout, st);
     {
         ProfScope ps(PF_DIRECT, 2.0 * nvox * Cin * Cout, (double)sizeof(T) * nvox * (Cin + Cout), st);
         hipLaunchKernelGGL((tinypw_wgrad_kernel<T>), dim3(nblk), dim3(256), 0, st, x, dy, part, g);
diff --git a/general-medical-image-segmentation-cnn-framework_amd/csrc/conv_wgrad_lowp.hip b/general-medical-image-segmentation-cnn-framework_amd/csrc/conv_wgrad_lowp.hip
--- a/general-medical-image-segmentation-cnn-framework_amd/csrc/conv_wgrad_lowp.hip
+++ b/general-medical-image-segmentation-cnn-framework_amd/csrc/conv_wgrad_lowp.hip
@@ -1,5 +1,6 @@
 #include "common.h"
 #include "internal.h"
+#include "grad_flush.h"
 #include <initializer_list>
 #include <type_traits>
 #include <stdlib.h>
@@ -777,7 +778,7 @@
     if (swap) {
         SEG_CHECK_ARG(((uintptr_t)x % 16) == 0 && ((uintptr_t)dy % 16) == 0, "conv_wgrad_lowp: pointers must be 16-byte aligned");
         Carver cv(ws);
-        float* part = cv.take<float>((size_t)psw.nstrips * psw.taps * Cin * Cout);
+        float* part = grad_slab(cv.take<float>((size_t)psw.nstrips * psw.taps * Cin * Cout), (size_t)psw.nstrips * psw.taps * Cin * Cout, st);
         float* amax = cv.take<float>(2);
         SEG_CHECK_WS(cv.used(), ws_bytes);
         LWgradArgs a{dy, x, part, lddy, ldx, N, D, H, W, Cout, Cin, Do, Ho, Wo, psw.ntx, psw.nty, psw.ntz, psw.ntiles, psw.nstrips, psw.npairs, Cin / psw.cob, psw.taps,
@@ -807,7 +808,7 @@
     SEG_CHECK_ARG(((uintptr_t)x % 16) == 0 && ((uintptr_t)dy % 16) == 0, "conv_wgrad_lowp: pointers must be 16-byte aligned");
     SEG_CHECK_ARG(lw_offsets_fit(math, H, W, ldx, Ho, Wo, lddy), "conv_wgrad_lowp: a tile's halo spans more than 2 GB (wgrad_lowp_supported says so)");
     Carver cv(ws);
-    float* part = cv.take<float>((size_t)p.nstrips * p.taps * Cin * Cout);
+    float* part = grad_slab(cv.take<float>((size_t)p.nstrips * p.taps * Cin * Cout), (size_t)p.nstrips * p.taps * Cin * Cout, st);
     const bool f16 = math == MATH_X3 && x3_f16();
     float* amax = f16 ? cv.take<float>(2) : nullptr;
     SEG_CHECK_WS(cv.used(), ws_bytes);
diff --git a/general-medical-image-segmentation-cnn-framework_amd/csrc/conv_wgrad_mfma.hip b/general-medical-image-segmentation-cnn-framework_amd/csrc/conv_wgrad_mfma.hip
--- a/general-medical-image-segmentation-cnn-framework_amd/csrc/conv_wgrad_mfma.hip
+++ b/general-medical-image-segmentation-cnn-framework_amd/csrc/conv_wgrad_mfma.hip
@@ -1,5 +1,6 @@
 #include "common.h"
 #include "internal.h"
+#include "grad_flush.h"
 #include <initializer_list>
 
 namespace seg {
@@ -214,7 +215,7 @@
     SEG_CHECK_ARG(wgrad_plan(k, N, D, H, W, Cin, Cout, &p), "conv_wgrad_mfma: unsupported shape");
     SEG_CHECK_ARG(((uintptr_t)x % 16) == 0 && ((uintptr_t)dy % 16) == 0, "conv_wgrad_mfma: pointers must be 16-byte aligned");
     Carver cv(ws);
-    float* part = cv.take<float>((size_t)p.nstrips * p.taps * Cin * Cout);
+    float* part = grad_slab(cv.take<float>((size_t)p.nstrips * p.taps * Cin * Cout), (size_t)p.nstrips * p.taps * Cin * Cout, st);
     SEG_CHECK_WS(cv.used(), ws_bytes);
     WgradArgs a{x, dy, part, ldx, lddy, N, D, H, W, Cin, Cout, p.ntx, p.nty, p.ntz, p.ntiles, p.nstrips, p.npairs, Cout / 32, p.taps};
     const int nwg = p.nstrips * p.npairs * p.planes;
diff --git a/general-medical-image-segmentation-cnn-framework_amd/csrc/convt.hip b/general-medical-image-segmentation-cnn-framework_amd/csrc/convt.hip
--- a/general-medical-image-segmentation-cnn-framework_amd/csrc/convt.hip
+++ b/general-medical-image-segmentation-cnn-framework_amd/csrc/convt.hip
@@ -1,5 +1,6 @@
 #include "common.h"
 #include "internal.h"
+#include "grad_flush.h"
 
 namespace seg {
 
@@ -84,29 +85,11 @@
 }
 
 __global__ __launch_bounds__(256) void convt_wgrad_reduce_kernel(const float* __restrict__ part, float* __restrict__ dw, int splits, int Cin, int Cout) {
-    __shared__ float sh[8][32];
-    const long long pairs = (long long)Cin * Cout, total = 8 * pairs;
-    const int c = threadIdx.x & 31, q = threadIdx.x >> 5;
-    const long long col = (long long)blockIdx.x * 32 + c;
-    float s0 = 0.f, s1 = 0.f;
-    if (col < total) {
-        const float* p = part + col;
-        int k = q;
-        for (; k + 8 < splits; k += 16) { s0 += p[(long long)k * total]; s1 += p[(long long)(k + 8) * total]; }
-        if (k < splits) s0 += p[(long long)k * total];
-    }
-    sh[q][c] = s0 + s1;
-    __syncthreads();
-    if (q == 0 && col < total) {
-        float s = sh[0][c];
-#pragma unroll
-        for (int j = 1; j < 8; ++j) s += sh[j][c];
-        const long long t = col / pairs, pr = col - t * pairs;
-        dw[pr * 8 + t] = s;
-    }
+    convt_wgrad_reduce_body((int)blockIdx.x, part, dw, splits, Cin, Cout);
 }
 
 void convt_wgrad_reduce(const float* part, float* dw, int splits, int Cin, int Cout, hipStream_t st) {
+    if (grad_defer(GradJob{part, dw, GJ_CONVT, 0, 0, 0, {splits, Cin, Cout, 0, 0, 0}}, st)) return;
     const long long b = ((long long)8 * Cin * Cout + 31) / 32;
     hipLaunchKernelGGL(convt_wgrad_reduce_kernel, dim3((unsigned)b), dim3(256), 0, st, part, dw, splits, Cin, Cout);
 }
diff --git a/general-medical-image-segmentation-cnn-framework_amd/csrc/convt_api.inc b/general-medical-image-segmentation-cnn-framework_amd/csrc/convt_api.inc
--- a/general-medical-image-segmentation-cnn-framework_amd/csrc/convt_api.inc
+++ b/general-medical-image-segmentation-cnn-framework_amd/csrc/convt_api.inc
@@ -72,7 +72,7 @@
     hipStream_t st = (hipStream_t)stream;
     const long long nvox = (long long)N * D * H * W;
     if (db) {
-        int rc = channel_sums(dy, lddy, nvox * 8, Cout, nullptr, nullptr, db, 0, ws, ws_bytes, st);
+        int rc = channel_sums(dy, lddy, nvox * 8, Cout, nullptr, nullptr, db, 0, ws, ws_bytes, st, true);
         if (rc) return rc;
     }
     if ((sizeof(TT) == 2 || f32_conv_policy() == MATH_X3) && convt_wgrad_lowp_supported(nvox, Cin, Cout, ldx, lddy, (int)sizeof(TT)) &&
@@ -97,7 +97,7 @@
     CONVT_NOTE(MI355SEG_PATH_CONVT_WGRAD_PLAIN);
     const int splits = convt_splits(nvox, Cin, Cout);
     Carver cv(ws);
-    float* part = cv.take<float>((size_t)splits * 8 * Cin * Cout);
+    float* part = grad_slab(cv.take<float>((size_t)splits * 8 * Cin * Cout), (size_t)splits * 8 * Cin * Cout, st);
     SEG_CHECK_WS(cv.used(), ws_bytes);
     long long vps = (nvox + splits - 1) / splits;
     dim3 grid(cdiv((long long)Cin * Cout, 256), 8, splits);
diff --git a/general-medical-image-segmentation-cnn-framework_amd/csrc/convt_wgrad_lowp.hip b/general-medical-image-segmentation-cnn-framework_amd/csrc/convt_wgrad_lowp.hip
--- a/general-medical-image-segmentation-cnn-framework_amd/csrc/convt_wgrad_lowp.hip
+++ b/general-medical-image-segmentation-cnn-framework_amd/csrc/convt_wgrad_lowp.hip
@@ -1,5 +1,6 @@
 #include "common.h"
 #include "internal.h"
+#include "grad_flush.h"
 #include <type_traits>
 
 namespace seg {
@@ -416,7 +417,7 @@
     SEG_CHECK_ARG(cw_plan(NP, nvox, Cin, Cout, &p), "convt_wgrad_lowp: unsupported shape");
     SEG_CHECK_ARG(((uintptr_t)x % 16) == 0 && ((uintptr_t)dy % 16) == 0, "convt_wgrad_lowp: pointers must be 16-byte aligned");
     Carver cv(ws);
-    float* part = cv.take<float>((size_t)p.nstrips * 8 * Cin * Cout);
+    float* part = grad_slab(cv.take<float>((size_t)p.nstrips * 8 * Cin * Cout), (size_t)p.nstrips * 8 * Cin * Cout, st);
     SEG_CHECK_WS(cv.used(), ws_bytes);
     CwArgs a{x, dy, part, ldx, lddy, N, D, H, W, Cin, Cout, p.ntiles, p.nstrips, p.npairs, (Cout + 31) / 32};
     SEG_SET_LDS((convt_wgrad_lowp_kernel<NP, IN_T>), CwCfg<NP>::LDS_BYTES);
diff --git a/general-medical-image-segmentation-cnn-framework_amd/csrc/grad_flush.h b/general-medical-image-segmentation-cnn-framework_amd/csrc/grad_flush.h
--- /dev/null
+++ b/general-medical-image-segmentation-cnn-framework_amd/csrc/grad_flush.h
@@ -0,0 +1,161 @@
+#pragma once
+#include "common.h"
+
+namespace seg {
+
+__device__ __forceinline__ void wgrad_reduce_body(float* tr, const int bx, const int by, const int bz, const float* __restrict__ part, float* __restrict__ dw,
+                                                  int splits, int T, int Cin, int Cout, int accumulate, int CIT, int TT) {
+    const long long total = (long long)T * Cin * Cout;
+    const int co0 = bx * 32, ci0 = by * CIT, t0 = bz * TT;
+    const int tn = min(TT, T - t0);
+    const int run = CIT * TT, pitch = run + 1;
+    for (int e0 = threadIdx.x; e0 < 32 * run; e0 += 1024) {
+        long long idx[4]; int dst[4]; bool ok[4];
+        double s[4] = {0.0, 0.0, 0.0, 0.0};
+#pragma unroll
+        for (int u = 0; u < 4; ++u) {
+            const int e = e0 + 256 * u;
+            const int col = e & 31, r = e >> 5;
+            const int cil = r % CIT, tl = r / CIT;
+            const int co = co0 + col, ci = ci0 + cil;
+            ok[u] = e < 32 * run && co < Cout && ci < Cin && tl < tn;
+            idx[u] = ok[u] ? ((long long)(t0 + tl) * Cin + ci) * Cout + co : 0;
+            dst[u] = e < 32 * run ? col * pitch + cil * TT + tl : -1;
+        }
+        for (int k = 0; k < splits; ++k) {
+            float v[4];
+#pragma unroll
+            for (int u = 0; u < 4; ++u) v[u] = part[(long long)k * total + idx[u]];
+#pragma unroll
+            for (int u = 0; u < 4; ++u) if (ok[u]) s[u] += (double)v[u];
+        }
+#pragma unroll
+        for (int u = 0; u < 4; ++u) if (dst[u] >= 0) tr[dst[u]] = (float)s[u];
+    }
+    __syncthreads();
+    const int cin_here = min(CIT, Cin - ci0);
+    for (int e = threadIdx.x; e < 32 * run; e += 256) {
+        const int col = e / run, j = e - col * run;
+        const int cil = j / TT, tl = j - cil * TT;
+        const int co = co0 + col;
+        if (co < Cout && cil < cin_here && tl < tn) {
+            const long long o = ((long long)co * Cin + ci0 + cil) * T + t0 + tl;
+            const float v = tr[col * pitch + j];
+            dw[o] = accumulate ? dw[o] + v : v;
+        }
+    }
+}
+
+template <bool SWAPPED>
+__device__ __forceinline__ void wgrad_reduce_cols_body(const int vb, const float* __restrict__ part, float* __restrict__ dw, int splits, int T, int Cin, int Cout,
+                                                       int accumulate) {
+    __shared__ double sh[8][32];
+    const long long total = (long long)T * Cin * Cout;
+    const int c = threadIdx.x & 31, q = threadIdx.x >> 5;
+    const long long col = (long long)vb * 32 + c;
+    double s0 = 0.0, s1 = 0.0;
+    if (col < total) {
+        const float* p = part + col;
+        int k = q;
+        for (; k + 8 < splits; k += 16) { s0 += (double)p[(long long)k * total]; s1 += (double)p[(long long)(k + 8) * total]; }
+        if (k < splits) s0 += (double)p[(long long)k * total];
+    }
+    sh[q][c] = s0 + s1;
+    __syncthreads();
+    if (q == 0 && col < total) {
+        double s = sh[0][c];
+#pragma unroll
+        for (int j = 1; j < 8; ++j) s += sh[j][c];
+        long long o;
+        if (SWAPPED) {
+            const int ci = (int)(col % Cin); const long long r = col / Cin;
+            const int co = (int)(r % Cout), tp = (int)(r / Cout);
+            o = ((long long)co * Cin + ci) * T + (T - 1 - tp);
+        } else {
+            const int co = (int)(col % Cout); const long long r = col / Cout;
+            const int ci = (int)(r % Cin), t = (int)(r / Cin);
+            o = ((long long)co * Cin + ci) * T + t;
+        }
+        dw[o] = accumulate ? dw[o] + (float)s : (float)s;
+    }
+}
+
+__device__ __forceinline__ void convt_wgrad_reduce_body(const int vb, const float* __restrict__ part, float* __restrict__ dw, int splits, int Cin, int Cout) {
+    __shared__ float sh[8][32];
+    const long long pairs = (long long)Cin * Cout, total = 8 * pairs;
+    const int c = threadIdx.x & 31, q = threadIdx.x >> 5;
+    const long long col = (long long)vb * 32 + c;
+    float s0 = 0.f, s1 = 0.f;
+    if (col < total) {
+        const float* p = part + col;
+        int k = q;
+        for (; k + 8 < splits; k += 16) { s0 += p[(long long)k * total]; s1 += p[(long long)(k + 8) * total]; }
+        if (k < splits) s0 += p[(long long)k * total];
+    }
+    sh[q][c] = s0 + s1;
+    __syncthreads();
+    if (q == 0 && col < total) {
+        float s = sh[0][c];
+#pragma unroll
+        for (int j = 1; j < 8; ++j) s += sh[j][c];
+        const long long t = col / pairs, pr = col - t * pairs;
+        dw[pr * 8 + t] = s;
+    }
+}
+
+__device__ __forceinline__ void sums_finalize_reduce(const int c, const float* __restrict__ part, int nblk, int C, double& a, double& b) {
+    a = 0.0; b = 0.0;
+    for (int k = threadIdx.x; k < nblk; k += 64) {
+        a += (double)part[((long long)k * C + c) * 2];
+        b += (double)part[((long long)k * C + c) * 2 + 1];
+    }
+    a = wave_sum(a); b = wave_sum(b);
+}
+__device__ __forceinline__ void sums_finalize_store(const int c, double a, double b, double* __restrict__ sum, double* __restrict__ sq,
+                                                    float* __restrict__ fsum, int accumulate) {
+    if (sum) sum[c] = a;
+    if (sq) sq[c] = b;
+    if (fsum) fsum[c] = accumulate ? fsum[c] + (float)a : (float)a;
+}
+
+__device__ __forceinline__ void colpart_finalize_body(const int c, const float* __restrict__ cpart, int nblk, int C, float* __restrict__ out) {
+    double s = 0.0;
+    for (int k = threadIdx.x; k < nblk; k += 64) s += (double)cpart[(long long)k * C + c];
+    s = wave_sum(s);
+    if (threadIdx.x == 0) out[c] = (float)s;
+}
+
+__device__ __forceinline__ void bh_finalize_body(const int j, const float* __restrict__ part, int nblk, int ncol, float* __restrict__ o0, int n0,
+                                                 float* __restrict__ o1, int n1, float* __restrict__ o2, int n2, float* __restrict__ o3,
+                                                 float* __restrict__ alias0, float* __restrict__ alias1) {
+    double s = 0.0;
+    for (int b = threadIdx.x; b < nblk; b += 64) s += (double)part[(long long)b * ncol + j];
+    s = wave_sum(s);
+    if (threadIdx.x != 0) return;
+    const float v = (float)s;
+    if (j < n0) { o0[j] = v; if (alias0) alias0[j] = v; }
+    else if (j < n0 + n1) { o1[j - n0] = v; if (alias1) alias1[j - n0] = v; }
+    else if (j < n0 + n1 + n2) { if (o2) o2[j - n0 - n1] = v; }
+    else if (o3) o3[j - n0 - n1 - n2] = v;
+}
+
+enum { GJ_NONE = 0, GJ_COLS, GJ_COLS_SWAPPED, GJ_WGRAD, GJ_CONVT, GJ_SUMS, GJ_COLPART, GJ_BH };
+struct GradJob {
+    const float* src;
+    float* dst;
+    int kind, accumulate;
+    int first, nblk;
+    int a[6];
+};
+constexpr int kGradJobsMax = 64;
+struct GradTable { int n, pad; GradJob job[kGradJobsMax]; };
+
+int grad_job_blocks(const GradJob& j);
+size_t grad_job_lds(const GradJob& j);
+int grad_table_find(const GradTable& t, int block);
+bool grad_table_push(GradTable& t, int cap, GradJob j, int* nblocks);
+
+float* grad_slab(float* fallback, size_t count, hipStream_t st);
+bool grad_defer(const GradJob& j, hipStream_t st);
+
+}
diff --git a/general-medical-image-segmentation-cnn-framework_amd/csrc/grad_flush.hip b/general-medical-image-segmentation-cnn-framework_amd/csrc/grad_flush.hip
--- /dev/null
+++ b/general-medical-image-segmentation-cnn-framework_amd/csrc/grad_flush.hip
@@ -0,0 +1,222 @@
+#include "common.h"
+#include "internal.h"
+#include "grad_flush.h"
+#include <algorithm>
+#include <mutex>
+#include <vector>
+
+namespace seg {
+
+namespace {
+
+__global__ __launch_bounds__(256) void grad_flush_kernel(const GradTable t) {
+    extern __shared__ float tr[];
+    const int bid = (int)blockIdx.x;
+    int lo = 0, hi = t.n - 1;
+    while (lo < hi) {
+        const int mid = (lo + hi + 1) >> 1;
+        if (t.job[mid].first <= bid) lo = mid; else hi = mid - 1;
+    }
+    const GradJob& j = t.job[lo];
+    const int vb = bid - j.first;
+    switch (j.kind) {
+        case GJ_COLS: wgrad_reduce_cols_body<false>(vb, j.src, j.dst, j.a[0], j.a[1], j.a[2], j.a[3], j.accumulate); break;
+        case GJ_COLS_SWAPPED: wgrad_reduce_cols_body<true>(vb, j.src, j.dst, j.a[0], j.a[1], j.a[2], j.a[3], j.accumulate); break;
+        case GJ_WGRAD: {
+            const int gx = (j.a[3] + 31) / 32, gy = (j.a[2] + j.a[4] - 1) / j.a[4];
+            wgrad_reduce_body(tr, vb % gx, (vb / gx) % gy, vb / (gx * gy), j.src, j.dst, j.a[0], j.a[1], j.a[2], j.a[3], j.accumulate, j.a[4], j.a[5]);
+            break;
+        }
+        case GJ_CONVT: convt_wgrad_reduce_body(vb, j.src, j.dst, j.a[0], j.a[1], j.a[2]); break;
+        default: {
+            if (threadIdx.x >= 64) return;
+            if (j.kind == GJ_SUMS) {
+                double a, b;
+                sums_finalize_reduce(vb, j.src, j.a[0], j.a[1], a, b);
+                if (threadIdx.x == 0) sums_finalize_store(vb, a, b, nullptr, nullptr, j.dst, j.accumulate);
+            } else if (j.kind == GJ_COLPART) {
+                colpart_finalize_body(vb, j.src, j.a[0], j.a[1], j.dst);
+            } else if (j.kind == GJ_BH) {
+                bh_finalize_body(vb, j.src, j.a[0], j.a[1], j.dst, j.a[1], nullptr, 0, nullptr, 0, nullptr, nullptr, nullptr);
+            }
+        }
+    }
+}
+
+struct DeferState {
+    bool open = false;
+    char* arena = nullptr;
+    size_t arena_bytes = 0, used = 0;
+    size_t wanted = 0;
+    hipStream_t st = nullptr; bool have_st = false;
+    GradTable tab{};
+    int nblocks = 0; size_t lds = 0;
+    int cap = kGradJobsMax;
+    int jobs = 0, launches = 0, kinds = 0;
+    std::vector<const float*> handed;
+    std::vector<const void*> dsts;
+} g_def;
+std::mutex g_mu;
+using Lock = std::lock_guard<std::mutex>;
+
+bool in_arena(const DeferState& s, const void* p) { return s.arena && (const char*)p >= s.arena && (const char*)p < s.arena + s.used; }
+
+int flush_locked(DeferState& s) {
+    if (s.tab.n == 0) return MI355SEG_OK;
+    SEG_SET_LDS(grad_flush_kernel, 64 * 1024);
+    hipLaunchKernelGGL(grad_flush_kernel, dim3(s.nblocks), dim3(256), s.lds, s.st, s.tab);
+    s.tab.n = 0; s.nblocks = 0; s.lds = 0;
+    ++s.launches;
+    SEG_CHECK_LAUNCH();
+    return MI355SEG_OK;
+}
+
+}
+
+int grad_job_blocks(const GradJob& j) {
+    switch (j.kind) {
+        case GJ_COLS: case GJ_COLS_SWAPPED: return (int)(((long long)j.a[1] * j.a[2] * j.a[3] + 31) / 32);
+        case GJ_WGRAD: return ((j.a[3] + 31) / 32) * ((j.a[2] + j.a[4] - 1) / j.a[4]) * ((j.a[1] + j.a[5] - 1) / j.a[5]);
+        case GJ_CONVT: return (int)(((long long)8 * j.a[1] * j.a[2] + 31) / 32);
+        case GJ_SUMS: case GJ_COLPART: case GJ_BH: return j.a[1];
+        default: return 0;
+    }
+}
+
+size_t grad_job_lds(const GradJob& j) { return j.kind == GJ_WGRAD ? (size_t)32 * (j.a[4] * j.a[5] + 1) * sizeof(float) : 0; }
+
+int grad_table_find(const GradTable& t, int block) {
+    int lo = 0, hi = t.n - 1;
+    while (lo < hi) {
+        const int mid = (lo + hi + 1) >> 1;
+        if (t.job[mid].first <= block) lo = mid; else hi = mid - 1;
+    }
+    return lo;
+}
+
+bool grad_table_push(GradTable& t, int cap, GradJob j, int* nblocks) {
+    const int nb = grad_job_blocks(j);
+    if (t.n >= cap || t.n >= kGradJobsMax || nb <= 0) return false;
+    j.first = *nblocks; j.nblk = nb;
+    t.job[t.n++] = j;
+    *nblocks += nb;
+    return true;
+}
+
+float* grad_slab(float* fallback, size_t count, hipStream_t st) {
+    Lock lk(g_mu);
+    DeferState& s = g_def;
+    if (!s.open) return fallback;
+    const size_t bytes = align_up(count * sizeof(float), 256);
+    s.wanted += bytes;
+    if (s.have_st && st != s.st) return fallback;
+    if (s.used + bytes > s.arena_bytes) {
+        if (bytes > s.arena_bytes || !s.handed.empty() || flush_locked(s) != MI355SEG_OK) return fallback;
+        s.used = 0;
+    }
+    float* p = reinterpret_cast<float*>(s.arena + s.used);
+    s.used += bytes;
+    s.st = st; s.have_st = true;
+    s.handed.push_back(p);
+    return p;
+}
+
+bool grad_defer(const GradJob& j, hipStream_t st) {
+    Lock lk(g_mu);
+    DeferState& s = g_def;
+    if (!s.open) return false;
+    s.dsts.push_back(j.dst);
+    auto h = std::find(s.handed.begin(), s.handed.end(), j.src);
+    const bool mine = h != s.handed.end();
+    if (mine) s.handed.erase(h);
+    for (int i = 0; i < s.tab.n; ++i)
+        if (s.tab.job[i].dst == j.dst) { if (flush_locked(s) != MI355SEG_OK) return false; break; }
+    if (mine && j.kind != GJ_NONE && in_arena(s, j.src) && st == s.st) {
+        if (s.tab.n >= s.cap && flush_locked(s) != MI355SEG_OK) return false;
+        if (grad_table_push(s.tab, s.cap, j, &s.nblocks)) {
+            s.lds = std::max(s.lds, grad_job_lds(j));
+            ++s.jobs; s.kinds |= 1 << j.kind;
+            return true;
+        }
+    }
+    return false;
+}
+
+}
+
+using namespace seg;
+
+extern "C" {
+
+int mi355seg_grad_defer_begin(void* arena, size_t arena_bytes) {
+    Lock lk(g_mu);
+    DeferState& s = g_def;
+    SEG_CHECK_ARG(!s.open, "mi355seg_grad_defer_begin: a bracket is open (grad_defer_begin without grad_defer_end); one bracket per process at a time");
+    SEG_CHECK_ARG((arena != nullptr || arena_bytes == 0) && ((uintptr_t)arena % 256) == 0, "mi355seg_grad_defer_begin: the arena must be 256-byte aligned (NULL with 0 bytes: nothing is deferred)");
+    s.open = true;
+    s.arena = (char*)arena; s.arena_bytes = arena ? arena_bytes : 0; s.used = 0; s.wanted = 0;
+    s.st = nullptr; s.have_st = false;
+    s.tab.n = 0; s.nblocks = 0; s.lds = 0; s.jobs = 0; s.launches = 0; s.kinds = 0;
+    s.handed.clear(); s.dsts.clear();
+    return MI355SEG_OK;
+}
+
+int mi355seg_grad_defer_flush(void* stream) {
+    Lock lk(g_mu);
+    DeferState& s = g_def;
+    SEG_CHECK_ARG(s.open, "mi355seg_grad_defer_flush: no open bracket");
+    SEG_CHECK_ARG(s.tab.n == 0 || (hipStream_t)stream == s.st, "mi355seg_grad_defer_flush: the queued reductions were called on another stream");
+    return flush_locked(s);
+}
+
+int mi355seg_grad_defer_end(void) {
+    Lock lk(g_mu);
+    DeferState& s = g_def;
+    if (!s.open) return MI355SEG_OK;
+    const int rc = flush_locked(s);
+    s.open = false; s.arena = nullptr; s.arena_bytes = 0; s.used = 0; s.handed.clear();
+    return rc;
+}
+
+int mi355seg_grad_defer_active(void) { Lock lk(g_mu); return g_def.open ? 1 : 0; }
+size_t mi355seg_grad_defer_arena_bytes(void) { Lock lk(g_mu); return g_def.wanted; }
+int mi355seg_grad_defer_jobs(void) { Lock lk(g_mu); return g_def.jobs; }
+int mi355seg_grad_defer_launches(void) { Lock lk(g_mu); return g_def.launches; }
+int mi355seg_grad_defer_kinds(void) { Lock lk(g_mu); return g_def.kinds; }
+
+int mi355seg_grad_defer_outside(const void* const* base_host, const size_t* bytes_host, int n) {
+    Lock lk(g_mu);
+    int out = 0;
+    for (const void* d : g_def.dsts) {
+        bool in = false;
+        for (int i = 0; i < n && !in; ++i)
+            in = (uintptr_t)d >= (uintptr_t)base_host[i] && (uintptr_t)d < (uintptr_t)base_host[i] + bytes_host[i];
+        out += in ? 0 : 1;
+    }
+    return out;
+}
+
+int mi355seg_grad_defer_probe(const int* kind, const int* args, int njobs, int cap, int* first, int* nblk, int* grid,
+                              const int* block, int nq, int* job_of_block) {
+    GradTable t{};
+    int nblocks = 0;
+    for (int i = 0; i < njobs; ++i) {
+        GradJob j{};
+        j.kind = kind[i];
+        for (int k = 0; k < 6; ++k) j.a[k] = args[6 * i + k];
+        const bool ok = grad_table_push(t, (cap >= 1 && cap <= kGradJobsMax) ? cap : kGradJobsMax, j, &nblocks);
+        first[i] = ok ? t.job[t.n - 1].first : -1;
+        nblk[i] = ok ? t.job[t.n - 1].nblk : 0;
+    }
+    *grid = nblocks;
+    for (int q = 0; q < nq; ++q) job_of_block[q] = t.n ? grad_table_find(t, block[q]) : -1;
+    return t.n;
+}
+
+int mi355seg_grad_defer_set_cap(int cap) {
+    Lock lk(g_mu);
+    g_def.cap = (cap >= 1 && cap <= kGradJobsMax) ? cap : kGradJobsMax;
+    return MI355SEG_OK;
+}
+
+}
diff --git a/general-medical-image-segmentation-cnn-framework_amd/csrc/internal.h b/general-medical-image-segmentation-cnn-framework_amd/csrc/internal.h
--- a/general-medical-image-segmentation-cnn-framework_amd/csrc/internal.h
+++ b/general-medical-image-segmentation-cnn-framework_amd/csrc/internal.h
@@ -5,9 +5,9 @@
 
 size_t colsum_ws_bytes(int C);
 int channel_sums(const float* x, int ldx, long long rows, int C, double* sum, double* sq, float* fsum, int accumulate,
-                 void* ws, size_t ws_bytes, hipStream_t st);
+                 void* ws, size_t ws_bytes, hipStream_t st, bool param_grad = false);
 int channel_sums(const bf16* x, int ldx, long long rows, int C, double* sum, double* sq, float* fsum, int accumulate,
-                 void* ws, size_t ws_bytes, hipStream_t st);
+                 void* ws, size_t ws_bytes, hipStream_t st, bool param_grad = false);
 
 int finalize_channel_partials(const float* part, int nblk, int C, double* sum, double* sq, hipStream_t st);
 
diff --git a/general-medical-image-segmentation-cnn-framework_amd/csrc/norm.hip b/general-medical-image-segmentation-cnn-framework_amd/csrc/norm.hip
--- a/general-medical-image-segmentation-cnn-framework_amd/csrc/norm.hip
+++ b/general-medical-image-segmentation-cnn-framework_amd/csrc/norm.hip
@@ -1,5 +1,6 @@
 #include "common.h"
 #include "internal.h"
+#include "grad_flush.h"
 #include <initializer_list>
 #include <type_traits>
 
@@ -628,21 +629,15 @@
                                      double* __restrict__ sq, float* __restrict__ fsum, int accumulate,
                                      const T* __restrict__ x, int ldx, long long rows, int use_pivot) {
     const int c = blockIdx.x;
-    double a = 0.0, b = 0.0;
-    for (int k = threadIdx.x; k < nblk; k += 64) {
-        a += (double)part[((long long)k * C + c) * 2];
-        b += (double)part[((long long)k * C + c) * 2 + 1];
-    }
-    a = wave_sum(a); b = wave_sum(b);
+    double a, b;
+    sums_finalize_reduce(c, part, nblk, C, a, b);
     if (threadIdx.x != 0) return;
     if (use_pivot) {
         const double pv = (double)stats_pivot(x, ldx, 0, rows, c), n = (double)rows;
         b = b + 2.0 * pv * a + n * pv * pv;
         a = a + n * pv;
     }
-    if (sum) sum[c] = a;
-    if (sq) sq[c] = b;
-    if (fsum) fsum[c] = accumulate ? fsum[c] + (float)a : (float)a;
+    sums_finalize_store(c, a, b, sum, sq, fsum, accumulate);
 }
 
 size_t colsum_ws_bytes(int C) { return align_up((size_t)kMaxRedBlocks * C * 2 * sizeof(float), 256); }
@@ -656,14 +651,16 @@
 
 template <typename T>
 static int channel_sums_chunk(const T* x, int ldx, long long rows, int C, double* sum, double* sq, float* fsum, int accumulate,
-                              void* ws, size_t ws_bytes, hipStream_t st) {
+                              void* ws, size_t ws_bytes, hipStream_t st, bool param_grad) {
     SEG_CHECK_WS(colsum_ws_bytes(C), ws_bytes);
-    float* part = (float*)ws;
+    const bool deferrable = param_grad && fsum && !sum && !sq;
+    float* part = deferrable ? grad_slab((float*)ws, (size_t)kMaxRedBlocks * C * 2, st) : (float*)ws;
     RedPlan p;
     const int use_pivot = sq != nullptr;
     SumF<T> f{x, ldx, rows, use_pivot};
     int rc = launch_colreduce2(f, rows, 1, C, ldx, part, &p, st);
     if (rc) return rc;
+    if (deferrable && grad_defer(GradJob{part, fsum, GJ_SUMS, accumulate, 0, 0, {p.nblk, C, 0, 0, 0, 0}}, st)) return MI355SEG_OK;
     hipLaunchKernelGGL(sums_finalize_kernel<T>, dim3(C), dim3(64), 0, st, part, p.nblk, C, sum, sq, fsum, accumulate, x, ldx, rows, use_pivot);
     SEG_CHECK_LAUNCH();
     return MI355SEG_OK;
@@ -671,7 +668,7 @@
 
 template <typename T>
 static int channel_sums_t(const T* x, int ldx, long long rows, int C, double* sum, double* sq, float* fsum, int accumulate,
-                          void* ws, size_t ws_bytes, hipStream_t st) {
+                          void* ws, size_t ws_bytes, hipStream_t st, bool param_grad) {
     int c0 = 0;
     while (c0 < C) {
         int rem = C - c0, take;
@@ -682,19 +679,19 @@
             take = rem < 256 ? rem : 256;
         }
         int rc = channel_sums_chunk(x + c0, ldx, rows, take, sum ? sum + c0 : nullptr, sq ? sq + c0 : nullptr, fsum ? fsum + c0 : nullptr,
-                                    accumulate, ws, ws_bytes, st);
+                                    accumulate, ws, ws_bytes, st, param_grad);
         if (rc) return rc;
         c0 += take;
     }
     return MI355SEG_OK;
 }
 int channel_sums(const float* x, int ldx, long long rows, int C, double* sum, double* sq, float* fsum, int accumulate,
-                 void* ws, size_t ws_bytes, hipStream_t st) {
-    return channel_sums_t(x, ldx, rows, C, sum, sq, fsum, accumulate, ws, ws_bytes, st);
+                 void* ws, size_t ws_bytes, hipStream_t st, bool param_grad) {
+    return channel_sums_t(x, ldx, rows, C, sum, sq, fsum, accumulate, ws, ws_bytes, st, param_grad);
 }
 int channel_sums(const bf16* x, int ldx, long long rows, int C, double* sum, double* sq, float* fsum, int accumulate,
-                 void* ws, size_t ws_bytes, hipStream_t st) {
-    return channel_sums_t(x, ldx, rows, C, sum, sq, fsum, accumulate, ws, ws_bytes, st);
+                 void* ws, size_t ws_bytes, hipStream_t st, bool param_grad) {
+    return channel_sums_t(x, ldx, rows, C, sum, sq, fsum, accumulate, ws, ws_bytes, st, param_grad);
 }
 
 template <int NV, int MODE>
diff --git a/general-medical-image-segmentation-cnn-framework_amd/csrc/norm_api.inc b/general-medical-image-segmentation-cnn-framework_amd/csrc/norm_api.inc
--- a/general-medical-image-segmentation-cnn-framework_amd/csrc/norm_api.inc
+++ b/general-medical-image-segmentation-cnn-framework_amd/csrc/norm_api.inc
@@ -98,9 +98,10 @@
     if (dx_colsum && nrb > 1024) nrb = 1024;
     const bool fused_sum = dx_colsum && rm.lanes == (v ? C / 4 : C) && (256 % rm.lanes) == 0;
     Carver cv(ws);
+    hipStream_t st = (hipStream_t)stream;
     float* dxpart = fused_sum ? cv.take<float>((size_t)nrb * C * 2) : nullptr;
     SEG_CHECK_WS(cv.used(), ws_bytes);
-    hipStream_t st = (hipStream_t)stream;
+    if (fused_sum) dxpart = grad_slab(dxpart, (size_t)nrb * C * 2, st);
     dim3 grid(nrb, groups);
     unsigned* ao = reinterpret_cast<unsigned*>(dx_amax);
     {
@@ -115,11 +116,12 @@
     }
     if (dx_colsum) {
         if (fused_sum) {
+            if (grad_defer(GradJob{dxpart, dx_colsum, GJ_SUMS, 0, 0, 0, {nrb, C, 0, 0, 0, 0}}, st)) return MI355SEG_OK;
             hipLaunchKernelGGL(sums_finalize_kernel<float>, dim3(C), dim3(64), 0, st, dxpart, nrb, C, (double*)nullptr, (double*)nullptr, dx_colsum, 0,
                                (const float*)nullptr, 0, 0LL, 0);
             SEG_CHECK_LAUNCH();
         } else {
-            return channel_sums(dx, lddx, rows, C, nullptr, nullptr, dx_colsum, 0, ws, ws_bytes, st);
+            return channel_sums(dx, lddx, rows, C, nullptr, nullptr, dx_colsum, 0, ws, ws_bytes, st, true);
         }
     }
     return MI355SEG_OK;
diff --git a/general-medical-image-segmentation-cnn-framework_amd/distributed.py b/general-medical-image-segmentation-cnn-framework_amd/distributed.py
--- a/general-medical-image-segmentation-cnn-framework_amd/distributed.py
+++ b/general-medical-image-segmentation-cnn-framework_amd/distributed.py
@@ -168,6 +168,9 @@
     def _active(self):
         return self.always or world_size() > 1
 
+    def runs_inside_backward(self):
+        return bool(self._handles) and self._active() and not getattr(self, "_suspended", False)
+
     def suspend_hooks(self, on=True):
         self._suspended = bool(on)
         if on:
diff --git a/general-medical-image-segmentation-cnn-framework_amd/engine.py b/general-medical-image-segmentation-cnn-framework_amd/engine.py
--- a/general-medical-image-segmentation-cnn-framework_amd/engine.py
+++ b/general-medical-image-segmentation-cnn-framework_amd/engine.py
@@ -45,6 +45,13 @@
         out["jaccard"] = m["mean_jaccard"]
     else:
         out["jaccard"], out["dice"] = metric_from_counts(out["counts"].cpu().tolist())
+
+
+def _grads_read_inside_backward(model, grad_hook):
+    probe = getattr(grad_hook, "runs_inside_backward", None)
+    if probe is not None:
+        return bool(probe())
+    return any(getattr(p, "_post_accumulate_grad_hooks", None) or getattr(p, "_backward_hooks", None) for p in model.parameters())
 
 
 def train_step(model, optimizer, x, gt, criterion=None, sync_metric=True, grad_hook=None, dtype=None, step_optimizer=True, _leaves=None,
@@ -63,7 +70,8 @@
     bns = [m for m in model.modules()
            if isinstance(m, torch.nn.modules.batchnorm._BatchNorm) and m.training and m.num_batches_tracked is not None]
     F.dropout_pool_begin_step()
-    with F.prepacked_weights(model, (str(dtype or F.compute_dtype()), F.conv_math_signature(), tuple(x.shape))) as pp:
+    sig = (str(dtype or F.compute_dtype()), F.conv_math_signature(), tuple(x.shape))
+    with F.prepacked_weights(model, sig) as pp:
         if (dtype or F.compute_dtype()) == torch.float32 and not pp.replaying:
             F.prefetch_weight_amax(model)
         try:
@@ -93,7 +101,9 @@
                 mask = F.argmax_channels(pred)
                 gt_lab = F.argmax_channels(gt2)
                 counts = F.dice_counts(gt_lab, mask)
-        loss.backward()
+        with F.deferred_param_grads(model, sig, reads_inside=_grads_read_inside_backward(model, grad_hook)) as dg:
+            loss.backward()
+            dg.flush(None if _leaves is None else [t.grad for t in _leaves.values()])
     if _leaves is not None:
         for name, p in model.named_parameters():
             p.grad = _leaves[name].grad
@@ -158,6 +168,7 @@
                 optimizer.step()
         F.amax_pool_reset()
         self._prepack_arenas = [rec.get("arena") for rec in F.prepack_plans(model).values()]
+        self._grad_arenas = [rec.get("arena") for rec in F.grad_arenas(model).values()]
 
     def __call__(self, x, gt, sync_metric=True):
         self.x.copy_(x, non_blocking=True)
diff --git a/general-medical-image-segmentation-cnn-framework_amd/functional.py b/general-medical-image-segmentation-cnn-framework_amd/functional.py
--- a/general-medical-image-segmentation-cnn-framework_amd/functional.py
+++ b/general-medical-image-segmentation-cnn-framework_amd/functional.py
@@ -189,6 +189,69 @@
         elif mode == "run":
             prepacked_weights.active = False
             L.call("mi355seg_prepack_done", _stream())
+        return False
+
+
+_GRAD_DEFER_OFF = os.environ.get("MI355SEG_GRAD_DEFER", "1") == "0"
+_GRAD_ARENA_MAX = 16 << 20
+_GRAD_ARENAS = weakref.WeakKeyDictionary()
+
+
+def grad_arenas(model):
+    return _GRAD_ARENAS.get(model, {})
+
+
+class deferred_param_grads:
+
+    def __init__(self, model, key, reads_inside=False):
+        self.model, self.key, self.mode, self.off = model, key, None, reads_inside or _GRAD_DEFER_OFF
+
+    def __enter__(self):
+        if self.off:
+            return self
+        self.params = [p for p in self.model.parameters() if p.requires_grad]
+        if not self.params or not self.params[0].is_cuda:
+            return self
+        recs = _GRAD_ARENAS.get(self.model)
+        if recs is None:
+            recs = _GRAD_ARENAS[self.model] = {}
+        rec = recs.get(self.key)
+        L = lib()
+        if rec is None:
+            if torch.cuda.is_current_stream_capturing():
+                return self
+            if len(recs) >= 4:
+                recs.pop(next(iter(recs)))
+            L.call("mi355seg_grad_defer_begin", None, 0)
+            self.mode, self.recs = "measure", recs
+        elif rec["arena"] is not None:
+            L.call("mi355seg_grad_defer_begin", _p(rec["arena"]), rec["arena"].numel())
+            self.mode = "run"
+        return self
+
+    def flush(self, grads=None):
+        L = lib()
+        if self.mode == "run":
+            L.call("mi355seg_grad_defer_flush", _stream())
+        elif self.mode == "measure":
+            grads = [g for g in (grads if grads is not None else [p.grad for p in self.params]) if g is not None]
+            n = len(grads)
+            base = (ctypes.c_void_p * n)(*[g.data_ptr() for g in grads])
+            size = (ctypes.c_size_t * n)(*[g.numel() * g.element_size() for g in grads])
+            self.outside = L.query("mi355seg_grad_defer_outside", base, size, n)
+
+    def __exit__(self, *exc):
+        mode, self.mode = self.mode, None
+        if mode is None:
+            return False
+        L = lib()
+        L.call("mi355seg_grad_defer_end")
+        if mode == "measure" and exc[0] is None and getattr(self, "outside", None) is not None:
+            nbytes = int(L.query("mi355seg_grad_defer_arena_bytes"))
+            ok = self.outside == 0 and nbytes > 0
+            nbytes = min(nbytes, _GRAD_ARENA_MAX)
+            arena = torch.empty(nbytes, dtype=torch.uint8, device=self.params[0].device) if ok else None
+            self.recs[self.key] = {"arena": arena, "bytes": nbytes if ok else 0}
         return False
 
 
diff --git a/include/mi355seg.h b/include/mi355seg.h
--- a/include/mi355seg.h
+++ b/include/mi355seg.h
@@ -646,6 +646,19 @@
 int mi355seg_prepack_active(void);
 int mi355seg_prepack_free(int plan);
 
+int mi355seg_grad_defer_begin(void* arena, size_t arena_bytes);
+int mi355seg_grad_defer_flush(void* stream);
+int mi355seg_grad_defer_end(void);
+int mi355seg_grad_defer_active(void);
+size_t mi355seg_grad_defer_arena_bytes(void);
+int mi355seg_grad_defer_jobs(void);
+int mi355seg_grad_defer_launches(void);
+int mi355seg_grad_defer_kinds(void);
+int mi355seg_grad_defer_outside(const void* const* base_host, const size_t* bytes_host, int n);
+int mi355seg_grad_defer_set_cap(int cap);
+int mi355seg_grad_defer_probe(const int* kind, const int* args, int njobs, int cap, int* first, int* nblk, int* grid,
+                              const int* block, int nq, int* job_of_block);
+
 #ifdef __cplusplus
 }
 #endif
```

After: 223.4 million voxels/s (median of 6 runs). 1.01x the previous value.
